# FifthEpoch/longcat-video-tta

Hardware: AMD Instinct MI355X
Metric: denoised latent frames/sec (49x720p, 50-step CFG denoise) (higher is better)
Workload: dtype bf16; 1 GPU; K3: 49x720p (13 latent frames, 46 800 tokens); DiT 48 blocks x 4096 hidden, CFG 4.0, 50-step flow-match Euler, no conditioning frames; depth=48, parallelism=dp1

## Files before the change

### include/lcv_hip.h

```cpp
#ifndef LCV_HIP_H
#define LCV_HIP_H

#include <stdint.h>

#ifdef __cplusplus
extern "C" {
#endif

#define LCV_OK 0
#define LCV_EINVAL (-1)
#define LCV_EDEVICE (-2)
#define LCV_ELAUNCH (-3)

int lcv_version(void);
const char* lcv_last_error(void);
int lcv_device_check(void);

int lcv_knobs_reload(void);
const char* lcv_knobs_list(void);

int lcv_adaln_modulate_fwd(const void* x, const float* mod, void* y,
                           int64_t B, int64_t T, int64_t S, int64_t C,
                           int64_t mod_stride, int64_t shift_off, int64_t scale_off,
                           float eps, void* stream);
int lcv_adaln_modulate_bwd(const void* x, const float* mod, const void* dy,
                           void* dx, float* dmod,
                           int64_t B, int64_t T, int64_t S, int64_t C,
                           int64_t mod_stride, int64_t shift_off, int64_t scale_off,
                           float eps, const void* dres, void* stream);
int lcv_layernorm_affine_fwd(const void* x, const float* w, const float* b, void* y,
                             int64_t rows, int64_t C, float eps, void* stream);
int lcv_layernorm_affine_bwd(const void* x, const float* w, const void* dy,
                             void* dx, float* dw, float* db,
                             int64_t rows, int64_t C, float eps, const void* dres, void* stream);

int lcv_gate_residual_fwd(const void* x, const void* y, const float* mod, void* out,
                          int64_t B, int64_t T, int64_t S, int64_t C,
                          int64_t mod_stride, int64_t gate_off, void* stream);
int lcv_gate_residual_bwd(const void* y, const float* mod, const void* dout,
                          void* dy, float* dmod,
                          int64_t B, int64_t T, int64_t S, int64_t C,
                          int64_t mod_stride, int64_t gate_off, void* stream);

int lcv_qknorm_rope_fwd(const void* q_in, const void* k_in, const void* v_in,
                        void* q_out, void* k_out, void* v_out,
                        const void* wq, const void* wk, const void* cs,
                        int64_t B, int64_t N, int64_t H,
                        int64_t in_sb, int64_t in_sn,
                        int64_t q_sb, int64_t q_sn,
                        int64_t kv_sb, int64_t kv_sn,
                        int64_t pos_off, float eps, float q_scale, void* stream);
int lcv_qknorm_rope_bwd(const void* q_in, const void* k_in,
                        const void* dq_out, const void* dk_out,
                        void* dq_in, void* dk_in,
                        const void* wq, const void* wk, const void* cs,
                        int64_t B, int64_t N, int64_t H,
                        int64_t in_sb, int64_t in_sn,
                        int64_t q_sb, int64_t q_sn,
                        int64_t kv_sb, int64_t kv_sn,
                        int64_t din_sb, int64_t din_sn,
                        int64_t pos_off, float eps, float q_scale, float* dwq, float* dwk, int64_t dw_slots, void* stream);

int lcv_timestep_embedding(const float* t, float* out, int64_t n, int64_t dim, float max_period, void* stream);

int lcv_attn_fwd(const void* q, const void* k, const void* v, void* o, float* lse,
                 int64_t B, int64_t H, int64_t Nq, int64_t Nk,
                 int64_t q_sb, int64_t q_sn, int64_t q_sh,
                 int64_t k_sb, int64_t k_sn, int64_t k_sh,
                 int64_t v_sb, int64_t v_sn, int64_t v_sh,
                 int64_t o_sb, int64_t o_sn, int64_t o_sh,
                 float scale, void* stream);
const char* lcv_attn_fwd_last_kernel(void);
int64_t lcv_attn_bwd_ws_floats(int64_t B, int64_t H, int64_t Nq, int64_t Nk);
int lcv_attn_bwd(const void* q, const void* k, const void* v, const void* o,
                 const void* d_o, const float* lse,
                 void* dq, void* dk, void* dv,
                 float* delta_ws, int accumulate_kv,
                 int64_t B, int64_t H, int64_t Nq, int64_t Nk,
                 int64_t q_sb, int64_t q_sn, int64_t q_sh,
                 int64_t k_sb, int64_t k_sn, int64_t k_sh,
                 int64_t v_sb, int64_t v_sn, int64_t v_sh,
                 int64_t o_sb, int64_t o_sn, int64_t o_sh,
                 int64_t dq_sb, int64_t dq_sn, int64_t dq_sh,
                 int64_t dk_sb, int64_t dk_sn, int64_t dk_sh,
                 int64_t dv_sb, int64_t dv_sn, int64_t dv_sh,
                 float scale, void* stream);

#define LCV_EPI_NONE 0
#define LCV_EPI_SWIGLU 1
#define LCV_EPI_GATE_RESIDUAL 2
#define LCV_EPI_GELU_TANH 3
#define LCV_EPI_SILU 4
int lcv_gemm_nt(const void* a, const void* w, const void* bias,
                const void* a2, const void* w2,
                void* c, int64_t M, int64_t N, int64_t K, int64_t K2,
                int64_t lda, int64_t ldw, int64_t lda2, int64_t ldw2, int64_t ldc,
                int epilogue, int out_f32,
                const void* resid, const float* mod, int64_t rows_per_frame,
                int64_t mod_stride, int64_t gate_off,
                void* stream);
int lcv_gemm_set_workspace(void* ws, int64_t bytes);
int lcv_lora_down(const void* x, const void* A, void* h, int64_t M, int64_t K, int64_t R,
                  int64_t Rpad, int64_t ldx, float s, void* stream);
int lcv_tn_skinny(const void* g, const void* x, float* out, int64_t M, int64_t K, int64_t R, int64_t Rpad,
                  int64_t ldx, float scale, float* ws, int64_t ws_bytes, void* stream);
int64_t lcv_tn_skinny_ws_bytes(int64_t M, int64_t K, int64_t R);
int lcv_linear_f32_smallm(const float* a, const void* w, const void* bias, float* out, int64_t M, int64_t N,
                          int64_t K, int act_in, void* stream);
int lcv_linear_f32_smallm_bwd(const float* dy, const void* w, const float* a, float* da, int64_t M, int64_t N,
                              int64_t K, int act_in, void* stream);

int lcv_swiglu_fwd(const void* gate, const void* up, void* out, int64_t rows, int64_t F,
                   int64_t ld_in, void* stream);
int lcv_swiglu_bwd(const void* gate, const void* up, const void* dout, void* dgate, void* dup,
                   int64_t rows, int64_t F, int64_t ld_in, void* stream);
int lcv_swiglu_bwd_interleaved(const void* gu, const void* dout, void* dgu, int64_t rows, int64_t F, void* stream);

int lcv_patchify(const void* x, void* tok, int64_t B, int64_t Cin, int64_t T, int64_t H, int64_t W,
                 int64_t Kpad, void* stream);
int lcv_unpatchify(const void* tok, float* out, int64_t B, int64_t Cout, int64_t T, int64_t H, int64_t W,
                   int tok_is_f32, void* stream);
int lcv_unpatchify_bwd(const float* dout, float* dtok, int64_t B, int64_t Cout, int64_t T, int64_t H, int64_t W,
                       void* stream);

int lcv_cfg_euler_step(const float* cond, const float* uncond, float* x, float* ws,
                       int64_t B, int64_t n, float guidance, float dt, int negate,
                       int use_zero_star, void* stream);
int lcv_euler_step(const float* v, float* x, int64_t n, float dt, int negate, void* stream);

int lcv_fm_noise(const void* x0, const void* eps, const float* sigma, void* out,
                 int64_t B, int64_t per_sample, void* stream);
#define LCV_FM_MSE_BLOCKS 1024
int lcv_fm_mse(const float* pred, const void* eps, const void* x0, float* loss_out, float* dpred, float* ws,
               int64_t B, int64_t C, int64_t T, int64_t Tc, int64_t HW, void* stream);
#define LCV_FM_MSE_PARTS 256
int lcv_fm_mse_samples(const float* pred, const void* eps, const void* x0, float* loss_out, float* ws,
                       int64_t B, int64_t C, int64_t T, int64_t Tc, int64_t HW, int64_t eps_bstride,
                       int64_t x0_bstride, void* stream);

typedef struct {
  void* param;
  void* grad;
  void* exp_avg;
  void* exp_avg_sq;
  int64_t numel;
  int64_t first_chunk;
} lcv_adam_tensor;
int lcv_grad_norm_clip(const lcv_adam_tensor* tensors, int64_t n_tensors, int64_t total_chunks, int param_f32,
                       float max_norm, float* per_tensor_ws, float* norm_coef_out, void* stream);
int lcv_adamw_step(const lcv_adam_tensor* tensors, int64_t n_tensors, int64_t total_chunks, int param_f32,
                   const float* norm_coef, double lr, double beta1, double beta2, double eps, double weight_decay,
                   int64_t step, void* stream);

int lcv_sgd_step(const lcv_adam_tensor* tensors, int64_t n_tensors, int64_t total_chunks, int param_f32,
                 const float* norm_coef, double lr, double weight_decay, void* stream);

int lcv_transpose_pad(const void* in, void* out, int64_t M, int64_t N, int64_t ld, int64_t Mpad, void* stream);
int lcv_rowsum(const void* in, void* out, int64_t rows, int64_t cols, int out_f32, void* stream);
int lcv_linear_f32_smallm_wgrad(const float* dy, const float* a, void* dw, void* db, int64_t M, int64_t N, int64_t K,
                                int act_in, void* stream);
int lcv_gelu_tanh_fwd(const void* x, void* y, int64_t n, void* stream);
int lcv_gelu_tanh_bwd(const void* x, const void* dy, void* dx, int64_t n, void* stream);

int lcv_causal_conv3d(const void* x, const void* w, const void* bias, const void* resid, void* out,
                      const void* zero_page, int64_t B, int64_t Tin, int64_t Hin, int64_t Win, int64_t Cin,
                      int64_t Cout, int64_t ldc, int kt, int kh, int kw, int up2x, void* stream);
const char* lcv_conv3d_last_kernel(void);
int lcv_conv3d_strided(const void* x, const void* w, const void* bias, void* out, const void* zero_page, int64_t B,
                       int64_t Tin, int64_t Hin, int64_t Win, int64_t Cin, int64_t Cout, int64_t ldc, int kt, int kh,
                       int kw, int st, int sh, int sw, int64_t Tout, int64_t Hout, int64_t Wout, void* stream);
int lcv_vae_rmsnorm_silu(const void* x, const void* gamma, void* y, int64_t rows, int64_t C, int64_t Cpad,
                         int apply_silu, void* stream);
int lcv_softmax_rows(const float* s, void* p, int64_t rows, int64_t n, int64_t ld_s, int64_t ld_p, float scale,
                     void* stream);

int lcv_frame_metric_partials(int64_t H, int64_t W, int64_t C, int win, int64_t* n_sqerr, int64_t* n_ssim);
int lcv_frame_sqerr(const float* gen, const void* gt, int gt_is_u8, float* partials, int64_t N, int64_t E, void* stream);
int lcv_frame_ssim(const float* gen, const void* gt, int gt_is_u8, float* partials, int64_t N, int64_t H, int64_t W,
                   int64_t C, const float* window , int win, float cov_norm,
                   int clamp_var, float c1, float c2, void* stream);

int lcv_gather_rows(const void* table, const int64_t* ids, void* out, int64_t n, int64_t C, int64_t vocab, void* stream);
int lcv_t5_rmsnorm(const void* x, const void* w, void* y, int64_t rows, int64_t C, float eps, void* stream);
int lcv_geglu_tanh_fwd(const void* gate, const void* up, void* out, int64_t rows, int64_t F, int64_t ld_in, void* stream);
int lcv_t5_attention(const void* q, const void* k, const void* v, void* out, const float* bias_by_dist,
                     const int* key_mask, int64_t B, int64_t S, int64_t H, int64_t ld_qkv, int64_t ld_o, int64_t bs_qkv,
                     int64_t bs_o, void* stream);

#ifdef __cplusplus
}
#endif
#endif
```

### longcat-video-tta_amd/csrc/attn_common.h

```cpp
#pragma once
#include "lcv_common.h"

#define AS3 __attribute__((address_space(3)))
typedef AS3 unsigned char lds_u8;
typedef __attribute__((address_space(1))) void gbl_void_t;
typedef AS3 void lds_void_t;
#define SCHED_FENCE() __builtin_amdgcn_sched_barrier(0)
#define ATTN_RESCALE_THR 6.0f

__device__ __forceinline__ int lane_now() { return (int)__builtin_amdgcn_mbcnt_hi(~0u, __builtin_amdgcn_mbcnt_lo(~0u, 0u)); }

__device__ __forceinline__ void half_pair(float v, float& lo, float& hi) {
  float a = v, b = v;
  asm volatile("s_nop 1\n\tv_permlane32_swap_b32 %0, %1\n\ts_nop 0" : "+v"(a), "+v"(b));
  lo = a;
  hi = b;
}
__device__ __forceinline__ float half_max(float v) {
  float lo, hi;
  half_pair(v, lo, hi);
  return fmaxf(lo, hi);
}
__device__ __forceinline__ float half_sum(float v) {
  float lo, hi;
  half_pair(v, lo, hi);
  return lo + hi;
}

__device__ __forceinline__ float gap_exp2(float x) { float y; asm volatile("v_exp_f32 %0, %1" : "=v"(y) : "v"(x)); return y; }
__device__ __forceinline__ float gap_add(float a, float b) { float y; asm volatile("v_add_f32 %0, %1, %2" : "=v"(y) : "v"(a), "v"(b)); return y; }
__device__ __forceinline__ float gap_max3(float a, float b, float c) { float y; asm volatile("v_max3_f32 %0, %1, %2, %3" : "=v"(y) : "v"(a), "v"(b), "v"(c)); return y; }
__device__ __forceinline__ unsigned gap_pack(float lo, float hi) { unsigned y; asm volatile("v_cvt_pk_bf16_f32 %0, %1, %2" : "=v"(y) : "v"(lo), "v"(hi)); return y; }

__device__ __forceinline__ int attn_swz(int row) { return ((row & 3) << 2) | ((row >> 2) & 3); }
__device__ __forceinline__ int attn_tile_off(int row, int ch) { return 256 * row + 16 * (ch ^ attn_swz(row)); }

#define ATTN_BLOCK_DECODE(p, blk, head, b)            \
  {                                                   \
    if ((p).xcd_remap) {                              \
      const int id = blockIdx.x;                      \
      const int xcd = id & 7, j = id >> 3;            \
      const int pair = (j / (p).gx) * 8 + xcd;        \
      blk = j - (j / (p).gx) * (p).gx;                \
      head = pair % (p).d.H;                          \
      b = pair / (p).d.H;                             \
    } else {                                          \
      blk = blockIdx.x; head = blockIdx.y; b = blockIdx.z; \
    }                                                 \
  }
struct AttnGrid { int gx, xcd_remap; dim3 grid; };
static inline AttnGrid attn_grid(int64_t B, int64_t H, int64_t blocks, bool enabled) {
  AttnGrid g;
  g.gx = (int)blocks;
  g.xcd_remap = (enabled && (B * H) % 8 == 0 && blocks >= 8) ? 1 : 0;
  g.grid = g.xcd_remap ? dim3((unsigned)blocks * (unsigned)(H * B)) : dim3((unsigned)blocks, (unsigned)H, (unsigned)B);
  return g;
}

struct AttnArgs {
  const void *q, *k, *v;
  void* o;
  const void* d_o;
  float* lse;
  float* delta_ws;
  void *dq, *dk, *dv;
  int64_t B, H, Nq, Nk;
  int64_t q_sb, q_sn, q_sh, k_sb, k_sn, k_sh, v_sb, v_sn, v_sh, o_sb, o_sn, o_sh;
  int64_t dq_sb, dq_sn, dq_sh, dk_sb, dk_sn, dk_sh, dv_sb, dv_sn, dv_sh;
  float scale;
  int accumulate_kv;
};
struct AttnDims {
  int64_t Nq, Nk;
  int H;
  int64_t q_sb, q_sn, q_sh, k_sb, k_sn, k_sh, v_sb, v_sn, v_sh, o_sb, o_sn, o_sh;
};
static inline AttnDims attn_dims(const AttnArgs& a) {
  return {a.Nq, a.Nk, (int)a.H, a.q_sb, a.q_sn, a.q_sh, a.k_sb, a.k_sn, a.k_sh, a.v_sb, a.v_sn, a.v_sh, a.o_sb, a.o_sn, a.o_sh};
}
struct AttnFwdLead {
  const bf16_t* q;
  const bf16_t* k;
  const bf16_t* v;
  bf16_t* o;
  float* lse;
  AttnDims d;
};
static inline AttnFwdLead attn_fwd_lead(const AttnArgs& a) {
  return {(const bf16_t*)a.q, (const bf16_t*)a.k, (const bf16_t*)a.v, (bf16_t*)a.o, a.lse, attn_dims(a)};
}

static inline bool attn_raise_lds(const void* kern, size_t bytes) {
  return hipFuncSetAttribute(kern, hipFuncAttributeMaxDynamicSharedMemorySize, (int)bytes) == hipSuccess;
}
#define ATTN_RAISE_LDS_ONCE(name, ok)                        \
  do {                                                       \
    static const bool attr_ok__ = (ok);                      \
    if (!attr_ok__) {                                        \
      lcv_set_error("%s: cannot raise dynamic LDS", name);   \
      return LCV_EDEVICE;                                    \
    }                                                        \
  } while (0)

int attn_fwd_w64_launch(const AttnArgs& a, bool xcd_ok, hipStream_t s);
int attn_fwd_pipe_launch(const AttnArgs& a, bool xcd_ok, hipStream_t s);
int attn_bwd_dq2_launch(const AttnArgs& a, hipStream_t s);
int attn_bwd_dkv2_launch(const AttnArgs& a, hipStream_t s);
```

### longcat-video-tta_amd/csrc/attn_fwd.hip

```cpp
#include "attn_common.h"
#include <type_traits>

struct AttnFwdParams : AttnFwdLead {
  float scale, scale_log2e;
  int gx, xcd_remap;
};

template <int NWAVES, int PRIO, bool XATTN, int VAR>
__global__ __launch_bounds__(NWAVES * 64) void attn_fwd_kernel(const AttnFwdParams p) {
  constexpr bool DMA = (VAR & 1) != 0;
  constexpr bool UNIT = (VAR & 2) != 0;
  static_assert(!DMA || NWAVES == 8, "LDS-DMA staging is laid out for 8 waves (2 K + 2 V instructions per wave)");
  constexpr int NT = NWAVES * 64;
  constexpr int QROWS = NWAVES * 32;
  constexpr int NCH = 1024 / NT;
  constexpr int TILE_BYTES = 64 * 256;
  extern __shared__ __attribute__((aligned(16))) unsigned char smem[];
  lds_u8* lds = (lds_u8*)smem;

  const int tid = threadIdx.x;
  const int lane = tid & 63;
  const int wave = __builtin_amdgcn_readfirstlane(tid >> 6);
  const int r = lane & 31, h = lane >> 5;
  int qb, head;
  int64_t b;
  ATTN_BLOCK_DECODE(p, qb, head, b);
  const int64_t q0 = (int64_t)qb * QROWS + wave * 32;

  const bf16_t* kbase = p.k + b * p.d.k_sb + (int64_t)head * p.d.k_sh;
  const bf16_t* vbase = p.v + b * p.d.v_sb + (int64_t)head * p.d.v_sh;

  bf16x8 qf[8];
  {
    int64_t qrow = q0 + r;
    if (qrow > p.d.Nq - 1) qrow = p.d.Nq - 1;
    const bf16_t* qp = p.q + b * p.d.q_sb + qrow * p.d.q_sn + (int64_t)head * p.d.q_sh + 8 * h;
#pragma unroll
    for (int ks = 0; ks < 8; ++ks) qf[ks] = *reinterpret_cast<const bf16x8*>(qp + 16 * ks);
  }

  int st_off[NCH];
  int st_row[NCH];
#pragma unroll
  for (int i = 0; i < NCH; ++i) {
    const int c = tid + i * NT;
    st_row[i] = c >> 4;
    st_off[i] = attn_tile_off(c >> 4, c & 15);
  }
  const int st_col = (tid & 15) * 8;
  u32x4 kreg[NCH], vreg[NCH];
  const bf16_t* kdma[2];
  const bf16_t* vdma[2];
  int dma_row[2], dma_col[2];
#pragma unroll
  for (int i = 0; i < 2; ++i) {
    dma_row[i] = 8 * wave + 4 * i + (lane >> 4);
    dma_col[i] = 8 * ((lane & 15) ^ attn_swz(dma_row[i]));
    kdma[i] = kbase + dma_row[i] * p.d.k_sn + dma_col[i];
    vdma[i] = vbase + dma_row[i] * p.d.v_sn + dma_col[i];
  }
  auto dma_half = [&](auto which_c, int t, int buf, auto full_c) {
    constexpr int which = decltype(which_c)::value;
    constexpr bool FULL = decltype(full_c)::value;
    lds_u8* dst = lds + buf * 2 * TILE_BYTES + which * TILE_BYTES + wave * 2048;
    const bf16_t** src = which ? vdma : kdma;
    const int64_t sn = which ? p.d.v_sn : p.d.k_sn;
    if (FULL || (int64_t)t * 64 + 64 <= p.d.Nk) {
#pragma unroll
      for (int i = 0; i < 2; ++i) {
        __builtin_amdgcn_global_load_lds((gbl_void_t*)src[i], (lds_void_t*)(dst + 1024 * i), 16, 0, 0);
        src[i] += 64 * sn;
      }
    } else {
#pragma unroll
      for (int i = 0; i < 2; ++i) {
        int64_t back = (int64_t)t * 64 + dma_row[i] - (p.d.Nk - 1);
        if (back < 0) back = 0;
        __builtin_amdgcn_global_load_lds((gbl_void_t*)(src[i] - back * sn), (lds_void_t*)(dst + 1024 * i), 16, 0, 0);
      }
    }
  };
  using K_ = std::integral_constant<int, 0>;
  using V_ = std::integral_constant<int, 1>;
  auto dma_tile = [&](int t, int buf, auto full_c) {
    dma_half(K_{}, t, buf, full_c);
    dma_half(V_{}, t, buf, full_c);
  };
  auto load_tile = [&](int64_t kv0) {
#pragma unroll
    for (int i = 0; i < NCH; ++i) {
      int64_t row = kv0 + st_row[i];
      if (row > p.d.Nk - 1) row = p.d.Nk - 1;
      kreg[i] = *reinterpret_cast<const u32x4*>(kbase + row * p.d.k_sn + st_col);
      vreg[i] = *reinterpret_cast<const u32x4*>(vbase + row * p.d.v_sn + st_col);
    }
  };
  auto store_tile = [&](int buf) {
    lds_u8* kb = lds + buf * 2 * TILE_BYTES;
#pragma unroll
    for (int i = 0; i < NCH; ++i) {
      *reinterpret_cast<__attribute__((address_space(3))) u32x4*>(kb + st_off[i]) = kreg[i];
      *reinterpret_cast<__attribute__((address_space(3))) u32x4*>(kb + TILE_BYTES + st_off[i]) = vreg[i];
    }
  };

  const int kf = attn_swz(r);
  const int k_row_off = 256 * r;
  const int q4 = (lane >> 2) & 3, p4 = lane & 3, g1 = (lane >> 4) & 1;
  int v_base[2], v_low[2];
#pragma unroll
  for (int half = 0; half < 2; ++half) {
    v_base[half] = 256 * (4 * h + 8 * half + q4) + 8 * (p4 & 1);
    v_low[half] = (2 * g1 + (p4 >> 1)) ^ (h + 2 * half);
  }

  f32x16 oacc[4];
#pragma unroll
  for (int d = 0; d < 4; ++d)
#pragma unroll
    for (int e = 0; e < 16; ++e) oacc[d][e] = 0.f;
  float m_run = UNIT ? 0.f : -INFINITY;
  f32x16 minit;
#pragma unroll
  for (int e = 0; e < 16; ++e) minit[e] = 0.f;
  float l_run = 0.f;

  if (PRIO == 1 && wave >= NWAVES / 2) __builtin_amdgcn_s_setprio(1);
  const int nt = (int)((p.d.Nk + 63) / 64);
  {
    if (DMA) {
      dma_tile(0, 0, std::false_type{});
    } else {
      load_tile(0);
      store_tile(0);
    }
    __syncthreads();
  }

  auto tile_body = [&](const int t, auto buf_c, auto last_c, auto next_full_c) {
    constexpr int buf = decltype(buf_c)::value;
    constexpr bool has_next = !decltype(last_c)::value;
    if (has_next) {
      if (DMA) dma_tile(t + 1, buf ^ 1, next_full_c);
      else load_tile((int64_t)(t + 1) * 64);
    }

    const lds_u8* kb = lds + buf * 2 * TILE_BYTES;
    const lds_u8* vb = kb + TILE_BYTES;

    f32x16 s0, s1;
#pragma unroll
    for (int e = 0; e < 16; ++e) { s0[e] = UNIT ? minit[e] : 0.f; s1[e] = UNIT ? minit[e] : 0.f; }
#pragma unroll
    for (int ks = 0; ks < 8; ++ks) {
      const int co = 16 * ((2 * ks + h) ^ kf);
      const bf16x8 a0 = *reinterpret_cast<const __attribute__((address_space(3))) bf16x8*>(kb + k_row_off + co);
      const bf16x8 a1 = *reinterpret_cast<const __attribute__((address_space(3))) bf16x8*>(kb + 32 * 256 + k_row_off + co);
      s0 = __builtin_amdgcn_mfma_f32_32x32x16_bf16(a0, qf[ks], s0, 0, 0, 0);
      s1 = __builtin_amdgcn_mfma_f32_32x32x16_bf16(a1, qf[ks], s1, 0, 0, 0);
    }

    if (!has_next && (p.d.Nk & 63)) {
      const int valid = (int)(p.d.Nk - (int64_t)t * 64);
#pragma unroll
      for (int e = 0; e < 16; ++e) {
        const int key = (e & 3) + 8 * (e >> 2) + 4 * h;
        if (key >= valid) s0[e] = -INFINITY;
        if (key + 32 >= valid) s1[e] = -INFINITY;
      }
    }

    float mxa = s0[0], mxb = s1[0];
#pragma unroll
    for (int e = 1; e < 16; ++e) {
      mxa = fmaxf(mxa, s0[e]);
      mxb = fmaxf(mxb, s1[e]);
    }
    float mx = fmaxf(mxa, mxb);
    mx = half_max(mx);
    float psum = 0.f;
    if constexpr (UNIT) {
      if (__builtin_amdgcn_ballot_w64(mx > ATTN_RESCALE_THR) != 0ull || t == 0) {
        const float d = (t == 0) ? mx : fmaxf(mx, 0.f);
        const float alpha = __builtin_amdgcn_exp2f(-d);
        m_run += d;
        l_run *= alpha;
#pragma unroll
        for (int dd = 0; dd < 4; ++dd)
#pragma unroll
          for (int e = 0; e < 16; ++e) oacc[dd][e] *= alpha;
#pragma unroll
        for (int e = 0; e < 16; ++e) {
          s0[e] -= d;
          s1[e] -= d;
          minit[e] = -m_run;
        }
      }
#pragma unroll
      for (int e = 0; e < 16; ++e) {
        s0[e] = __builtin_amdgcn_exp2f(s0[e]);
        s1[e] = __builtin_amdgcn_exp2f(s1[e]);
        psum += s0[e] + s1[e];
      }
    } else {
      if (__builtin_amdgcn_ballot_w64((mx - m_run) * p.scale_log2e > ATTN_RESCALE_THR) != 0ull) {
        const float m_new = fmaxf(m_run, mx);
        const float alpha = __builtin_amdgcn_exp2f((m_run - m_new) * p.scale_log2e);
        m_run = m_new;
        l_run *= alpha;
#pragma unroll
        for (int d = 0; d < 4; ++d)
#pragma unroll
          for (int e = 0; e < 16; ++e) oacc[d][e] *= alpha;
      }
      const float mc = m_run * p.scale_log2e;
#pragma unroll
      for (int e = 0; e < 16; ++e) {
        s0[e] = __builtin_amdgcn_exp2f(s0[e] * p.scale_log2e - mc);
        s1[e] = __builtin_amdgcn_exp2f(s1[e] * p.scale_log2e - mc);
        psum += s0[e] + s1[e];
      }
    }
    l_run += psum;

    bf16x8 pb[4];
#pragma unroll
    for (int j = 0; j < 8; ++j) {
      pb[0][j] = (__bf16)s0[j];
      pb[1][j] = (__bf16)s0[8 + j];
      pb[2][j] = (__bf16)s1[j];
      pb[3][j] = (__bf16)s1[8 + j];
    }

#pragma unroll
    for (int kk = 0; kk < 4; ++kk) {
#pragma unroll
      for (int d = 0; d < 4; ++d) {
        const int dx = 64 * (d ^ q4);
        const s16x4 lo = __builtin_amdgcn_ds_read_tr16_b64_v4i16(
            (__attribute__((address_space(3))) s16x4*)(vb + v_base[0] + 4096 * kk + dx + 16 * v_low[0]));
        const s16x4 hi = __builtin_amdgcn_ds_read_tr16_b64_v4i16(
            (__attribute__((address_space(3))) s16x4*)(vb + v_base[1] + 4096 * kk + dx + 16 * v_low[1]));
        const bf16x8 vf = __builtin_bit_cast(bf16x8, __builtin_shufflevector(lo, hi, 0, 1, 2, 3, 4, 5, 6, 7));
        oacc[d] = __builtin_amdgcn_mfma_f32_32x32x16_bf16(vf, pb[kk], oacc[d], 0, 0, 0);
      }
    }

    if (has_next && !DMA) store_tile(buf ^ 1);
    __syncthreads();
  };
  {
    using B0 = std::integral_constant<int, 0>;
    using B1 = std::integral_constant<int, 1>;
    using Y = std::true_type;
    using N = std::false_type;
    int t = 0;
    for (; t + 3 < nt; t += 2) {
      tile_body(t, B0{}, N{}, Y{});
      tile_body(t + 1, B1{}, N{}, Y{});
    }
    const int left = nt - t;
    if (left == 3) {
      tile_body(t, B0{}, N{}, Y{});
      tile_body(t + 1, B1{}, N{}, N{});
      tile_body(t + 2, B0{}, Y{}, N{});
    } else if (left == 2) {
      tile_body(t, B0{}, N{}, N{});
      tile_body(t + 1, B1{}, Y{}, N{});
    } else {
      tile_body(t, B0{}, Y{}, N{});
    }
  }

  const float l_tot = half_sum(l_run);
  const float inv = 1.0f / l_tot;
  const int64_t qrow = q0 + r;
  if (qrow < p.d.Nq) {
    bf16_t* op = p.o + b * p.d.o_sb + qrow * p.d.o_sn + (int64_t)head * p.d.o_sh;
#pragma unroll
    for (int d = 0; d < 4; ++d)
#pragma unroll
      for (int i = 0; i < 4; ++i) {
        u16x4 pk;
#pragma unroll
        for (int e = 0; e < 4; ++e) pk[e] = f2bf(oacc[d][4 * i + e] * inv);
        *reinterpret_cast<u16x4*>(op + 32 * d + 8 * i + 4 * h) = pk;
      }
    if (p.lse && h == 0) p.lse[(b * p.d.H + head) * p.d.Nq + qrow] = m_run * p.scale + __logf(l_tot);
  }
}

static thread_local const char* g_last_attn_kernel = "none";
extern "C" const char* lcv_attn_fwd_last_kernel(void) { return g_last_attn_kernel; }

extern "C" int lcv_attn_fwd(const void* q, const void* k, const void* v, void* o, float* lse, int64_t B,
                            int64_t H, int64_t Nq, int64_t Nk, int64_t q_sb, int64_t q_sn, int64_t q_sh,
                            int64_t k_sb, int64_t k_sn, int64_t k_sh, int64_t v_sb, int64_t v_sn,
                            int64_t v_sh, int64_t o_sb, int64_t o_sn, int64_t o_sh, float scale,
                            void* stream) {
  LCV_CHECK_ARG(q && k && v && o, "attn_fwd: null pointer");
  LCV_CHECK_ARG(B > 0 && H > 0 && H <= 65535 && B <= 65535, "attn_fwd: bad B/H");
  LCV_CHECK_ARG(Nk > 0, "attn_fwd: Nk must be > 0 (empty key set has no softmax)");
  LCV_CHECK_ARG(q_sn % 8 == 0 && k_sn % 8 == 0 && v_sn % 8 == 0 && q_sh % 8 == 0 && k_sh % 8 == 0 &&
                    v_sh % 8 == 0 && q_sb % 8 == 0 && k_sb % 8 == 0 && v_sb % 8 == 0,
                "attn_fwd: q/k/v strides must be multiples of 8 elements");
  LCV_CHECK_ARG(o_sn % 4 == 0 && o_sh % 4 == 0 && o_sb % 4 == 0, "attn_fwd: o strides must be multiples of 4 elements");
  LCV_CHECK_ARG(((uintptr_t)q % 16 == 0) && ((uintptr_t)k % 16 == 0) && ((uintptr_t)v % 16 == 0) && ((uintptr_t)o % 8 == 0),
                "attn_fwd: pointers must be 16-byte aligned");
  if (Nq == 0) return LCV_OK;
  AttnArgs a = {};
  a.q = q; a.k = k; a.v = v; a.o = o; a.lse = lse; a.B = B; a.H = H; a.Nq = Nq; a.Nk = Nk; a.scale = scale;
  a.q_sb = q_sb; a.q_sn = q_sn; a.q_sh = q_sh; a.k_sb = k_sb; a.k_sn = k_sn; a.k_sh = k_sh;
  a.v_sb = v_sb; a.v_sn = v_sn; a.v_sh = v_sh; a.o_sb = o_sb; a.o_sn = o_sn; a.o_sh = o_sh;
  constexpr int NW = 8;
  const size_t lds = 2 * 2 * 64 * 256;
  const char* xe = lcv_knob("LCV_ATTN_XCD");
  const bool xcd_ok = !(xe && xe[0] == '0');
  const AttnGrid g = attn_grid(B, H, (Nq + NW * 32 - 1) / (NW * 32), xcd_ok);
  const AttnFwdParams p = {attn_fwd_lead(a), scale, scale * 1.4426950408889634f, g.gx, g.xcd_remap};
  auto launch = [&](auto kern) -> int {
    if (!attn_raise_lds((const void*)kern, lds)) {
      lcv_set_error("attn_fwd: cannot raise dynamic LDS");
      return LCV_EDEVICE;
    }
    hipLaunchKernelGGL(kern, g.grid, dim3(NW * 64), lds, (hipStream_t)stream, p);
    return LCV_OK;
  };
  const bool unit = p.scale_log2e > 1.0f - 4e-7f && p.scale_log2e < 1.0f + 4e-7f;
  int rc;
  const bool span32 = (uint64_t)Nk * (uint64_t)(k_sn > v_sn ? k_sn : v_sn) * 2 < (1ull << 32) &&
                      (uint64_t)Nq * (uint64_t)q_sn * 2 < (1ull << 32);
  const char* we = lcv_knob("LCV_ATTN_FWD_W64");
  if (unit && Nk > 512 && span32 && !(we && we[0] == '0')) {
    g_last_attn_kernel = "attn_fwd_w64_kernel";
    return attn_fwd_w64_launch(a, xcd_ok, (hipStream_t)stream);
  }
  if (unit && Nk > 512 && span32) {
    g_last_attn_kernel = "attn_fwd_pipe_kernel";
    return attn_fwd_pipe_launch(a, xcd_ok, (hipStream_t)stream);
  }
  if (Nk <= 512) { g_last_attn_kernel = "attn_fwd_kernel<8, 0, true, 0>"; rc = launch(attn_fwd_kernel<NW, 0, true, 0>); }
  else if (unit) { g_last_attn_kernel = "attn_fwd_kernel<8, 0, false, 3>"; rc = launch(attn_fwd_kernel<NW, 0, false, 3>); }
  else { g_last_attn_kernel = "attn_fwd_kernel<8, 0, false, 1>"; rc = launch(attn_fwd_kernel<NW, 0, false, 1>); }
  if (rc != LCV_OK) return rc;
  LCV_LAUNCH_CHECK("attn_fwd");
  return LCV_OK;
}
```

### longcat-video-tta_amd/csrc/attn_fwd_w64.hip

```cpp
#include "attn_common.h"
#include <type_traits>

struct AttnFwdW64Params : AttnFwdLead {
  float scale;
  int gx, xcd_remap;
};

template <int I, int N, class F>
__device__ __forceinline__ void w64_static_for(F&& f) {
  if constexpr (I < N) { f(std::integral_constant<int, I>{}); w64_static_for<I + 1, N>(f); }
}
enum : unsigned char { W64_NONE, W64_EXP, W64_ADD, W64_PACK, W64_LRUN, W64_VOFF, W64_MAX, W64_HMAX, W64_BALLOT, W64_M0, W64_DMA };
struct W64Op { unsigned char kind, b, e; };
constexpr int W64_SLOTS = 6;
constexpr W64Op W64_P1[32][W64_SLOTS] = {
  {{W64_EXP, 0, 0}, {W64_EXP, 1, 0}},
  {{W64_EXP, 0, 1}},
  {{W64_PACK, 0, 0}, {W64_ADD, 0, 1}, {W64_EXP, 1, 1}, {W64_EXP, 0, 2}},
  {{W64_ADD, 0, 2}, {W64_PACK, 1, 0}, {W64_ADD, 1, 1}, {W64_EXP, 1, 2}},
  {{W64_ADD, 1, 2}, {W64_EXP, 0, 3}, {W64_EXP, 1, 3}},
  {{W64_PACK, 0, 1}, {W64_ADD, 0, 3}, {W64_PACK, 1, 1}, {W64_ADD, 1, 3}, {W64_EXP, 0, 4}},
  {{W64_ADD, 0, 4}, {W64_EXP, 1, 4}, {W64_EXP, 0, 5}},
  {{W64_PACK, 0, 2}, {W64_ADD, 0, 5}, {W64_ADD, 1, 4}, {W64_EXP, 1, 5}},
  {{W64_PACK, 1, 2}, {W64_ADD, 1, 5}, {W64_EXP, 0, 6}, {W64_EXP, 1, 6}},
// ... 76 lines not shown
constexpr bool w64_apart(int from, int to) {
  const int gf = from / 8, gt = to / 8;
  for (int g = gf; g <= gt; ++g) {
    const int ph = g < 32 ? 1 : 2, i = g & 31;
    if ((g > gf && w64_read_first(ph, i)) || (g < gt && w64_wait_last(ph, i))) return true;
  }
  return false;
}
constexpr bool w64_table_complete() {
  int exp_at[2][32] = {}, add_at[2][32] = {}, pack_at[2][16] = {}, max_at[2][9] = {}, n = 0;
  for (int b = 0; b < 2; ++b) for (int m = 0; m < 9; ++m) max_at[b][m] = -1;
  for (int b = 0; b < 2; ++b) for (int e = 0; e < 32; ++e) { exp_at[b][e] = -1; add_at[b][e] = -1; }
  for (int b = 0; b < 2; ++b) for (int m = 0; m < 16; ++m) pack_at[b][m] = -1;
  for (int g = 0; g < 64; ++g)
    for (int s = 0; s < W64_SLOTS; ++s) {
      const W64Op o = g < 32 ? W64_P1[g][s] : W64_P2[g - 32][s];
      const int at = 8 * g + s;
      if (o.kind == W64_EXP) { if (exp_at[o.b][o.e] >= 0) return false; exp_at[o.b][o.e] = at; ++n; }
      if (o.kind == W64_ADD) { if (o.e == 0 || exp_at[o.b][o.e] < 0 || (o.e > 1 && add_at[o.b][o.e - 1] < 0)) return false; add_at[o.b][o.e] = at; }
      if (o.kind == W64_PACK) { if (exp_at[o.b][2 * o.e] < 0 || exp_at[o.b][2 * o.e + 1] < 0) return false; pack_at[o.b][o.e] = at; }
      if (o.kind == W64_LRUN && add_at[o.b][31] < 0) return false;
      if (o.kind == W64_MAX) { if (o.e > 0 && max_at[o.b][o.e - 1] < 0) return false; max_at[o.b][o.e] = at; }
      if (o.kind == W64_HMAX && max_at[o.b][8] < 0) return false;
      if (o.kind == W64_ADD && !(w64_apart(exp_at[o.b][o.e], at) && w64_apart(o.e == 1 ? exp_at[o.b][0] : add_at[o.b][o.e - 1], at))) return false;
      if (o.kind == W64_PACK && !(w64_apart(exp_at[o.b][2 * o.e], at) && w64_apart(exp_at[o.b][2 * o.e + 1], at))) return false;
      if (o.kind == W64_LRUN && !w64_apart(add_at[o.b][31], at)) return false;
      if (o.kind == W64_MAX && o.e > 0 && !w64_apart(max_at[o.b][o.e - 1], at)) return false;
      if (o.kind == W64_HMAX && !w64_apart(max_at[o.b][8], at)) return false;
    }
  for (int b = 0; b < 2; ++b)
    for (int m = 0; m < 16; ++m)
      if (pack_at[b][m] < 0 || pack_at[b][m] >= 8 * (32 + 8 * (m / 4) + b - 1) + W64_SLOTS) return false;
  return n == 64;
}
static_assert(w64_table_complete(), "attn_fwd_w64 gap table: an exp, add or pack is missing, doubled, out of order or right behind what it reads");
static_assert(w64_table_ok(W64_P1, 1, 38, 2) && w64_table_ok(W64_P2, 2, 37, 1), "attn_fwd_w64 gap table over its budget");

template <bool GUARD>
__device__ __forceinline__ void mfma_s(f32x16& c, const bf16x8& a, const bf16x8& b) {
  if constexpr (GUARD) asm volatile("s_nop 3\n\tv_mfma_f32_32x32x16_bf16 %0, %1, %2, %0" : "+v"(c) : "v"(a), "a"(b));
  else asm volatile("v_mfma_f32_32x32x16_bf16 %0, %1, %2, %0" : "+v"(c) : "v"(a), "a"(b));
}
template <bool GUARD>
__device__ __forceinline__ void mfma_s_first(f32x16& d, const f32x16& c, const bf16x8& a, const bf16x8& b) {
  if constexpr (GUARD) asm volatile("s_nop 3\n\tv_mfma_f32_32x32x16_bf16 %0, %2, %3, %1" : "=&v"(d) : "v"(c), "v"(a), "a"(b));
  else asm volatile("v_mfma_f32_32x32x16_bf16 %0, %2, %3, %1" : "=&v"(d) : "v"(c), "v"(a), "a"(b));
}
template <bool GUARD>
__device__ __forceinline__ void mfma_o(f32x16& c, const bf16x8& a, const bf16x8& b) {
  if constexpr (GUARD) asm volatile("s_nop 3\n\tv_mfma_f32_32x32x16_bf16 %0, %1, %2, %0" : "+a"(c) : "v"(a), "v"(b));
  else asm volatile("v_mfma_f32_32x32x16_bf16 %0, %1, %2, %0" : "+a"(c) : "v"(a), "v"(b));
}

#define SCW(S, nb, j) (S[(j) >> 4][nb][(j) & 15])

__global__ __launch_bounds__(256) void attn_fwd_w64_kernel(const AttnFwdW64Params p) {
  constexpr int TILE = 64 * 256;
  extern __shared__ __attribute__((aligned(16))) unsigned char smem[];
  lds_u8* lds = (lds_u8*)smem;
  constexpr int V_REGION = 2 * TILE;

  const int tid = threadIdx.x;
  const int lane = tid & 63;
  const int wave = __builtin_amdgcn_readfirstlane(tid >> 6);
  const int r = lane & 31, h = lane >> 5;
  int qb, head;
  int64_t b;
  ATTN_BLOCK_DECODE(p, qb, head, b);
  const int64_t q0 = (int64_t)qb * 256 + wave * 64;
  const int nt = (int)((p.d.Nk + 63) / 64);
  const bool ragged = (p.d.Nk & 63) != 0;
  const char* kbase_u = lcv_uniform_ptr(p.k + b * p.d.k_sb + (int64_t)head * p.d.k_sh);
  const char* vbase_u = lcv_uniform_ptr(p.v + b * p.d.v_sb + (int64_t)head * p.d.v_sh);

  auto dma_row_of = [&](int ln, int i) { return 16 * wave + 4 * i + (ln >> 4); };
  auto dma_colb_of = [&](int ln, int i) {
    const int row = dma_row_of(ln, i);
    return 16 * ((ln & 15) ^ attn_swz(row));
  };
  unsigned koff[4], voff[4];
#pragma unroll
  for (int i = 0; i < 4; ++i) {
    koff[i] = (unsigned)(dma_row_of(lane, i) * p.d.k_sn * 2 + dma_colb_of(lane, i));
    voff[i] = (unsigned)(dma_row_of(lane, i) * p.d.v_sn * 2 + dma_colb_of(lane, i));
  }
  auto last_off = [&](int i, int64_t sn) {
    const int ln = lane_now();
    int64_t row = (int64_t)(nt - 1) * 64 + dma_row_of(ln, i);
    if (row > p.d.Nk - 1) row = p.d.Nk - 1;
    return (unsigned)(row * sn * 2 + dma_colb_of(ln, i));
  };
  const unsigned lds_wave = (unsigned)(uintptr_t)lds + (unsigned)wave * 4096u;
  auto dma_one = [&](int which, int i, int dst_tile, int tile, bool known_full) __attribute__((always_inline)) {
    const int64_t sn = which ? p.d.v_sn : p.d.k_sn;
    const char* base = which ? vbase_u : kbase_u;
    unsigned off = which ? voff[i] : koff[i];
    if (!known_full && tile == nt - 1) off = last_off(i, sn);
    else base += (int64_t)tile * (128 * sn);
    asm volatile("s_mov_b32 m0, %2\n\ts_nop 0\n\tglobal_load_lds_dwordx4 %0, %1"
                 :: "v"(off), "s"(base), "s"(lds_wave + (unsigned)dst_tile + 1024u * i) : "memory", "m0");
  };
  auto dma_m0 = [&](int i, int dst_tile) __attribute__((always_inline)) {
    asm volatile("s_mov_b32 m0, %0" :: "s"(lds_wave + (unsigned)dst_tile + 1024u * i) : "memory", "m0");
  };
  auto dma_req = [&](int which, int i, int tile, bool known_full) __attribute__((always_inline)) {
    const int64_t sn = which ? p.d.v_sn : p.d.k_sn;
    const char* base = which ? vbase_u : kbase_u;
    unsigned off = which ? voff[i] : koff[i];
    if (!known_full && tile == nt - 1) off = last_off(i, sn);
    else base += (int64_t)tile * (128 * sn);
    asm volatile("global_load_lds_dwordx4 %0, %1" :: "v"(off), "s"(base) : "memory");
  };
  auto dma_tile = [&](int which, int dst_tile, int tile) __attribute__((always_inline)) {
#pragma unroll
    for (int i = 0; i < 4; ++i) dma_one(which, i, dst_tile, tile, false);
  };
  constexpr int KOP = 0, VOP = 1;
  auto dma_wait_and_barrier = [&]() { asm volatile("s_waitcnt vmcnt(0)\n\ts_barrier" ::: "memory"); };

  int k_off[8];
  int v_off[2][4];
  auto set_read_offsets = [&](int ln, int slot) {
    const int rr = ln & 31, hh = ln >> 5;
    const int kfz = ((rr & 3) << 2) | ((rr >> 2) & 3);
#pragma unroll
    for (int ks = 0; ks < 8; ++ks) k_off[ks] = 256 * rr + 16 * ((2 * ks + hh) ^ kfz);
    const int q4 = (ln >> 2) & 3, p4 = ln & 3, g1 = (ln >> 4) & 1;
#pragma unroll
    for (int half = 0; half < 2; ++half)
#pragma unroll
      for (int d = 0; d < 4; ++d)
        v_off[half][d] = (int)(unsigned)(uintptr_t)lds + V_REGION + slot * TILE + 256 * (4 * hh + 8 * half + q4) + 8 * (p4 & 1) + 64 * (d ^ q4) +
                         16 * ((2 * g1 + (p4 >> 1)) ^ (hh + 2 * half));
  };
  set_read_offsets(lane, 2);
  auto read_k = [&](const lds_u8* kb, int f) __attribute__((always_inline)) -> bf16x8 {
    return *reinterpret_cast<const AS3 bf16x8*>(kb + (f & 1) * 32 * 256 + k_off[f >> 1]);
  };
  auto read_v = [&](int g) __attribute__((always_inline)) -> bf16x8 {
    const s16x4 lo = __builtin_amdgcn_ds_read_tr16_b64_v4i16((AS3 s16x4*)(uintptr_t)(unsigned)(v_off[0][g & 3] + 4096 * (g >> 2)));
    const s16x4 hi = __builtin_amdgcn_ds_read_tr16_b64_v4i16((AS3 s16x4*)(uintptr_t)(unsigned)(v_off[1][g & 3] + 4096 * (g >> 2)));
    return __builtin_bit_cast(bf16x8, __builtin_shufflevector(lo, hi, 0, 1, 2, 3, 4, 5, 6, 7));
  };

  bf16x8 qf[2][8];
#pragma unroll
  for (int nb = 0; nb < 2; ++nb) {
    int64_t qrow = q0 + 32 * nb + r;
    if (qrow > p.d.Nq - 1) qrow = p.d.Nq - 1;
    const bf16_t* qp = p.q + b * p.d.q_sb + qrow * p.d.q_sn + (int64_t)head * p.d.q_sh + 8 * h;
#pragma unroll
    for (int ks = 0; ks < 8; ++ks) qf[nb][ks] = *reinterpret_cast<const bf16x8*>(qp + 16 * ks);
  }
#pragma unroll
  for (int nb = 0; nb < 2; ++nb)
#pragma unroll
    for (int ks = 0; ks < 8; ++ks) asm volatile("" : "+a"(qf[nb][ks]));

  f32x16 oacc[2][4];
#pragma unroll
  for (int nb = 0; nb < 2; ++nb)
#pragma unroll
    for (int d = 0; d < 4; ++d) {
#pragma unroll
      for (int e = 0; e < 16; ++e) oacc[nb][d][e] = 0.f;
      asm volatile("" : "+a"(oacc[nb][d]));
    }
  float m_run[2] = {0.f, 0.f}, l_run[2] = {0.f, 0.f};
  f32x16 minit[2];
#pragma unroll
  for (int nb = 0; nb < 2; ++nb)
#pragma unroll
    for (int e = 0; e < 16; ++e) minit[nb][e] = 0.f;
  f32x16 sa[2][2], sb[2][2];

  auto mask_last = [&](f32x16 (&s)[2][2]) __attribute__((always_inline)) {
    const int valid = (int)(p.d.Nk - (int64_t)(nt - 1) * 64);
    const int hh_ = lane_now() >> 5;
#pragma unroll
    for (int nb = 0; nb < 2; ++nb)
#pragma unroll
      for (int e = 0; e < 16; ++e) {
        const int key = (e & 3) + 8 * (e >> 2) + 4 * hh_;
        if (key >= valid) s[0][nb][e] = -INFINITY;
        if (key + 32 >= valid) s[1][nb][e] = -INFINITY;
      }
  };
  auto fence_o = [&]() __attribute__((always_inline)) {
    asm volatile("s_nop 15\n\ts_nop 15\n\ts_nop 15\n\ts_nop 15"
                 : "+a"(oacc[0][0]), "+a"(oacc[0][1]), "+a"(oacc[0][2]), "+a"(oacc[0][3]), "+a"(oacc[1][0]), "+a"(oacc[1][1]),
                   "+a"(oacc[1][2]), "+a"(oacc[1][3]));
  };
  auto fence_s = [&](f32x16 (&s)[2][2]) __attribute__((always_inline)) {
    asm volatile("s_nop 15\n\ts_nop 15\n\ts_nop 15\n\ts_nop 15" : "+v"(s[0][0]), "+v"(s[0][1]), "+v"(s[1][0]), "+v"(s[1][1]));
  };
  auto settle = [&](f32x16 (&s)[2][2], auto nb_c, float mx, bool first, bool need) __attribute__((always_inline)) {
    constexpr int nb = decltype(nb_c)::value;
    if (need || first) {
      fence_o();
      const float d = first ? mx : fmaxf(mx, 0.f);
      const float alpha = __builtin_amdgcn_exp2f(-d);
      m_run[nb] += d;
      l_run[nb] *= alpha;
#pragma unroll
      for (int dd = 0; dd < 4; ++dd)
#pragma unroll
        for (int e = 0; e < 16; ++e) oacc[nb][dd][e] *= alpha;
#pragma unroll
      for (int e = 0; e < 16; ++e) {
        s[0][nb][e] -= d;
        s[1][nb][e] -= d;
        asm volatile("v_mov_b32 %0, %1" : "+v"(minit[nb][e]) : "v"(-m_run[nb]));
      }
      fence_o();
    }
  };

#ifndef W64_PD
#define W64_PD 2
#endif
  constexpr int PD = W64_PD, RING = PD + 1;
  bf16x8 kfr[RING], vfr[RING];
  int v_slot = 2;
  auto next_v_slot = [&]() __attribute__((always_inline)) -> int {
    v_slot = (v_slot == 2) ? 0 : v_slot + 1;
    return (v_slot == 0) ? -2 * TILE : TILE;
  };

  dma_tile(KOP, 0, 0);
  dma_tile(VOP, V_REGION, 0);
  dma_tile(KOP, TILE, 1);
  dma_tile(VOP, V_REGION + TILE, 1);
  dma_wait_and_barrier();
  {
#pragma unroll
    for (int kb_ = 0; kb_ < 2; ++kb_)
#pragma unroll
      for (int nb = 0; nb < 2; ++nb)
#pragma unroll
        for (int e = 0; e < 16; ++e) sa[kb_][nb][e] = 0.f;
#pragma unroll
    for (int f = 0; f < 16; ++f) {
      const bf16x8 a = read_k(lds, f);
      mfma_s<true>(sa[f & 1][0], a, qf[0][f >> 1]);
      mfma_s<true>(sa[f & 1][1], a, qf[1][f >> 1]);
    }
    fence_s(sa);
    auto first_settle = [&](auto nb_c) __attribute__((always_inline)) {
      constexpr int nb = decltype(nb_c)::value;
      float mx = sa[0][nb][0];
#pragma unroll
      for (int e = 1; e < 16; ++e) mx = fmaxf(mx, sa[0][nb][e]);
#pragma unroll
      for (int e = 0; e < 16; ++e) mx = fmaxf(mx, sa[1][nb][e]);
      settle(sa, nb_c, half_max(mx), true, true);
    };
    first_settle(std::integral_constant<int, 0>{});
    first_settle(std::integral_constant<int, 1>{});
  }
  __syncthreads();
  dma_tile(KOP, 0, 2);
#pragma unroll
  for (int i = 0; i < PD; ++i) kfr[i] = read_k(lds + TILE, i);

  auto iteration = [&](const int t, auto par_c, auto steady_c, f32x16 (&c)[2][2], f32x16 (&n)[2][2]) __attribute__((always_inline)) {
    constexpr int PAR = decltype(par_c)::value;
    constexpr bool STEADY = decltype(steady_c)::value;
    const lds_u8* kb = lds + (PAR ^ 1) * TILE;
    const lds_u8* kb_next = lds + PAR * TILE;
    const bool has_k3 = STEADY || t + 3 < nt;
    const bool has_v2 = STEADY || t + 2 < nt;
    const int v_delta = next_v_slot();
    const int v_dst = V_REGION + ((v_slot == 0) ? 2 : v_slot - 1) * TILE;
    float psum[2];
    float ex[2][32];
    unsigned pw[2][16];
    float mxa[2] = {0.f, 0.f}, mxb[2] = {0.f, 0.f}, mxh[2] = {0.f, 0.f};
    bool need[2] = {false, false};
    auto run_op = [&](auto phase_c, auto gap_c, auto slot_c) __attribute__((always_inline)) {
      constexpr W64Op o = decltype(phase_c)::value == 1 ? W64_P1[decltype(gap_c)::value][decltype(slot_c)::value]
                                                        : W64_P2[decltype(gap_c)::value][decltype(slot_c)::value];
      constexpr int b_ = o.b, e = o.e;
      if constexpr (o.kind == W64_EXP) ex[b_][e] = gap_exp2(SCW(c, b_, e));
      if constexpr (o.kind == W64_ADD) psum[b_] = gap_add((e == 1) ? ex[b_][0] : psum[b_], ex[b_][e]);
      if constexpr (o.kind == W64_PACK) pw[b_][e] = gap_pack(ex[b_][2 * e], ex[b_][2 * e + 1]);
      if constexpr (o.kind == W64_LRUN) l_run[b_] = gap_add(l_run[b_], psum[b_]);
      if constexpr (o.kind == W64_VOFF) asm volatile("v_add_u32 %0, %1, %0" : "+v"(v_off[b_ >> 2][b_ & 3]) : "s"(v_delta));
      if constexpr (o.kind == W64_MAX) {
        if constexpr (e == 0) {
          mxa[b_] = gap_max3(n[0][b_][0], n[0][b_][1], n[0][b_][2]);
          mxb[b_] = gap_max3(n[1][b_][0], n[1][b_][1], n[1][b_][2]);
        } else if constexpr (e < 7) {
          mxa[b_] = gap_max3(mxa[b_], n[0][b_][2 * e + 1], n[0][b_][2 * e + 2]);
          mxb[b_] = gap_max3(mxb[b_], n[1][b_][2 * e + 1], n[1][b_][2 * e + 2]);
        } else if constexpr (e == 7) {
          mxa[b_] = gap_max3(mxa[b_], n[0][b_][15], mxb[b_]);
        } else {
          mxb[b_] = gap_max3(mxa[b_], n[1][b_][15], n[1][b_][14]);
        }
      }
      if constexpr (o.kind == W64_HMAX) mxh[b_] = half_max(mxb[b_]);
      if constexpr (o.kind == W64_BALLOT) need[b_] = __builtin_amdgcn_ballot_w64(mxh[b_] > ATTN_RESCALE_THR) != 0ull;
      if constexpr (o.kind == W64_M0) {
        if constexpr (b_ < 4) { if (has_k3) dma_m0(b_, (PAR ^ 1) * TILE); }
        else { if (has_v2) dma_m0(b_ & 3, v_dst); }
      }
// ... 139 lines not shown
```

### longcat-video-tta_amd/csrc/elementwise.hip

```cpp
#include "lcv_common.h"
#include "cfg_guidance.h"

#define ROWNORM_MAXCH 8

template <int MODE>
__global__ __launch_bounds__(256) void rownorm_fwd_kernel(
    const bf16_t* __restrict__ x, const float* __restrict__ p_add, const float* __restrict__ p_mul,
    bf16_t* __restrict__ y, int64_t rows, int C, int64_t S, int64_t mod_stride, float eps) {
  const int lane = threadIdx.x & 63;
  const int64_t row = (int64_t)blockIdx.x * 4 + (threadIdx.x >> 6);
  if (row >= rows) return;
  const bf16_t* xr = x + row * C;
  float v[ROWNORM_MAXCH][8];
  float sum = 0.f;
#pragma unroll
  for (int ch = 0; ch < ROWNORM_MAXCH; ++ch) {
    const int c = (ch * 64 + lane) * 8;
    if (c < C) {
      u16x8 raw = *reinterpret_cast<const u16x8*>(xr + c);
      unpack8(raw, v[ch]);
#pragma unroll
      for (int i = 0; i < 8; ++i) sum += v[ch][i];
    } else {
#pragma unroll
      for (int i = 0; i < 8; ++i) v[ch][i] = 0.f;
    }
  }
  const float mean = wave_sum(sum) / (float)C;
  float sq = 0.f;
#pragma unroll
  for (int ch = 0; ch < ROWNORM_MAXCH; ++ch) {
    const int c = (ch * 64 + lane) * 8;
    if (c < C) {
#pragma unroll
      for (int i = 0; i < 8; ++i) {
        const float d = v[ch][i] - mean;
        sq += d * d;
      }
    }
  }
  const float rstd = rsqrtf(wave_sum(sq) / (float)C + eps);
  const float* pa = p_add;
  const float* pm = p_mul;
  if (MODE == 0) {
    const int64_t frame = row / S;
    pa += frame * mod_stride;
    pm += frame * mod_stride;
  }
  bf16_t* yr = y + row * C;
#pragma unroll
  for (int ch = 0; ch < ROWNORM_MAXCH; ++ch) {
    const int c = (ch * 64 + lane) * 8;
    if (c < C) {
      const f32x4 a0 = *reinterpret_cast<const f32x4*>(pa + c);
      const f32x4 a1 = *reinterpret_cast<const f32x4*>(pa + c + 4);
      const f32x4 m0 = *reinterpret_cast<const f32x4*>(pm + c);
      const f32x4 m1 = *reinterpret_cast<const f32x4*>(pm + c + 4);
      float o[8];
#pragma unroll
      for (int i = 0; i < 8; ++i) {
        const float xh = (v[ch][i] - mean) * rstd;
        const float mul = (i < 4) ? m0[i] : m1[i - 4];
        const float add = (i < 4) ? a0[i] : a1[i - 4];
        o[i] = (MODE == 0) ? (xh * (mul + 1.0f) + add) : (xh * mul + add);
      }
      *reinterpret_cast<u16x8*>(yr + c) = pack8(o);
    }
  }
}

extern "C" int lcv_adaln_modulate_fwd(const void* x, const float* mod, void* y, int64_t B, int64_t T,
                                      int64_t S, int64_t C, int64_t mod_stride, int64_t shift_off,
                                      int64_t scale_off, float eps, void* stream) {
  LCV_CHECK_ARG(x && mod && y, "adaln_modulate_fwd: null pointer");
  LCV_CHECK_ARG(C > 0 && C % 8 == 0 && C <= 4096, "adaln_modulate_fwd: C=%ld must be a multiple of 8 and <= 4096", (long)C);
  LCV_CHECK_ARG(B > 0 && T > 0 && S > 0, "adaln_modulate_fwd: bad sizes");
  LCV_CHECK_ARG(shift_off % 4 == 0 && scale_off % 4 == 0 && mod_stride % 4 == 0, "adaln_modulate_fwd: offsets must be 16-byte aligned");
  const int64_t rows = B * T * S;
  const unsigned grid = (unsigned)((rows + 3) / 4);
  hipLaunchKernelGGL(rownorm_fwd_kernel<0>, dim3(grid), dim3(256), 0, (hipStream_t)stream,
                     (const bf16_t*)x, mod + shift_off, mod + scale_off, (bf16_t*)y, rows, (int)C, S,
                     mod_stride, eps);
  LCV_LAUNCH_CHECK("adaln_modulate_fwd");
  return LCV_OK;
}

extern "C" int lcv_layernorm_affine_fwd(const void* x, const float* w, const float* b, void* y,
                                        int64_t rows, int64_t C, float eps, void* stream) {
  LCV_CHECK_ARG(x && w && b && y, "layernorm_affine_fwd: null pointer");
  LCV_CHECK_ARG(C > 0 && C % 8 == 0 && C <= 4096, "layernorm_affine_fwd: C=%ld must be a multiple of 8 and <= 4096", (long)C);
  if (rows == 0) return LCV_OK;
  const unsigned grid = (unsigned)((rows + 3) / 4);
  hipLaunchKernelGGL(rownorm_fwd_kernel<1>, dim3(grid), dim3(256), 0, (hipStream_t)stream,
                     (const bf16_t*)x, b, w, (bf16_t*)y, rows, (int)C, (int64_t)1, (int64_t)0, eps);
  LCV_LAUNCH_CHECK("layernorm_affine_fwd");
  return LCV_OK;
}

__global__ __launch_bounds__(256) void gate_residual_fwd_kernel(
    const bf16_t* __restrict__ x, const bf16_t* __restrict__ y, const float* __restrict__ gate,
    bf16_t* __restrict__ out, int64_t n_packets, int cpk , int64_t S, int64_t mod_stride) {
  for (int64_t p = (int64_t)blockIdx.x * blockDim.x + threadIdx.x; p < n_packets;
       p += (int64_t)gridDim.x * blockDim.x) {
    const int64_t row = p / cpk;
    const int c = (int)(p - row * cpk) * 8;
    float xf[8], yf[8], o[8];
    unpack8(*reinterpret_cast<const u16x8*>(x + p * 8), xf);
    unpack8(*reinterpret_cast<const u16x8*>(y + p * 8), yf);
    if (gate) {
      const float* g = gate + (row / S) * mod_stride + c;
      const f32x4 g0 = *reinterpret_cast<const f32x4*>(g);
      const f32x4 g1 = *reinterpret_cast<const f32x4*>(g + 4);
#pragma unroll
      for (int i = 0; i < 8; ++i) o[i] = xf[i] + ((i < 4) ? g0[i] : g1[i - 4]) * yf[i];
    } else {
#pragma unroll
      for (int i = 0; i < 8; ++i) o[i] = xf[i] + yf[i];
    }
    *reinterpret_cast<u16x8*>(out + p * 8) = pack8(o);
  }
}

extern "C" int lcv_gate_residual_fwd(const void* x, const void* y, const float* mod, void* out,
                                     int64_t B, int64_t T, int64_t S, int64_t C, int64_t mod_stride,
                                     int64_t gate_off, void* stream) {
  LCV_CHECK_ARG(x && y && out, "gate_residual_fwd: null pointer");
  LCV_CHECK_ARG(C > 0 && C % 8 == 0, "gate_residual_fwd: C must be a multiple of 8");
  LCV_CHECK_ARG(gate_off % 4 == 0 && mod_stride % 4 == 0, "gate_residual_fwd: offsets must be 16-byte aligned");
  const int64_t n_packets = B * T * S * (C / 8);
  if (n_packets == 0) return LCV_OK;
  int64_t blocks = (n_packets + 255) / 256;
  if (blocks > 256 * 16) blocks = 256 * 16;
  hipLaunchKernelGGL(gate_residual_fwd_kernel, dim3((unsigned)blocks), dim3(256), 0, (hipStream_t)stream,
                     (const bf16_t*)x, (const bf16_t*)y, mod ? mod + gate_off : nullptr, (bf16_t*)out,
                     n_packets, (int)(C / 8), S, mod_stride);
  LCV_LAUNCH_CHECK("gate_residual_fwd");
  return LCV_OK;
}

__device__ __forceinline__ void norm_rope_vec(const bf16_t* src, bf16_t* dst, const float (&w)[8],
                                              const float (&cs)[8], bool do_rope, float eps, float out_scale) {
  float f[8];
  unpack8(*reinterpret_cast<const u16x8*>(src), f);
  float ss = 0.f;
#pragma unroll
  for (int i = 0; i < 8; ++i) ss += f[i] * f[i];
  ss += __shfl_xor(ss, 8, 64);
  ss += __shfl_xor(ss, 4, 64);
  ss += __shfl_xor(ss, 2, 64);
  ss += __shfl_xor(ss, 1, 64);
  const float r = rsqrtf(ss * (1.0f / 128.0f) + eps);
  float o[8];
#pragma unroll
  for (int i = 0; i < 8; ++i) f[i] = bfround(bfround(f[i] * r) * w[i]);
  if (do_rope) {
#pragma unroll
    for (int i = 0; i < 4; ++i) {
      const float c = cs[2 * i], s = cs[2 * i + 1];
      const float x0 = f[2 * i], x1 = f[2 * i + 1];
      o[2 * i] = __fadd_rn(__fmul_rn(x0, c), __fmul_rn(-x1, s));
      o[2 * i + 1] = __fadd_rn(__fmul_rn(x1, c), __fmul_rn(x0, s));
    }
  } else {
#pragma unroll
    for (int i = 0; i < 8; ++i) o[i] = f[i];
  }
#pragma unroll
  for (int i = 0; i < 8; ++i) o[i] *= out_scale;
  *reinterpret_cast<u16x8*>(dst) = pack8(o);
}

__global__ __launch_bounds__(256) void qknorm_rope_fwd_kernel(
    const bf16_t* __restrict__ q_in, const bf16_t* __restrict__ k_in, const bf16_t* __restrict__ v_in,
    bf16_t* __restrict__ q_out, bf16_t* __restrict__ k_out, bf16_t* __restrict__ v_out,
    const bf16_t* __restrict__ wq, const bf16_t* __restrict__ wk, const float* __restrict__ cs_tab,
    int H, int64_t in_sb, int64_t in_sn, int64_t q_sb, int64_t q_sn, int64_t kv_sb, int64_t kv_sn,
    int64_t pos_off, float eps, float q_scale) {
  const int64_t n = blockIdx.x, b = blockIdx.y;
  const int sub = threadIdx.x & 15;
  const int hl = threadIdx.x >> 4;
  float cs[8] = {1, 0, 1, 0, 1, 0, 1, 0};
  const bool do_rope = cs_tab != nullptr;
  if (do_rope) {
    const float* p = cs_tab + ((pos_off + n) * 64 + sub * 4) * 2;
    const f32x4 a = *reinterpret_cast<const f32x4*>(p);
    const f32x4 c = *reinterpret_cast<const f32x4*>(p + 4);
    cs[0] = a[0]; cs[1] = a[1]; cs[2] = a[2]; cs[3] = a[3];
    cs[4] = c[0]; cs[5] = c[1]; cs[6] = c[2]; cs[7] = c[3];
  }
  float wqf[8], wkf[8];
  unpack8(*reinterpret_cast<const u16x8*>(wq + sub * 8), wqf);
  unpack8(*reinterpret_cast<const u16x8*>(wk + sub * 8), wkf);
  const int64_t in_base = b * in_sb + n * in_sn;
  for (int h0 = 0; h0 < H; h0 += 16) {
    const int h = h0 + hl;
    if (h >= H) continue;
    const int64_t off = (int64_t)h * 128 + sub * 8;
    if (q_in) norm_rope_vec(q_in + in_base + off, q_out + b * q_sb + n * q_sn + off, wqf, cs, do_rope, eps, q_scale);
    if (k_in) norm_rope_vec(k_in + in_base + off, k_out + b * kv_sb + n * kv_sn + off, wkf, cs, do_rope, eps, 1.0f);
    if (v_out) {
      *reinterpret_cast<u16x8*>(v_out + b * kv_sb + n * kv_sn + off) =
          *reinterpret_cast<const u16x8*>(v_in + in_base + off);
    }
  }
}

extern "C" int lcv_qknorm_rope_fwd(const void* q_in, const void* k_in, const void* v_in, void* q_out,
                                   void* k_out, void* v_out, const void* wq, const void* wk,
                                   const void* cs, int64_t B, int64_t N, int64_t H, int64_t in_sb,
                                   int64_t in_sn, int64_t q_sb, int64_t q_sn, int64_t kv_sb,
                                   int64_t kv_sn, int64_t pos_off, float eps, float q_scale, void* stream) {
  LCV_CHECK_ARG((q_in || k_in) && wq && wk, "qknorm_rope_fwd: null pointer");
  LCV_CHECK_ARG(q_scale > 0.f, "qknorm_rope_fwd: q_scale must be positive (1 = none)");
  LCV_CHECK_ARG(!q_in || q_out, "qknorm_rope_fwd: q_out missing");
  LCV_CHECK_ARG(!k_in || k_out, "qknorm_rope_fwd: k_out missing");
  LCV_CHECK_ARG(H > 0, "qknorm_rope_fwd: H must be positive");
  LCV_CHECK_ARG(in_sn % 8 == 0 && q_sn % 8 == 0 && kv_sn % 8 == 0 && in_sb % 8 == 0 && q_sb % 8 == 0 && kv_sb % 8 == 0,
                "qknorm_rope_fwd: strides must be multiples of 8 elements");
  if (B == 0 || N == 0) return LCV_OK;
  const bool copy_v = v_out && v_in && v_out != v_in;
  hipLaunchKernelGGL(qknorm_rope_fwd_kernel, dim3((unsigned)N, (unsigned)B), dim3(256), 0,
                     (hipStream_t)stream, (const bf16_t*)q_in, (const bf16_t*)k_in, (const bf16_t*)v_in,
                     (bf16_t*)q_out, (bf16_t*)k_out, copy_v ? (bf16_t*)v_out : nullptr, (const bf16_t*)wq,
                     (const bf16_t*)wk, (const float*)cs, (int)H, in_sb, in_sn, q_sb, q_sn, kv_sb, kv_sn,
                     pos_off, eps, q_scale);
  LCV_LAUNCH_CHECK("qknorm_rope_fwd");
  return LCV_OK;
}

__global__ __launch_bounds__(256) void swiglu_fwd_kernel(const bf16_t* __restrict__ gate,
                                                         const bf16_t* __restrict__ up,
                                                         bf16_t* __restrict__ out, int64_t rows,
                                                         int fpk , int64_t ld_in) {
  const int64_t n_packets = rows * fpk;
  for (int64_t p = (int64_t)blockIdx.x * blockDim.x + threadIdx.x; p < n_packets;
       p += (int64_t)gridDim.x * blockDim.x) {
    const int64_t row = p / fpk;
    const int c = (int)(p - row * fpk) * 8;
    float g[8], u[8], o[8];
    unpack8(*reinterpret_cast<const u16x8*>(gate + row * ld_in + c), g);
    unpack8(*reinterpret_cast<const u16x8*>(up + row * ld_in + c), u);
#pragma unroll
    for (int i = 0; i < 8; ++i) o[i] = bfround(silu_f(g[i])) * u[i];
    *reinterpret_cast<u16x8*>(out + p * 8) = pack8(o);
  }
}

extern "C" int lcv_swiglu_fwd(const void* gate, const void* up, void* out, int64_t rows, int64_t F,
                              int64_t ld_in, void* stream) {
  LCV_CHECK_ARG(gate && up && out, "swiglu_fwd: null pointer");
  LCV_CHECK_ARG(F % 8 == 0 && ld_in % 8 == 0, "swiglu_fwd: F and ld_in must be multiples of 8");
  const int64_t n_packets = rows * (F / 8);
  if (n_packets == 0) return LCV_OK;
  int64_t blocks = (n_packets + 255) / 256;
  if (blocks > 256 * 16) blocks = 256 * 16;
  hipLaunchKernelGGL(swiglu_fwd_kernel, dim3((unsigned)blocks), dim3(256), 0, (hipStream_t)stream,
                     (const bf16_t*)gate, (const bf16_t*)up, (bf16_t*)out, rows, (int)(F / 8), ld_in);
  LCV_LAUNCH_CHECK("swiglu_fwd");
  return LCV_OK;
}

__global__ __launch_bounds__(256) void patchify_kernel(const bf16_t* __restrict__ x,
                                                       bf16_t* __restrict__ tok, int64_t B, int Cin,
                                                       int T, int H, int W, int Kpad) {
  const int Hh = H / 2, Wh = W / 2;
  const int kq = Kpad / 4;
  const int64_t total = (int64_t)B * T * Hh * Wh * kq;
  for (int64_t i = (int64_t)blockIdx.x * blockDim.x + threadIdx.x; i < total;
       i += (int64_t)gridDim.x * blockDim.x) {
    const int c = (int)(i % kq);
    int64_t tkn = i / kq;
    const int wq = (int)(tkn % Wh);
    int64_t r = tkn / Wh;
    const int hq = (int)(r % Hh);
    r /= Hh;
    const int t = (int)(r % T);
    const int64_t b = r / T;
    u16x4 o = {0, 0, 0, 0};
    if (c < Cin) {
      const bf16_t* p = x + ((((b * Cin + c) * T + t) * H + 2 * hq) * (int64_t)W + 2 * wq);
      const u16x2 r0 = *reinterpret_cast<const u16x2*>(p);
      const u16x2 r1 = *reinterpret_cast<const u16x2*>(p + W);
      o[0] = r0[0]; o[1] = r0[1]; o[2] = r1[0]; o[3] = r1[1];
    }
    *reinterpret_cast<u16x4*>(tok + tkn * Kpad + c * 4) = o;
  }
}

extern "C" int lcv_patchify(const void* x, void* tok, int64_t B, int64_t Cin, int64_t T, int64_t H,
                            int64_t W, int64_t Kpad, void* stream) {
  LCV_CHECK_ARG(x && tok, "patchify: null pointer");
  LCV_CHECK_ARG(H % 2 == 0 && W % 2 == 0, "patchify: H, W must be even (patch 1x2x2)");
  LCV_CHECK_ARG(Kpad % 4 == 0 && Kpad >= Cin * 4, "patchify: Kpad must be a multiple of 4 and >= 4*Cin");
  const int64_t total = B * T * (H / 2) * (W / 2) * (Kpad / 4);
  if (total == 0) return LCV_OK;
  int64_t blocks = (total + 255) / 256;
  if (blocks > 256 * 16) blocks = 256 * 16;
  hipLaunchKernelGGL(patchify_kernel, dim3((unsigned)blocks), dim3(256), 0, (hipStream_t)stream,
                     (const bf16_t*)x, (bf16_t*)tok, B, (int)Cin, (int)T, (int)H, (int)W, (int)Kpad);
  LCV_LAUNCH_CHECK("patchify");
  return LCV_OK;
}

template <typename TokT>
__global__ __launch_bounds__(256) void unpatchify_kernel(const TokT* __restrict__ tok,
                                                         float* __restrict__ out, int64_t B, int Cout,
                                                         int T, int H, int W) {
  const int Hh = H / 2, Wh = W / 2;
  const int64_t total = (int64_t)B * Cout * T * H * W;
  for (int64_t i = (int64_t)blockIdx.x * blockDim.x + threadIdx.x; i < total;
       i += (int64_t)gridDim.x * blockDim.x) {
    const int w = (int)(i % W);
    int64_t r = i / W;
    const int h = (int)(r % H);
    r /= H;
    const int t = (int)(r % T);
    r /= T;
    const int c = (int)(r % Cout);
    const int64_t b = r / Cout;
    const int64_t tkn = ((b * T + t) * Hh + (h >> 1)) * Wh + (w >> 1);
    const int k = ((h & 1) * 2 + (w & 1)) * Cout + c;
    const TokT vraw = tok[tkn * (4 * Cout) + k];
// ... 253 lines not shown
```

### longcat-video-tta_amd/csrc/lcv_common.h

```cpp
#pragma once
#include <hip/hip_runtime.h>
#include <stdint.h>
#include <stdio.h>
#include <stdarg.h>
#include "../../include/lcv_hip.h"

typedef unsigned short bf16_t;
typedef __attribute__((ext_vector_type(2))) unsigned short u16x2;
typedef __attribute__((ext_vector_type(4))) unsigned short u16x4;
typedef __attribute__((ext_vector_type(8))) unsigned short u16x8;
typedef __attribute__((ext_vector_type(8))) __bf16 bf16x8;
typedef __attribute__((ext_vector_type(4))) __bf16 bf16x4;
typedef __attribute__((ext_vector_type(4))) short s16x4;
typedef __attribute__((ext_vector_type(4))) float f32x4;
typedef __attribute__((ext_vector_type(16))) float f32x16;
typedef __attribute__((ext_vector_type(4))) unsigned int u32x4;
typedef __attribute__((ext_vector_type(2))) unsigned int u32x2;

#define LCV_WAVE 64

void lcv_set_error(const char* fmt, ...);
#define LCV_CHECK_ARG(cond, ...)            \
  do {                                      \
    if (!(cond)) {                          \
      lcv_set_error(__VA_ARGS__);           \
      return LCV_EINVAL;                    \
    }                                       \
  } while (0)
#define LCV_LAUNCH_CHECK(name)                                             \
  do {                                                                     \
    hipError_t e__ = hipGetLastError();                                    \
    if (e__ != hipSuccess) {                                               \
      lcv_set_error("%s: launch failed: %s", name, hipGetErrorString(e__)); \
      return LCV_ELAUNCH;                                                  \
    }                                                                      \
  } while (0)

const char* lcv_knob(const char* name);

__device__ __forceinline__ float bf2f(bf16_t u) {
  return __builtin_bit_cast(float, (unsigned int)u << 16);
}
__device__ __forceinline__ bf16_t f2bf(float f) {
  __bf16 b = (__bf16)f;
  return __builtin_bit_cast(bf16_t, b);
}
__device__ __forceinline__ float bfround(float f) { return bf2f(f2bf(f)); }

__device__ __forceinline__ void unpack8(const u16x8& v, float (&f)[8]) {
#pragma unroll
  for (int i = 0; i < 8; ++i) f[i] = bf2f(v[i]);
}
__device__ __forceinline__ u16x8 pack8(const float (&f)[8]) {
  u16x8 v;
#pragma unroll
  for (int i = 0; i < 8; ++i) v[i] = f2bf(f[i]);
  return v;
}

__device__ __forceinline__ float wave_sum(float v) {
#pragma unroll
  for (int o = 32; o > 0; o >>= 1) v += __shfl_xor(v, o, 64);
  return v;
}
__device__ __forceinline__ float wave_max(float v) {
#pragma unroll
  for (int o = 32; o > 0; o >>= 1) v = fmaxf(v, __shfl_xor(v, o, 64));
  return v;
}

__device__ __forceinline__ float silu_f(float x) { return x / (1.0f + __expf(-x)); }

__device__ __forceinline__ void lcv_lds_dma16(const void* gsrc, unsigned lds_dst) {
  unsigned keep;
  asm volatile("s_mov_b32 %0, m0\n\ts_mov_b32 m0, %2\n\ts_nop 0\n\tglobal_load_lds_dwordx4 %1, off\n\ts_mov_b32 m0, %0"
               : "=&s"(keep)
               : "v"(gsrc), "s"(lds_dst)
               : "memory");
}
__device__ __forceinline__ void lcv_lds_dma16_sv(unsigned voff, const char* sbase, unsigned lds_dst) {
  unsigned keep;
  asm volatile("s_mov_b32 %0, m0\n\ts_mov_b32 m0, %3\n\ts_nop 0\n\tglobal_load_lds_dwordx4 %1, %2\n\ts_mov_b32 m0, %0"
               : "=&s"(keep)
               : "v"(voff), "s"(sbase), "s"(lds_dst)
               : "memory");
}
__device__ __forceinline__ void lcv_lds_dma4_sv(unsigned voff, const char* sbase, unsigned lds_dst) {
  unsigned keep;
  asm volatile("s_mov_b32 %0, m0\n\ts_mov_b32 m0, %3\n\ts_nop 0\n\tglobal_load_lds_dword %1, %2\n\ts_mov_b32 m0, %0"
               : "=&s"(keep)
               : "v"(voff), "s"(sbase), "s"(lds_dst)
               : "memory");
}
__device__ __forceinline__ const char* lcv_uniform_ptr(const void* ptr) {
  const unsigned long long v = (unsigned long long)ptr;
  const unsigned lo = __builtin_amdgcn_readfirstlane((unsigned)v), hi = __builtin_amdgcn_readfirstlane((unsigned)(v >> 32));
  return (const char*)(((unsigned long long)hi << 32) | lo);
}
__device__ __forceinline__ void lcv_dma_wait_all() { asm volatile("s_waitcnt vmcnt(0)" ::: "memory"); }
```

### longcat-video-tta_amd/csrc/lib.hip

```cpp
#include "lcv_common.h"
#include <mutex>
#include <stdlib.h>
#include <string.h>

static thread_local char g_err[512] = "";

void lcv_set_error(const char* fmt, ...) {
  va_list ap;
  va_start(ap, fmt);
  vsnprintf(g_err, sizeof(g_err), fmt, ap);
  va_end(ap);
}

extern "C" int lcv_version(void) { return 14; }

extern "C" const char* lcv_last_error(void) { return g_err; }

extern "C" int lcv_device_check(void) {
  int dev = 0;
  if (hipGetDevice(&dev) != hipSuccess) {
    lcv_set_error("device_check: no HIP device");
    return LCV_EDEVICE;
  }
  hipDeviceProp_t prop;
  if (hipGetDeviceProperties(&prop, dev) != hipSuccess) {
    lcv_set_error("device_check: hipGetDeviceProperties failed");
    return LCV_EDEVICE;
  }
  if (strncmp(prop.gcnArchName, "gfx950", 6) != 0) {
    lcv_set_error("device_check: device is %s, this library is built for gfx950 only", prop.gcnArchName);
    return LCV_EDEVICE;
  }
  return LCV_OK;
}

namespace {
struct Knob { const char* name; char value[32]; bool set; };
Knob g_knobs[] = {
    {"LCV_GEMM_TILE"}, {"LCV_GEMM_GROUP_M"}, {"LCV_GEMM_FAST_EPI"}, {"LCV_GEMM_SPLITK_TAIL"},
    {"LCV_CONV_8P"}, {"LCV_CONV_N192"}, {"LCV_CONV_ROWS"}, {"LCV_CONV_ROWS_GRID"}, {"LCV_CONV_ROWS_ORDER"},
    {"LCV_ATTN_FWD_W64"}, {"LCV_ATTN_XCD"},
    {"LCV_ATTN_BWD_VAR"}, {"LCV_ATTN_BWD_DKV_WAVES"}, {"LCV_ATTN_BWD_DQ_WAVES"}, {"LCV_ATTN_BWD_PIPE"}, {"LCV_ATTN_BWD_STAGGER"},
    {"LCV_ATTN_BWD_XCD"},
};
std::mutex g_knob_mutex;
bool g_knobs_read = false;
void knobs_read_locked() {
  for (Knob& k : g_knobs) {
    const char* e = getenv(k.name);
    k.set = e != nullptr;
    k.value[0] = 0;
    if (e) { strncpy(k.value, e, sizeof(k.value) - 1); k.value[sizeof(k.value) - 1] = 0; }
  }
  g_knobs_read = true;
}
}

const char* lcv_knob(const char* name) {
  std::lock_guard<std::mutex> g(g_knob_mutex);
  if (!g_knobs_read) knobs_read_locked();
  for (const Knob& k : g_knobs)
    if (strcmp(k.name, name) == 0) return k.set ? k.value : nullptr;
  return nullptr;
}

extern "C" int lcv_knobs_reload(void) {
  std::lock_guard<std::mutex> g(g_knob_mutex);
  knobs_read_locked();
  int n = 0;
  for (const Knob& k : g_knobs) n += k.set ? 1 : 0;
  return n;
}

extern "C" const char* lcv_knobs_list(void) {
  static char buf[1024];
  static std::once_flag once;
  std::call_once(once, [] {
    buf[0] = 0;
    for (const Knob& k : g_knobs) { strcat(buf, k.name); strcat(buf, " "); }
  });
  return buf;
}
```

### longcat-video-tta_amd/lcv_hip/autograd_ops.py

```python
import weakref
from typing import List, Optional

import torch

from . import ops
from .lib import (LCV_EPI_GELU_TANH, LCV_EPI_NONE, LCV_EPI_SWIGLU, LcvError)

BF16 = torch.bfloat16
F32 = torch.float32

_EPI = {None: LCV_EPI_NONE, "gelu_tanh": LCV_EPI_GELU_TANH}


def _needs_grad(*ts) -> bool:
    return torch.is_grad_enabled() and any(t is not None and t.requires_grad for t in ts)


_WT_CACHE = {}


def transposed_weight(w: torch.Tensor) -> torch.Tensor:
    key = id(w)
    ent = _WT_CACHE.get(key)
    if ent is not None and ent[0]() is w and ent[1] == w._version and ent[2].data_ptr() != 0:
        return ent[2]
    with torch.no_grad():
        wt = w.detach().t().contiguous()
    _WT_CACHE[key] = (weakref.ref(w, lambda _r, k=key: _WT_CACHE.pop(k, None)), w._version, wt)
    return wt


def clear_weight_caches():
    _WT_CACHE.clear()
    _XT_LAST.clear()


_XT_LAST = {}


def _transposed_input(x: torch.Tensor) -> torch.Tensor:
    key = (x.data_ptr(), x._version, tuple(x.shape))
    ent = _XT_LAST.get("x")
    if ent is not None and ent[0] == key:
        return ent[1]
    xt = ops.transpose_pad(x)
    _XT_LAST["x"] = (key, xt)
    return xt


def _dense_param_grads(x2: torch.Tensor, dyb: torch.Tensor, want_dw: bool, want_db: bool, w_dtype, b_dtype):
    dyT = ops.transpose_pad(dyb)
    dw = ops.dense_wgrad(dyT, _transposed_input(x2)).to(w_dtype) if want_dw else None
    db = ops.rowsum(dyT).to(b_dtype) if want_db else None
    return dw, db


def _pad_cols(t: torch.Tensor, width: int = 64) -> torch.Tensor:
    out = torch.zeros((t.shape[0], width), dtype=t.dtype, device=t.device)
    out[:, : t.shape[1]].copy_(t)
    return out


class _LinearFn(torch.autograd.Function):
    @staticmethod
    def forward(ctx, x, w, b, epi, out_f32):
        ctx.save_for_backward(x if w.requires_grad else None, w)
        ctx.out_f32 = out_f32
        ctx.b_dtype = b.dtype if b is not None else None
        if epi != LCV_EPI_NONE:
            raise LcvError("linear: fused activation epilogues have no backward (use the unfused form when training)")
        return ops.gemm_nt(x, w, b, epilogue=epi, out_f32=out_f32)

    @staticmethod
    def backward(ctx, dy):
        x, w = ctx.saved_tensors
        dyb = (dy if dy.dtype == BF16 else dy.to(BF16)).contiguous()
        N, K = w.shape
        dx = dw = db = None
        if ctx.needs_input_grad[0]:
            if not w.requires_grad:
                wt = transposed_weight(w)
            elif N % 64 == 0 and w.is_contiguous():
                wt = ops.transpose_pad(w.detach())
            else:
                wt = w.detach().t().contiguous()
            dx = ops.gemm_nt(dyb, wt, None)
        want_db = ctx.needs_input_grad[2]
        if w.requires_grad and N <= 32 and not want_db:
            dw = ops.tn_skinny(_pad_cols(dyb), x, N).to(w.dtype)
        elif w.requires_grad and K <= 32 and not want_db:
            dw = ops.tn_skinny(_pad_cols(x), dyb, K).t().contiguous().to(w.dtype)
        elif w.requires_grad or want_db:
            dw, db = _dense_param_grads(x if w.requires_grad else None, dyb, w.requires_grad, want_db, w.dtype, ctx.b_dtype)
        return dx, dw, db, None, None


def linear(x: torch.Tensor, w: torch.Tensor, b: Optional[torch.Tensor], epilogue: Optional[str] = None,
           out_f32: bool = False) -> torch.Tensor:
    x = x if x.dtype == BF16 else x.to(BF16)
    if not x.is_contiguous():
        x = x.contiguous()
    epi = _EPI[epilogue]
    if _needs_grad(x, w, b):
        return _LinearFn.apply(x, w, b, epi, out_f32)
    return ops.gemm_nt(x, w, b, epilogue=epi, out_f32=out_f32)


class _LinearF32Fn(torch.autograd.Function):
    @staticmethod
    def forward(ctx, a, w, b, act_in):
        ctx.save_for_backward(a, w)
        ctx.act_in = act_in
        ctx.b_dtype = b.dtype if b is not None else None
        return ops.linear_f32_smallm(a, w, b, act_in)

    @staticmethod
    def backward(ctx, dy):
        a, w = ctx.saved_tensors
        dw = db = None
        if w.requires_grad or ctx.needs_input_grad[2]:
            dw, db = ops.linear_f32_smallm_wgrad(dy.contiguous().float(), a, ctx.act_in, ctx.needs_input_grad[2])
            dw = dw.to(w.dtype) if w.requires_grad else None
            db = db.to(ctx.b_dtype) if db is not None else None
        da = ops.linear_f32_smallm_bwd(dy.contiguous(), w, a, ctx.act_in) if ctx.needs_input_grad[0] else None
        return da, dw, db, None


def linear_f32(a: torch.Tensor, w: torch.Tensor, b: Optional[torch.Tensor], act_in: int = 0) -> torch.Tensor:
    if _needs_grad(a, w, b):
        return _LinearF32Fn.apply(a.contiguous(), w, b, act_in)
    return ops.linear_f32_smallm(a, w, b, act_in)


class _AdaLNFn(torch.autograd.Function):
    @staticmethod
    def forward(ctx, x, mod, shift_idx, scale_idx, T, eps):
        ctx.save_for_backward(x, mod)
        ctx.args = (shift_idx, scale_idx, T, eps)
        return ops.adaln_modulate(x, mod, shift_idx, scale_idx, T, eps)

    @staticmethod
    def backward(ctx, dy):
        x, mod = ctx.saved_tensors
        shift_idx, scale_idx, T, eps = ctx.args
        dx, dmod = ops.adaln_modulate_bwd(x, mod, dy.contiguous(), shift_idx, scale_idx, T, eps,
                                          need_dmod=ctx.needs_input_grad[1])
        return dx, dmod, None, None, None, None


class _AdaLNForkFn(torch.autograd.Function):

    @staticmethod
    def forward(ctx, x, mod, shift_idx, scale_idx, T, eps):
        ctx.save_for_backward(x, mod)
        ctx.args = (shift_idx, scale_idx, T, eps)
        ctx.set_materialize_grads(False)
        return ops.adaln_modulate(x, mod, shift_idx, scale_idx, T, eps), x.view_as(x)

    @staticmethod
    def backward(ctx, dy, dres):
        x, mod = ctx.saved_tensors
        shift_idx, scale_idx, T, eps = ctx.args
        if dy is None:
            return dres, None, None, None, None, None
        dx, dmod = ops.adaln_modulate_bwd(x, mod, dy.contiguous(), shift_idx, scale_idx, T, eps,
                                          need_dmod=ctx.needs_input_grad[1], dres=dres)
        return dx, dmod, None, None, None, None


def adaln_modulate_fork(x, mod, shift_idx, scale_idx, T, eps=1e-6):
    if _needs_grad(x, mod):
        return _AdaLNForkFn.apply(x, mod, shift_idx, scale_idx, T, eps)
    return ops.adaln_modulate(x, mod, shift_idx, scale_idx, T, eps), x


def adaln_modulate(x, mod, shift_idx, scale_idx, T, eps=1e-6):
    if _needs_grad(x, mod):
        return _AdaLNFn.apply(x, mod, shift_idx, scale_idx, T, eps)
    return ops.adaln_modulate(x, mod, shift_idx, scale_idx, T, eps)


class _LayerNormAffineFn(torch.autograd.Function):
    @staticmethod
    def forward(ctx, x, w, b, eps):
        ctx.save_for_backward(x, w)
        ctx.eps = eps
        return ops.layernorm_affine(x, w, b, eps)

    @staticmethod
    def backward(ctx, dy):
        x, w = ctx.saved_tensors
        dx, dw, db = ops.layernorm_affine_bwd(x, w, dy.contiguous(), ctx.eps,
                                              need_dw=ctx.needs_input_grad[1] or ctx.needs_input_grad[2])
        return dx, (dw.to(w.dtype) if dw is not None else None), (db.to(w.dtype) if db is not None else None), None


class _LayerNormAffineForkFn(torch.autograd.Function):

    @staticmethod
    def forward(ctx, x, w, b, eps):
        ctx.save_for_backward(x, w)
        ctx.eps = eps
        ctx.set_materialize_grads(False)
        return ops.layernorm_affine(x, w, b, eps), x.view_as(x)

    @staticmethod
    def backward(ctx, dy, dres):
        x, w = ctx.saved_tensors
        if dy is None:
            return dres, None, None, None
        dx, dw, db = ops.layernorm_affine_bwd(x, w, dy.contiguous(), ctx.eps,
                                              need_dw=ctx.needs_input_grad[1] or ctx.needs_input_grad[2], dres=dres)
        return dx, (dw.to(w.dtype) if dw is not None else None), (db.to(w.dtype) if db is not None else None), None


def layernorm_affine_fork(x, w, b, eps=1e-6):
    if _needs_grad(x, w, b):
        return _LayerNormAffineForkFn.apply(x, w, b, eps)
    return ops.layernorm_affine(x, w, b, eps), x


def layernorm_affine(x, w, b, eps=1e-6):
    if _needs_grad(x, w, b):
        return _LayerNormAffineFn.apply(x, w, b, eps)
    return ops.layernorm_affine(x, w, b, eps)


class _GateResidualFn(torch.autograd.Function):
    @staticmethod
    def forward(ctx, x, y, mod, gate_idx, T):
        ctx.save_for_backward(y, mod)
        ctx.args = (gate_idx, T)
        return ops.gate_residual(x, y, mod, gate_idx, T)

    @staticmethod
    def backward(ctx, dout):
        y, mod = ctx.saved_tensors
        gate_idx, T = ctx.args
        dout = dout.contiguous()
        if mod is None:
            return dout, dout, None, None, None
        dy, dmod = ops.gate_residual_bwd(y, mod, dout, gate_idx, T, need_dmod=ctx.needs_input_grad[2])
        return dout, dy, dmod, None, None


def gate_residual(x, y, mod, gate_idx, T):
    if _needs_grad(x, y, mod):
        return _GateResidualFn.apply(x, y, mod, gate_idx, T)
    return ops.gate_residual(x, y, mod, gate_idx, T)


class _PadFrontZeroFn(torch.autograd.Function):
    @staticmethod
    def forward(ctx, x, n):
        ctx.n = n
        B, N, C = x.shape
        out = x.new_zeros((B, N + n, C))
        out[:, n:].copy_(x)
        return out

    @staticmethod
    def backward(ctx, dout):
        return dout[:, ctx.n:].contiguous(), None


def pad_front_zero(x: torch.Tensor, n: int) -> torch.Tensor:
    if _needs_grad(x):
        return _PadFrontZeroFn.apply(x, n)
    B, N, C = x.shape
    out = x.new_zeros((B, N + n, C))
    out[:, n:].copy_(x)
    return out


def _attend_regions(q, k, v, scale, n_cond, need_lse):
    B, N, H, D = q.shape
    o = torch.empty((B, N, H, D), dtype=BF16, device=q.device)
    lses = []
    if n_cond > 0:
        _, l1 = ops.attention(q[:, :n_cond], k[:, :n_cond], v[:, :n_cond], scale, out=o[:, :n_cond], need_lse=need_lse)
        lses.append(l1)
        if N > n_cond:
            _, l2 = ops.attention(q[:, n_cond:], k, v, scale, out=o[:, n_cond:], need_lse=need_lse)
            lses.append(l2)
    else:
        _, l1 = ops.attention(q, k, v, scale, out=o, need_lse=need_lse)
        lses.append(l1)
    return o, lses


class _SelfAttentionFn(torch.autograd.Function):
    @staticmethod
    def forward(ctx, qkv, wq, wk, cs, scale, n_cond, eps):
        B, N, _, H, D = qkv.shape
        qk = torch.empty((B, N, 2, H, D), dtype=BF16, device=qkv.device)
        ops.qknorm_rope(qkv[:, :, 0], qkv[:, :, 1], None, qk[:, :, 0], qk[:, :, 1], None, wq, wk, cs, 0, eps,
                        q_scale=ops.log2_qscale(scale))
        o, lses = _attend_regions(qk[:, :, 0], qk[:, :, 1], qkv[:, :, 2], ops.LN2, n_cond, True)
        ctx.save_for_backward(qkv, qk, o, wq, wk, cs, *lses)
        ctx.args = (scale, n_cond, eps)
        return o

    @staticmethod
    def backward(ctx, do):
        qkv, qk, o, wq, wk, cs, *lses = ctx.saved_tensors
        scale, n_cond, eps = ctx.args
        want_dw = wq.requires_grad or wk.requires_grad
        B, N, _, H, D = qkv.shape
        do = do.contiguous()
        dqkv = torch.empty_like(qkv)
        dqk_r = torch.empty((B, N, 2, H, D), dtype=BF16, device=qkv.device)
        q, k, v = qk[:, :, 0], qk[:, :, 1], qkv[:, :, 2]
        dq, dk, dv = dqk_r[:, :, 0], dqk_r[:, :, 1], dqkv[:, :, 2]
        if n_cond > 0 and N > n_cond:
            ops.attention_bwd(q[:, n_cond:], k, v, o[:, n_cond:], do[:, n_cond:], lses[1],
                              dq[:, n_cond:], dk, dv, ops.LN2, accumulate_kv=False)
            ops.attention_bwd(q[:, :n_cond], k[:, :n_cond], v[:, :n_cond], o[:, :n_cond], do[:, :n_cond], lses[0],
                              dq[:, :n_cond], dk[:, :n_cond], dv[:, :n_cond], ops.LN2, accumulate_kv=True)
        else:
            ops.attention_bwd(q, k, v, o, do, lses[0], dq, dk, dv, ops.LN2, accumulate_kv=False)
        dwq = torch.zeros(D, dtype=torch.float32, device=qkv.device) if want_dw else None
        dwk = torch.zeros(D, dtype=torch.float32, device=qkv.device) if want_dw else None
        ops.qknorm_rope_bwd(qkv[:, :, 0], qkv[:, :, 1], dq, dk, dqkv[:, :, 0], dqkv[:, :, 1], wq, wk, cs, 0, eps,
                            q_scale=ops.log2_qscale(scale), dwq=dwq, dwk=dwk)
        return (dqkv, dwq.to(wq.dtype) if (want_dw and wq.requires_grad) else None,
                dwk.to(wk.dtype) if (want_dw and wk.requires_grad) else None, None, None, None, None)


def self_attention(qkv, wq, wk, cs, scale, n_cond, eps, return_kv=False):
    if _needs_grad(qkv, wq, wk):
        if return_kv:
            raise LcvError("self_attention: return_kv is an inference-only path")
        return _SelfAttentionFn.apply(qkv, wq, wk, cs, scale, n_cond, eps), None
    q, k, v = qkv[:, :, 0], qkv[:, :, 1], qkv[:, :, 2]
    ops.qknorm_rope(q, k, None, q, k, None, wq, wk, cs, 0, eps, q_scale=ops.log2_qscale(scale))
    o, _ = _attend_regions(q, k, v, ops.LN2, n_cond, False)
    kv = (k.contiguous(), v.contiguous()) if return_kv else None
    return o, kv


class _SPSelfAttentionFn(torch.autograd.Function):

    @staticmethod
    def forward(ctx, qkv, wq, wk, cs, scale, eps, sp, n_cond_loc, n_cond_glob):
        B, N, _, H, D = qkv.shape
        qk = torch.empty((B, N, 2, H, D), dtype=BF16, device=qkv.device)
        ops.qknorm_rope(qkv[:, :, 0], qkv[:, :, 1], None, qk[:, :, 0], qk[:, :, 1], None, wq, wk, cs, sp.token_offset, eps,
                        q_scale=ops.log2_qscale(scale))
        k_full, v_full = sp.all_gather_kv(qk[:, :, 1].contiguous(), qkv[:, :, 2].contiguous())
        q = qk[:, :, 0]
        o = torch.empty((B, N, H, D), dtype=BF16, device=qkv.device)
        lses = []
        if n_cond_loc > 0:
            _, l1 = ops.attention(q[:, :n_cond_loc], k_full[:, :n_cond_glob], v_full[:, :n_cond_glob], ops.LN2,
                                  out=o[:, :n_cond_loc], need_lse=True)
            lses.append(l1)
        if N > n_cond_loc:
            _, l2 = ops.attention(q[:, n_cond_loc:], k_full, v_full, ops.LN2, out=o[:, n_cond_loc:], need_lse=True)
            lses.append(l2)
        ctx.save_for_backward(qkv, qk, k_full, v_full, o, wq, wk, cs, *lses)
        ctx.args = (scale, eps, sp, n_cond_loc, n_cond_glob)
        return o

    @staticmethod
    def backward(ctx, do):
        qkv, qk, k_full, v_full, o, wq, wk, cs, *lses = ctx.saved_tensors
        scale, eps, sp, n_cond_loc, n_cond_glob = ctx.args
        B, N, _, H, D = qkv.shape
        do = do.contiguous()
        q = qk[:, :, 0]
        dq = torch.zeros((B, N, H, D), dtype=BF16, device=qkv.device)
        dk_full = sp.padded_zeros(k_full)
        dv_full = sp.padded_zeros(v_full)
        i = 0
        if n_cond_loc > 0:
            ops.attention_bwd(q[:, :n_cond_loc], k_full[:, :n_cond_glob], v_full[:, :n_cond_glob], o[:, :n_cond_loc],
                              do[:, :n_cond_loc], lses[i], dq[:, :n_cond_loc], dk_full[:, :n_cond_glob],
                              dv_full[:, :n_cond_glob], ops.LN2, accumulate_kv=False)
            i += 1
        if N > n_cond_loc:
            ops.attention_bwd(q[:, n_cond_loc:], k_full, v_full, o[:, n_cond_loc:], do[:, n_cond_loc:], lses[i],
                              dq[:, n_cond_loc:], dk_full, dv_full, ops.LN2, accumulate_kv=(n_cond_loc > 0))
        dk = sp.reduce_scatter_kv(dk_full)
        dv = sp.reduce_scatter_kv(dv_full)
        dqkv = torch.empty_like(qkv)
        want_dw = wq.requires_grad or wk.requires_grad
        dwq = torch.zeros(D, dtype=torch.float32, device=qkv.device) if want_dw else None
        dwk = torch.zeros(D, dtype=torch.float32, device=qkv.device) if want_dw else None
        ops.qknorm_rope_bwd(qkv[:, :, 0], qkv[:, :, 1], dq, dk, dqkv[:, :, 0], dqkv[:, :, 1], wq, wk, cs, sp.token_offset, eps,
                            q_scale=ops.log2_qscale(scale), dwq=dwq, dwk=dwk)
        dqkv[:, :, 2].copy_(dv)
        return (dqkv, dwq.to(wq.dtype) if (want_dw and wq.requires_grad) else None,
                dwk.to(wk.dtype) if (want_dw and wk.requires_grad) else None, None, None, None, None, None, None)


def sp_self_attention(qkv, wq, wk, cs, scale, eps, sp, n_cond_loc, n_cond_glob):
    if _needs_grad(qkv, wq, wk):
        return _SPSelfAttentionFn.apply(qkv, wq, wk, cs, scale, eps, sp, n_cond_loc, n_cond_glob)
    B, N, _, H, D = qkv.shape
    q, k, v = qkv[:, :, 0], qkv[:, :, 1], qkv[:, :, 2]
    ops.qknorm_rope(q, k, None, q, k, None, wq, wk, cs, sp.token_offset, eps, q_scale=ops.log2_qscale(scale))
    if n_cond_glob == 0 and sp.overlap and qkv.is_cuda and sp.world > 1:
        return _sp_attention_overlapped(q, k.contiguous(), v.contiguous(), sp)
    k_full, v_full = sp.all_gather_kv(k.contiguous(), v.contiguous())
    if n_cond_glob == 0:
        o, _ = ops.attention(q, k_full, v_full, ops.LN2)
        return o
    o = torch.empty((B, N, H, D), dtype=BF16, device=qkv.device)
    if n_cond_loc > 0:
        ops.attention(q[:, :n_cond_loc], k_full[:, :n_cond_glob], v_full[:, :n_cond_glob], ops.LN2, out=o[:, :n_cond_loc])
    if N > n_cond_loc:
        ops.attention(q[:, n_cond_loc:], k_full, v_full, ops.LN2, out=o[:, n_cond_loc:])
    return o


def _sp_attention_overlapped(q, k_loc, v_loc, sp):
    main = torch.cuda.current_stream()
    side = sp.side_stream(q.device)
    side.wait_stream(main)
    with torch.cuda.stream(side):
        k_full, v_full = sp.all_gather_kv(k_loc, v_loc)
    parts = [ops.attention(q, k_loc, v_loc, ops.LN2, need_lse=True)]
    main.wait_stream(side)
    k_full.record_stream(main); v_full.record_stream(main)
    lo, hi = sp.token_offset, sp.token_offset + k_loc.shape[1]
    if lo > 0:
        parts.append(ops.attention(q, k_full[:, :lo], v_full[:, :lo], ops.LN2, need_lse=True))
    if hi < k_full.shape[1]:
        parts.append(ops.attention(q, k_full[:, hi:], v_full[:, hi:], ops.LN2, need_lse=True))
    return merge_attention_parts(parts)


def merge_attention_parts(parts):
    if len(parts) == 1:
        return parts[0][0]
    lses = torch.stack([l for _, l in parts], 0)
    lse = torch.logsumexp(lses, dim=0)
    out = None
    for (o_i, l_i) in parts:
        w_i = torch.exp(l_i - lse).permute(0, 2, 1).unsqueeze(-1)
        out = o_i.float() * w_i if out is None else out + o_i.float() * w_i
    return out.to(BF16)


def cached_attention(qkv, k_c, v_c, wq, wk, cs, scale, eps):
    if _needs_grad(qkv):
        raise LcvError("cached_attention: the KV-cached step is an inference-only path")
    B, N, _, H, D = qkv.shape
    n_c = k_c.shape[1]
    kbuf = torch.empty((B, n_c + N, H, D), dtype=BF16, device=qkv.device)
    vbuf = torch.empty((B, n_c + N, H, D), dtype=BF16, device=qkv.device)
    kbuf[:, :n_c].copy_(k_c if k_c.shape[0] == B else k_c.expand(B, -1, -1, -1))
    vbuf[:, :n_c].copy_(v_c if v_c.shape[0] == B else v_c.expand(B, -1, -1, -1))
    q = qkv[:, :, 0]
    ops.qknorm_rope(q, qkv[:, :, 1], qkv[:, :, 2], q, kbuf[:, n_c:], vbuf[:, n_c:], wq, wk, cs, n_c, eps,
                    q_scale=ops.log2_qscale(scale))
    o, _ = ops.attention(q, kbuf, vbuf, ops.LN2)
    return o


class _CrossAttentionFn(torch.autograd.Function):
    @staticmethod
    def forward(ctx, q_raw, kv_raw, wq, wk, seqlens, scale, eps):
        B, N, H, D = q_raw.shape
        L = kv_raw.shape[1]
        qn = torch.empty_like(q_raw)
        kn = torch.empty((1, L, H, D), dtype=BF16, device=q_raw.device)
        ops.qknorm_rope(q_raw, None, None, qn, None, None, wq, wk, None, 0, eps)
        ops.qknorm_rope(None, kv_raw[:, :, 0], None, None, kn, None, wq, wk, None, 0, eps)
        o = torch.empty_like(q_raw)
        lses, off = [], 0
        for b in range(B):
            Lb = int(seqlens[b])
            _, l = ops.attention(qn[b:b + 1], kn[:, off:off + Lb], kv_raw[:, off:off + Lb, 1], scale, out=o[b:b + 1],
                                 need_lse=True)
            lses.append(l)
            off += Lb
        ctx.save_for_backward(q_raw, kv_raw, qn, kn, o, wq, wk, *lses)
        ctx.args = (list(seqlens), scale, eps)
        return o

    @staticmethod
    def backward(ctx, do):
        q_raw, kv_raw, qn, kn, o, wq, wk, *lses = ctx.saved_tensors
        seqlens, scale, eps = ctx.args
        want_dw = wq.requires_grad or wk.requires_grad
        B, N, H, D = q_raw.shape
        L = kv_raw.shape[1]
        do = do.contiguous()
        dqn = torch.empty_like(qn)
        dkv = torch.zeros((1, L, 2, H, D), dtype=BF16, device=q_raw.device)
        off = 0
        for b in range(B):
            Lb = int(seqlens[b])
            ops.attention_bwd(qn[b:b + 1], kn[:, off:off + Lb], kv_raw[:, off:off + Lb, 1], o[b:b + 1], do[b:b + 1],
                              lses[b], dqn[b:b + 1], dkv[:, off:off + Lb, 0], dkv[:, off:off + Lb, 1], scale,
                              accumulate_kv=False)
            off += Lb
        dq_raw = torch.empty_like(q_raw)
        dwq = torch.zeros(D, dtype=torch.float32, device=q_raw.device) if want_dw else None
        dwk = torch.zeros(D, dtype=torch.float32, device=q_raw.device) if want_dw else None
        ops.qknorm_rope_bwd(q_raw, None, dqn, None, dq_raw, None, wq, wk, None, 0, eps, dwq=dwq)
        dkv_raw = torch.empty_like(kv_raw)
        ops.qknorm_rope_bwd(None, kv_raw[:, :, 0], None, dkv[:, :, 0], None, dkv_raw[:, :, 0], wq, wk, None, 0, eps, dwk=dwk)
        dkv_raw[:, :, 1].copy_(dkv[:, :, 1])
        return (dq_raw, dkv_raw, dwq.to(wq.dtype) if (want_dw and wq.requires_grad) else None,
                dwk.to(wk.dtype) if (want_dw and wk.requires_grad) else None, None, None, None)


def cross_attention(q, kv, wq, wk, seqlens: List[int], scale, eps):
    if _needs_grad(q, kv, wq, wk):
        return _CrossAttentionFn.apply(q, kv, wq, wk, seqlens, scale, eps)
    B, N, H, D = q.shape
    k, v = kv[:, :, 0], kv[:, :, 1]
    ops.qknorm_rope(q, None, None, q, None, None, wq, wk, None, 0, eps)
    ops.qknorm_rope(None, k, None, None, k, None, wq, wk, None, 0, eps)
    o = torch.empty_like(q)
    off = 0
    for b in range(B):
        Lb = int(seqlens[b])
        ops.attention(q[b:b + 1], k[:, off:off + Lb], v[:, off:off + Lb], scale, out=o[b:b + 1])
        off += Lb
    return o


class _GeluTanhFn(torch.autograd.Function):
    @staticmethod
    def forward(ctx, x):
        ctx.save_for_backward(x)
        return ops.gelu_tanh(x)

    @staticmethod
    def backward(ctx, dy):
        (x,) = ctx.saved_tensors
        return ops.gelu_tanh_bwd(x, (dy if dy.dtype == BF16 else dy.to(BF16)).contiguous())


def gelu_tanh(x: torch.Tensor) -> torch.Tensor:
    if _needs_grad(x):
        return _GeluTanhFn.apply(x)
    return ops.gelu_tanh(x)


class _SwiGLUFn(torch.autograd.Function):
    @staticmethod
    def forward(ctx, g, u):
        ctx.save_for_backward(g, u)
        return ops.swiglu(g, u)

    @staticmethod
    def backward(ctx, dout):
        g, u = ctx.saved_tensors
        dg, du = ops.swiglu_bwd(g, u, dout.contiguous())
        return dg, du


def swiglu(g, u):
    if _needs_grad(g, u):
        return _SwiGLUFn.apply(g, u)
    return ops.swiglu(g, u)


class _SwiGLUFusedFn(torch.autograd.Function):

    @staticmethod
    def forward(ctx, x2, w13):
        gu = torch.empty((x2.shape[0], w13.shape[0]), dtype=BF16, device=x2.device)
        h = ops.gemm_nt(x2, w13, None, epilogue=LCV_EPI_SWIGLU, swiglu_aux=gu)
        ctx.save_for_backward(gu, w13)
        return h

    @staticmethod
    def backward(ctx, dh):
        gu, w13 = ctx.saved_tensors
        dgu = ops.swiglu_bwd_interleaved(gu, dh if dh.is_contiguous() else dh.contiguous())
        return ops.gemm_nt(dgu, transposed_weight(w13), None), None


def swiglu_fused(x2: torch.Tensor, w13: torch.Tensor) -> torch.Tensor:
    x2 = x2 if x2.is_contiguous() else x2.contiguous()
    if torch.is_grad_enabled() and x2.requires_grad:
        return _SwiGLUFusedFn.apply(x2, w13)
    return ops.gemm_nt(x2, w13, None, epilogue=LCV_EPI_SWIGLU)


class _PatchEmbedFn(torch.autograd.Function):

    @staticmethod
    def forward(ctx, x, w, b):
        B, C = x.shape[0], w.shape[0]
        kin = w[0].numel()
        kpad = ((kin + 63) // 64) * 64
        w2 = w.reshape(C, kin)
        if kpad != kin:
            w2 = torch.nn.functional.pad(w2, (0, kpad - kin))
        tok = ops.patchify(x if x.dtype == BF16 else x.to(BF16), kpad).view(-1, kpad)
        ctx.save_for_backward(tok)
        ctx.meta = (tuple(w.shape), kin, w.dtype, b.dtype if b is not None else None, w.requires_grad)
        return ops.gemm_nt(tok, w2.contiguous(), b).view(B, -1, C)

    @staticmethod
    def backward(ctx, dy):
        (tok,) = ctx.saved_tensors
        wshape, kin, wdt, bdt, wreq = ctx.meta
        dyb = dy.reshape(-1, dy.shape[-1])
        dyb = (dyb if dyb.dtype == BF16 else dyb.to(BF16)).contiguous()
        dw2, db = _dense_param_grads(tok, dyb, wreq, ctx.needs_input_grad[2], wdt, bdt)
        dw = dw2[:, :kin].reshape(wshape).contiguous() if dw2 is not None else None
        return None, dw, db


def patch_embed(x: torch.Tensor, w: torch.Tensor, b: torch.Tensor) -> torch.Tensor:
    if _needs_grad(x):
        raise LcvError("patch_embed: gradients w.r.t. the latent input are out of scope")
    if _needs_grad(w, b):
        return _PatchEmbedFn.apply(x, w, b)
    B = x.shape[0]
    C = w.shape[0]
    kin = w[0].numel()
    kpad = ((kin + 63) // 64) * 64
    w2 = w.reshape(C, kin)
    if kpad != kin:
        w2 = torch.nn.functional.pad(w2, (0, kpad - kin))
    tok = ops.patchify(x if x.dtype == BF16 else x.to(BF16), kpad)
    y = ops.gemm_nt(tok.view(-1, kpad), w2.contiguous(), b)
    return y.view(B, -1, C)


class _UnpatchifyFn(torch.autograd.Function):
    @staticmethod
    def forward(ctx, tok, Cout, T, H, W):
        ctx.args = (Cout, T, H, W, tok.dtype)
        return ops.unpatchify(tok, Cout, T, H, W)

    @staticmethod
    def backward(ctx, dout):
        Cout, T, H, W, dt = ctx.args
        return ops.unpatchify_bwd(dout.contiguous(), Cout, T, H, W).to(dt), None, None, None, None


def unpatchify(tok, Cout, T, H, W):
    if _needs_grad(tok):
        return _UnpatchifyFn.apply(tok, Cout, T, H, W)
    return ops.unpatchify(tok, Cout, T, H, W)
```

### longcat-video-tta_amd/lcv_hip/lib.py

```python
import ctypes
import os
from ctypes import c_char_p, c_double, c_float, c_int, c_int64, c_uint64, c_void_p
from pathlib import Path

_LIB_PATH = Path(__file__).resolve().parent / "liblcv_hip.so"

P, I64, F32, I, F64, U64 = c_void_p, c_int64, c_float, c_int, c_double, c_uint64

_SIGNATURES = {
    "lcv_device_check": [],
    "lcv_adaln_modulate_fwd": [P, P, P, I64, I64, I64, I64, I64, I64, I64, F32, P],
    "lcv_adaln_modulate_bwd": [P, P, P, P, P, I64, I64, I64, I64, I64, I64, I64, F32, P, P],
    "lcv_layernorm_affine_fwd": [P, P, P, P, I64, I64, F32, P],
    "lcv_layernorm_affine_bwd": [P, P, P, P, P, P, I64, I64, F32, P, P],
    "lcv_gate_residual_fwd": [P, P, P, P, I64, I64, I64, I64, I64, I64, P],
    "lcv_gate_residual_bwd": [P, P, P, P, P, I64, I64, I64, I64, I64, I64, P],
    "lcv_qknorm_rope_fwd": [P, P, P, P, P, P, P, P, P, I64, I64, I64, I64, I64, I64, I64, I64, I64, I64, F32, F32, P],
    "lcv_qknorm_rope_bwd": [P, P, P, P, P, P, P, P, P, I64, I64, I64, I64, I64, I64, I64, I64, I64, I64, I64, I64, F32, F32, P, P, I64, P],
    "lcv_attn_fwd": [P, P, P, P, P, I64, I64, I64, I64] + [I64] * 12 + [F32, P],
    "lcv_attn_bwd": [P, P, P, P, P, P, P, P, P, P, I, I64, I64, I64, I64] + [I64] * 21 + [F32, P],
    "lcv_gemm_nt": [P, P, P, P, P, P, I64, I64, I64, I64, I64, I64, I64, I64, I64, I, I, P, P, I64, I64, I64, P],
    "lcv_gemm_set_workspace": [P, I64],
    "lcv_linear_f32_smallm": [P, P, P, P, I64, I64, I64, I, P],
    "lcv_lora_down": [P, P, P, I64, I64, I64, I64, I64, F32, P],
    "lcv_tn_skinny": [P, P, P, I64, I64, I64, I64, I64, F32, P, I64, P],
    "lcv_linear_f32_smallm_bwd": [P, P, P, P, I64, I64, I64, I, P],
    "lcv_timestep_embedding": [P, P, I64, I64, F32, P],
    "lcv_swiglu_fwd": [P, P, P, I64, I64, I64, P],
    "lcv_swiglu_bwd": [P, P, P, P, P, I64, I64, I64, P],
    "lcv_swiglu_bwd_interleaved": [P, P, P, I64, I64, P],
    "lcv_patchify": [P, P, I64, I64, I64, I64, I64, I64, P],
    "lcv_unpatchify": [P, P, I64, I64, I64, I64, I64, I, P],
    "lcv_unpatchify_bwd": [P, P, I64, I64, I64, I64, I64, P],
    "lcv_cfg_euler_step": [P, P, P, P, I64, I64, F32, F32, I, I, P],
    "lcv_euler_step": [P, P, I64, F32, I, P],
    "lcv_fm_noise": [P, P, P, P, I64, I64, P],
    "lcv_fm_mse": [P, P, P, P, P, P, I64, I64, I64, I64, I64, P],
    "lcv_fm_mse_samples": [P, P, P, P, P, I64, I64, I64, I64, I64, I64, I64, P],
    "lcv_grad_norm_clip": [P, I64, I64, I, F32, P, P, P],
    "lcv_adamw_step": [P, I64, I64, I, P, F64, F64, F64, F64, F64, I64, P],
    "lcv_sgd_step": [P, I64, I64, I, P, F64, F64, P],
    "lcv_transpose_pad": [P, P, I64, I64, I64, I64, P],
    "lcv_rowsum": [P, P, I64, I64, I, P],
    "lcv_linear_f32_smallm_wgrad": [P, P, P, P, I64, I64, I64, I, P],
    "lcv_gelu_tanh_fwd": [P, P, I64, P],
    "lcv_gelu_tanh_bwd": [P, P, P, I64, P],
    "lcv_causal_conv3d": [P, P, P, P, P, P, I64, I64, I64, I64, I64, I64, I64, I, I, I, I, P],
    "lcv_conv3d_strided": [P, P, P, P, P, I64, I64, I64, I64, I64, I64, I64, I, I, I, I, I, I, I64, I64, I64, P],
    "lcv_vae_rmsnorm_silu": [P, P, P, I64, I64, I64, I, P],
    "lcv_softmax_rows": [P, P, I64, I64, I64, I64, F32, P],
    "lcv_gather_rows": [P, P, P, I64, I64, I64, P],
    "lcv_t5_rmsnorm": [P, P, P, I64, I64, F32, P],
    "lcv_geglu_tanh_fwd": [P, P, P, I64, I64, I64, P],
    "lcv_t5_attention": [P, P, P, P, P, P, I64, I64, I64, I64, I64, I64, I64, P],
    "lcv_frame_metric_partials": [I64, I64, I64, I, P, P],
    "lcv_frame_sqerr": [P, P, I, P, I64, I64, P],
    "lcv_frame_ssim": [P, P, I, P, I64, I64, I64, I64, P, I, F32, I, F32, F32, P],
}

_SIGNATURES_LPIPS = {
    "lcv_lpips_pack_weight": [P, P, I64, I64, I64, I64, I64, P],
    "lcv_lpips_conv_relu": [P, P, I, I, P, P, P, P, I64, I64, I64, I64, I64, I64, I64, I64, I64, I64, P],
    "lcv_lpips_maxpool": [P, P, I64, I64, I64, I64, P],
    "lcv_lpips_tap_distance": [P, P, P, P, I, I64, I64, I64, P],
}
LCV_LPIPS_TAP_BLOCKS = 64

_SIGNATURES_DET = {
    "lcv_det_adaln_modulate_bwd": [P, P, P, P, P, I64, I64, I64, I64, I64, I64, I64, F32, P, P, I64, P],
    "lcv_det_layernorm_affine_bwd": [P, P, P, P, P, P, I64, I64, F32, P, P, I64, P],
    "lcv_det_gate_residual_bwd": [P, P, P, P, P, I64, I64, I64, I64, I64, I64, P, I64, P],
    "lcv_det_qknorm_rope_bwd": [P, P, P, P, P, P, P, P, P, I64, I64, I64, I64, I64, I64, I64, I64, I64, I64, I64, I64, F32, F32, P, P, P, I64, P],
    "lcv_det_linear_f32_smallm_bwd": [P, P, P, P, I64, I64, I64, I, P, I64, P],
    "lcv_det_grad_norm_clip": [P, I64, I64, I, F32, P, P, P, I64, P],
}
LCV_DET_ADALN, LCV_DET_LAYERNORM, LCV_DET_GATE, LCV_DET_QKNORM, LCV_DET_SMALLM, LCV_DET_GRAD_NORM = range(6)

_SIGNATURES_LORA = {
    "lcv_lora_down_dropout": [P, P, P, I64, I64, I64, I64, I64, F32, F64, U64, U64, I64, P],
    "lcv_tn_skinny_dropout": [P, P, P, I64, I64, I64, I64, I64, F32, F64, U64, U64, I64, P, I64, P],
    "lcv_lora_dx_dropout_add": [P, P, P, I64, I64, I64, I64, I64, F64, U64, U64, I64, P],
    "lcv_lora_dropout_mask": [P, I64, I64, F64, U64, U64, I64, P],
}

_SIGNATURES_MASTER = {
    "lcv_master_sgd_step": [P, P, I64, I64, P, F64, F64, P],
    "lcv_master_adamw_step": [P, P, I64, I64, P, F64, F64, F64, F64, F64, I64, P],
    "lcv_master_split": [P, P, P, I64, P],
    "lcv_master_join": [P, P, P, I64, P],
}

_SIGNATURES_MOMENTS8 = {
    "lcv_master_adamw8_step": [P, P, P, I64, I64, P, F64, F64, F64, F64, F64, I64, P],
    "lcv_moments8_encode": [P, P, P, P, P, I64, P],
    "lcv_moments8_decode": [P, P, P, P, P, I64, P],
}

_SIGNATURES_ACCUM = {
    "lcv_grad_accumulate": [P, P, I64, I64, F64, P],
    "lcv_master_sgd_step_g32": [P, P, I64, I64, P, F64, F64, P],
    "lcv_master_adamw_step_g32": [P, P, I64, I64, P, F64, F64, F64, F64, F64, I64, P],
}

_SIGNATURES_ANCHOR = {
    "lcv_master_sgd_step_anchor": [P, P, P, I64, I64, P, F64, F64, I, P],
    "lcv_master_adamw_step_anchor": [P, P, P, I64, I64, P, F64, F64, F64, F64, F64, I64, I, P],
    "lcv_master_adamw8_step_anchor": [P, P, P, P, I64, I64, P, F64, F64, F64, F64, F64, I64, P],
    "lcv_master_drift_sumsq": [P, P, P, I64, I64, P, I64, P, P],
}

_SIGNATURES_EMA = {
    "lcv_master_ema_load": [P, P, P, I64, I64, P],
    "lcv_master_ema_update": [P, P, P, I64, I64, F64, P],
    "lcv_master_ema_swap": [P, P, P, I64, I64, P],
}

_SIGNATURES_STEPCACHE = {
    "lcv_stepcache_diff": [P, P, P, P, I64, I64, F32, P, I64, P, P],
    "lcv_stepcache_store": [P, P, P, I64, P],
    "lcv_stepcache_apply": [P, P, P, I64, P],
}

_SIGNATURES_SOLVER = {
    "lcv_cfg_lms_step": [P, P, P, P, P, P, P, I64, I64, F32, F32, F32, F32, I, I, I, P],
}

_SIGNATURES_CFGREUSE = {
    "lcv_cfg_delta_store": [P, P, P, P, P, I64, I64, F32, I, P],
    "lcv_cfg_delta_apply": [P, P, P, I64, I64, P],
}

_SIGNATURES_APG = {
    "lcv_cfg_apg": [P, P, P, P, P, P, I64, I64, F32, F32, F32, F32, I, I, P],
}

_SIGNATURES_SR = {
    "lcv_sr_sgd_step": [P, I64, I64, P, F64, F64, U64, U64, P],
    "lcv_sr_adamw_step": [P, I64, I64, P, F64, F64, F64, F64, F64, I64, U64, U64, P],
    "lcv_sr_round": [P, P, I64, U64, U64, P],
}

LCV_EPI_NONE, LCV_EPI_SWIGLU, LCV_EPI_GATE_RESIDUAL, LCV_EPI_GELU_TANH, LCV_EPI_SILU = 0, 1, 2, 3, 4


class LcvError(RuntimeError):
    code = None

    @property
    def fatal(self) -> bool:
        return self.code in (-2, -3)


_lib = None


def lib_path() -> Path:
    return _LIB_PATH


def load():
    global _lib
    if _lib is not None:
        return _lib
    if not _LIB_PATH.exists():
        raise LcvError(
            f"{_LIB_PATH} is missing: build it with `python __graft_entry__.py` (hipcc, gfx950). "
            "There is no fallback path.")
    import torch
    lib = ctypes.CDLL(str(_LIB_PATH), mode=os.RTLD_NOW | getattr(os, "RTLD_LOCAL", 0))
    lib.lcv_version.restype = c_int
    lib.lcv_version.argtypes = []
    lib.lcv_last_error.restype = c_char_p
# ... 56 lines not shown
```

### longcat-video-tta_amd/lcv_hip/ops.py

```python
import os
from typing import Optional, Tuple

import torch

from . import lib as _lib
from .lib import (LCV_EPI_GATE_RESIDUAL, LCV_EPI_GELU_TANH, LCV_EPI_NONE, LCV_EPI_SILU, LCV_EPI_SWIGLU,
                  call)

BF16 = torch.bfloat16
F32 = torch.float32
PROFILE = None
PROFILE_BWD = None


_DETERMINISTIC = os.environ.get("LCV_DETERMINISTIC", "") == "1"


def set_deterministic(flag: bool) -> None:
    global _DETERMINISTIC
    _DETERMINISTIC = bool(flag)


def is_deterministic() -> bool:
    return _DETERMINISTIC


def _det_ws(kind: int, device, d0: int, d1: int = 0, d2: int = 0):
    n = int(_lib.load().lcv_det_ws_bytes(kind, d0, d1, d2))
    if n < 0:
        raise _lib.LcvError(f"lcv_det_ws_bytes: unknown kind {kind}")
    return torch.empty((max(n, 16) // 4,), dtype=F32, device=device), n


def _ptr(t: Optional[torch.Tensor]):
    return None if t is None else t.data_ptr()


def _stream():
    return torch.cuda.current_stream().cuda_stream


def _req(t: torch.Tensor, dtype, name: str):
    if not t.is_cuda:
        raise _lib.LcvError(f"{name}: tensor must live on the GPU (no CPU path exists)")
    if t.dtype != dtype:
        raise _lib.LcvError(f"{name}: expected {dtype}, got {t.dtype}")


def adaln_modulate(x: torch.Tensor, mod: torch.Tensor, shift_idx: int, scale_idx: int, T: int,
                   eps: float = 1e-6) -> torch.Tensor:
    _req(x, BF16, "adaln_modulate.x"); _req(mod, F32, "adaln_modulate.mod")
    B, N, C = x.shape
    x = x.contiguous(); mod = mod.contiguous()
    y = torch.empty_like(x)
    call("lcv_adaln_modulate_fwd", _ptr(x), _ptr(mod), _ptr(y), B, T, N // T, C, mod.shape[-1],
         shift_idx * C, scale_idx * C, eps, _stream())
    return y


def layernorm_affine(x: torch.Tensor, w: torch.Tensor, b: torch.Tensor, eps: float = 1e-6) -> torch.Tensor:
    _req(x, BF16, "layernorm_affine.x")
    C = x.shape[-1]
    x = x.contiguous()
    wf = w.detach().to(F32).contiguous(); bf = b.detach().to(F32).contiguous()
    y = torch.empty_like(x)
    call("lcv_layernorm_affine_fwd", _ptr(x), _ptr(wf), _ptr(bf), _ptr(y), x.numel() // C, C, eps, _stream())
    return y


def gate_residual(x: torch.Tensor, y: torch.Tensor, mod: Optional[torch.Tensor], gate_idx: int, T: int) -> torch.Tensor:
    _req(x, BF16, "gate_residual.x"); _req(y, BF16, "gate_residual.y")
    B, N, C = x.shape
    x = x.contiguous(); y = y.contiguous()
    out = torch.empty_like(x)
    if mod is not None:
        _req(mod, F32, "gate_residual.mod")
        mod = mod.contiguous()
        call("lcv_gate_residual_fwd", _ptr(x), _ptr(y), _ptr(mod), _ptr(out), B, T, N // T, C, mod.shape[-1],
             gate_idx * C, _stream())
    else:
        call("lcv_gate_residual_fwd", _ptr(x), _ptr(y), None, _ptr(out), B, 1, N, C, 0, 0, _stream())
    return out


def timestep_embedding(t: torch.Tensor, dim: int, max_period: float = 10000.0) -> torch.Tensor:
    _req(t, F32, "timestep_embedding.t")
    t = t.contiguous().view(-1)
    out = torch.empty((t.numel(), dim), dtype=F32, device=t.device)
    call("lcv_timestep_embedding", _ptr(t), _ptr(out), t.numel(), dim, float(max_period), _stream())
    return out


def qknorm_rope(q_in: Optional[torch.Tensor], k_in: Optional[torch.Tensor], v_in: Optional[torch.Tensor],
                q_out: Optional[torch.Tensor], k_out: Optional[torch.Tensor], v_out: Optional[torch.Tensor],
                wq: torch.Tensor, wk: torch.Tensor, cs: Optional[torch.Tensor], pos_off: int = 0,
                eps: float = 1e-6, q_scale: float = 1.0) -> None:
    ref = q_in if q_in is not None else k_in
    B, N, H, D = ref.shape
    if D != 128:
        raise _lib.LcvError("qknorm_rope: head_dim must be 128")

    def chk(t, name):
        if t is None:
            return
        _req(t, BF16, name)
        if t.stride(3) != 1 or t.stride(2) != D:
            raise _lib.LcvError(f"{name}: (H, D) must be contiguous")

    for t, nme in ((q_in, "q_in"), (k_in, "k_in"), (v_in, "v_in"), (q_out, "q_out"), (k_out, "k_out"), (v_out, "v_out")):
        chk(t, "qknorm_rope." + nme)
    ins = [t for t in (q_in, k_in, v_in) if t is not None]
    if any(t.stride(0) != ins[0].stride(0) or t.stride(1) != ins[0].stride(1) for t in ins):
        raise _lib.LcvError("qknorm_rope: q_in/k_in/v_in must share strides")
    kvs = [t for t in (k_out, v_out) if t is not None]
    if kvs and any(t.stride(0) != kvs[0].stride(0) or t.stride(1) != kvs[0].stride(1) for t in kvs):
        raise _lib.LcvError("qknorm_rope: k_out/v_out must share strides")
    if cs is not None:
        _req(cs, F32, "qknorm_rope.cs")
        if cs.shape[0] < pos_off + N:
            raise _lib.LcvError("qknorm_rope: cos/sin table shorter than pos_off + N")
    qo = q_out if q_out is not None else ref
    ko = kvs[0] if kvs else ref
    call("lcv_qknorm_rope_fwd", _ptr(q_in), _ptr(k_in), _ptr(v_in), _ptr(q_out), _ptr(k_out), _ptr(v_out),
         _ptr(wq), _ptr(wk), _ptr(cs), B, N, H, ins[0].stride(0), ins[0].stride(1), qo.stride(0), qo.stride(1),
         ko.stride(0), ko.stride(1), pos_off, eps, q_scale, _stream())


LOG2E = 1.4426950408889634
LN2 = 0.6931471805599453


def log2_qscale(scale: float) -> float:
    return scale * LOG2E


def attention(q: torch.Tensor, k: torch.Tensor, v: torch.Tensor, scale: float,
              out: Optional[torch.Tensor] = None, need_lse: bool = False) -> Tuple[torch.Tensor, Optional[torch.Tensor]]:
    for t, nme in ((q, "q"), (k, "k"), (v, "v")):
        _req(t, BF16, "attention." + nme)
        if t.shape[-1] != 128 or t.stride(-1) != 1:
            raise _lib.LcvError("attention: head_dim must be 128 and contiguous")
    B, Nq, H, D = q.shape
    Nk = k.shape[1]
    if out is None:
        out = torch.empty((B, Nq, H, D), dtype=BF16, device=q.device)
    lse = torch.empty((B, H, Nq), dtype=F32, device=q.device) if need_lse else None
    if PROFILE is not None:
        ev0 = torch.cuda.Event(enable_timing=True); ev1 = torch.cuda.Event(enable_timing=True)
        ev0.record()
    call("lcv_attn_fwd", _ptr(q), _ptr(k), _ptr(v), _ptr(out), _ptr(lse), B, H, Nq, Nk,
         q.stride(0), q.stride(1), q.stride(2), k.stride(0), k.stride(1), k.stride(2),
         v.stride(0), v.stride(1), v.stride(2), out.stride(0), out.stride(1), out.stride(2),
         float(scale), _stream())
    if PROFILE is not None:
        ev1.record()
        PROFILE.append((ev0, ev1, 4.0 * B * H * Nq * Nk * D, Nq, Nk, _lib.load().lcv_attn_fwd_last_kernel().decode()))
    return out, lse


_GEMM_WS = {}
GEMM_WS_BYTES = 256 << 20


def _ensure_gemm_workspace(device: torch.device) -> None:
    idx = device.index if device.index is not None else torch.cuda.current_device()
    if idx not in _GEMM_WS:
        if _GEMM_WS:
            raise _lib.LcvError(
                f"gemm_nt on cuda:{idx}, but this process already bound the library's split-K workspace to cuda:"
                f"{next(iter(_GEMM_WS))}: the build runs one process per GPU (torch.distributed), a second device in the "
                "same process would write its partial sums into the first device's memory")
        ws = torch.empty(GEMM_WS_BYTES, dtype=torch.uint8, device=device)
        call("lcv_gemm_set_workspace", _ptr(ws), GEMM_WS_BYTES)
        _GEMM_WS[idx] = ws


PARAM_EPOCH = 0


def gemm_nt(a: torch.Tensor, w: torch.Tensor, bias: Optional[torch.Tensor] = None, *,
            a2: Optional[torch.Tensor] = None, w2: Optional[torch.Tensor] = None,
            epilogue: int = LCV_EPI_NONE, out_f32: bool = False, resid: Optional[torch.Tensor] = None,
            mod: Optional[torch.Tensor] = None, gate_idx: int = 0, rows_per_frame: int = 1,
            out: Optional[torch.Tensor] = None, swiglu_aux: Optional[torch.Tensor] = None) -> torch.Tensor:
    _req(a, BF16, "gemm_nt.a"); _req(w, BF16, "gemm_nt.w")
    if a.shape[0] >= 2048:
        _ensure_gemm_workspace(a.device)
    if a.dim() != 2 or w.dim() != 2 or a.stride(1) != 1 or w.stride(1) != 1:
        raise _lib.LcvError("gemm_nt: a and w must be 2-D with contiguous rows")
    M, K = a.shape
    N = w.shape[0]
    if w.shape[1] != K:
        raise _lib.LcvError(f"gemm_nt: K mismatch ({K} vs {w.shape[1]})")
    if K % 64:
        pad = 64 - K % 64
        a = torch.nn.functional.pad(a, (0, pad))
        w = torch.nn.functional.pad(w, (0, pad))
        K += pad
    K2 = 0
    if a2 is not None:
        _req(a2, BF16, "gemm_nt.a2"); _req(w2, BF16, "gemm_nt.w2")
        K2 = a2.shape[1]
    n_out = N // 2 if epilogue == LCV_EPI_SWIGLU else N
    if out is None:
        out = torch.empty((M, n_out), dtype=F32 if out_f32 else BF16, device=a.device)
    if bias is not None:
        _req(bias, BF16, "gemm_nt.bias")
    if swiglu_aux is not None:
        _req(swiglu_aux, BF16, "gemm_nt.swiglu_aux")
        if epilogue != LCV_EPI_SWIGLU or resid is not None or swiglu_aux.shape != (M, N) or not swiglu_aux.is_contiguous():
            raise _lib.LcvError("gemm_nt: swiglu_aux needs the SwiGLU epilogue and a contiguous [M, N] tensor")
        resid = swiglu_aux
    C = N
    mod_stride = 0
    if mod is not None:
        _req(mod, F32, "gemm_nt.mod")
        mod_stride = mod.shape[-1]
    call("lcv_gemm_nt", _ptr(a), _ptr(w), _ptr(bias), _ptr(a2), _ptr(w2), _ptr(out), M, N, K, K2,
         a.stride(0), w.stride(0), a2.stride(0) if a2 is not None else 0, w2.stride(0) if w2 is not None else 0,
         out.stride(0), epilogue, 1 if out_f32 else 0, _ptr(resid), _ptr(mod), rows_per_frame, mod_stride,
         gate_idx * C, _stream())
    return out


def linear_f32_smallm(a: torch.Tensor, w: torch.Tensor, bias: Optional[torch.Tensor], act_in: int = 0) -> torch.Tensor:
    _req(a, F32, "linear_f32_smallm.a"); _req(w, BF16, "linear_f32_smallm.w")
    a = a.contiguous()
    M, K = a.shape
    N = w.shape[0]
    out = torch.empty((M, N), dtype=F32, device=a.device)
    call("lcv_linear_f32_smallm", _ptr(a), _ptr(w.contiguous()), _ptr(bias), _ptr(out), M, N, K, act_in, _stream())
    return out


def _lora_down(name: str, x: torch.Tensor, A: torch.Tensor, s: float, rpad: int, draw=()) -> torch.Tensor:
    M, K = x.shape
    h = torch.empty((M, rpad), dtype=BF16, device=x.device)
    call(name, _ptr(x), _ptr(A.contiguous()), _ptr(h), M, K, A.shape[0], rpad, x.stride(0), float(s), *draw, _stream())
    return h


def lora_down(x: torch.Tensor, A: torch.Tensor, s: float, rpad: int = 64) -> torch.Tensor:
    _req(x, BF16, "lora_down.x"); _req(A, BF16, "lora_down.A")
    return _lora_down("lcv_lora_down", x, A, s, rpad)


_U64 = (1 << 64) - 1


def draw_philox_offset(device: torch.device) -> Tuple[int, int]:
    index = device.index if device.index is not None else torch.cuda.current_device()
    gen = torch.cuda.default_generators[index]
    seed, offset = gen.initial_seed(), gen.get_offset()
    gen.set_offset(offset + 4)
    return seed, offset


def sr_round(x: torch.Tensor, seed: int, offset: int, out: Optional[torch.Tensor] = None) -> torch.Tensor:
    _req(x, F32, "sr_round.x")
    if not x.is_contiguous():
        raise _lib.LcvError("sr_round: x must be contiguous")
    out = torch.empty(x.shape, dtype=BF16, device=x.device) if out is None else out
    _req(out, BF16, "sr_round.out")
    if out.numel() != x.numel() or not out.is_contiguous():
        raise _lib.LcvError("sr_round: out must be contiguous with x's element count")
    if x.numel():
        call("lcv_sr_round", _ptr(x), _ptr(out), x.numel(), int(seed) & _U64, int(offset) & _U64, _stream())
    return out


def _draw(p: float, seed: int, offset: int, row0: int) -> tuple:
    return float(p), int(seed) & _U64, int(offset) & _U64, int(row0)


def lora_down_dropout(x: torch.Tensor, A: torch.Tensor, s: float, p: float, seed: int, offset: int, rpad: int = 64,
                      row0: int = 0) -> torch.Tensor:
    _req(x, BF16, "lora_down_dropout.x"); _req(A, BF16, "lora_down_dropout.A")
    if x.dim() != 2 or x.stride(1) != 1:
        raise _lib.LcvError("lora_down_dropout: x must be 2-D with contiguous rows")
    return _lora_down("lcv_lora_down_dropout", x, A, s, rpad, _draw(p, seed, offset, row0))


def tn_skinny_dropout(g: torch.Tensor, x: torch.Tensor, R: int, p: float, seed: int, offset: int, scale: float = 1.0,
                      row0: int = 0) -> torch.Tensor:
    _req(g, BF16, "tn_skinny_dropout.g"); _req(x, BF16, "tn_skinny_dropout.x")
    if x.dim() != 2 or x.stride(1) != 1 or not g.is_contiguous():
        raise _lib.LcvError("tn_skinny_dropout: x must be 2-D with contiguous rows, g contiguous")
    return _tn_skinny("lcv_tn_skinny_dropout", g, x, R, scale, _draw(p, seed, offset, row0))


def lora_dx_dropout_add(dx: torch.Tensor, g: torch.Tensor, A: torch.Tensor, p: float, seed: int, offset: int,
                        row0: int = 0) -> torch.Tensor:
    _req(dx, BF16, "lora_dx_dropout_add.dx"); _req(g, BF16, "lora_dx_dropout_add.g"); _req(A, BF16, "lora_dx_dropout_add.A")
    if dx.dim() != 2 or not dx.is_contiguous() or g.dim() != 2 or g.stride(1) != 1:
        raise _lib.LcvError("lora_dx_dropout_add: dx must be 2-D contiguous, g 2-D with contiguous rows")
    M, K = dx.shape
    R = A.shape[0]
    call("lcv_lora_dx_dropout_add", _ptr(dx), _ptr(g), _ptr(A.contiguous()), M, K, R, g.shape[1], g.stride(0),
         *_draw(p, seed, offset, row0), _stream())
    return dx


def lora_dropout_mask(M: int, K: int, p: float, seed: int, offset: int, row0: int = 0, device="cuda") -> torch.Tensor:
    out = torch.empty((M, K), dtype=torch.uint8, device=device)
    _req(out, torch.uint8, "lora_dropout_mask.out")
    call("lcv_lora_dropout_mask", _ptr(out), M, K, *_draw(p, seed, offset, row0), _stream())
# ... 690 lines not shown
```

### longcat-video-tta_amd/longcat_video/modules/layers.py

```python
from typing import Optional, Tuple

import torch
import torch.nn as nn

from lcv_hip import autograd_ops as A
from lcv_hip import ops

BF16 = torch.bfloat16


def is_pristine(m: nn.Module, cls) -> bool:
    return (type(m) is cls and "forward" not in m.__dict__ and not m._forward_hooks
            and not m._forward_pre_hooks and not m._backward_hooks and not getattr(m, "_backward_pre_hooks", {}))


class HipLinear(nn.Linear):

    def reset_parameters(self) -> None:
        pass

    def forward(self, x: torch.Tensor) -> torch.Tensor:
        shp = x.shape
        y = A.linear(x.reshape(-1, shp[-1]), self.weight, self.bias)
        return y.view(*shp[:-1], self.out_features)


def _proj_out(proj: "HipLinear", o: torch.Tensor, fuse) -> torch.Tensor:
    if fuse is None:
        return proj(o)
    from lcv_hip.lib import LCV_EPI_GATE_RESIDUAL
    resid, mod, gate_idx, T = fuse
    B, N, C = resid.shape
    out = ops.gemm_nt(o.reshape(B * N, -1), proj.weight, proj.bias, epilogue=LCV_EPI_GATE_RESIDUAL,
                      resid=resid.reshape(B * N, C), mod=mod, gate_idx=gate_idx, rows_per_frame=max(N // T, 1))
    return out.view(B, N, C)


class LayerNorm_FP32(nn.LayerNorm):

    def forward(self, x: torch.Tensor) -> torch.Tensor:
        if self.weight is None:
            raise RuntimeError("the non-affine mod_norm_* layers are fused into adaln_modulate")
        return A.layernorm_affine(x, self.weight, self.bias, self.eps)


class RMSNorm_FP32(nn.Module):

    def __init__(self, dim: int, eps: float = 1e-6, device=None, dtype=None):
        super().__init__()
        self.eps = eps
        self.weight = nn.Parameter(torch.ones(dim, device=device, dtype=dtype))


class AdaLNModulation(nn.Sequential):

    def __init__(self, tembed_dim: int, out_dim: int, device=None, dtype=None):
        super().__init__(nn.SiLU(), HipLinear(tembed_dim, out_dim, bias=True, device=device, dtype=dtype))

    def forward(self, t: torch.Tensor) -> torch.Tensor:
        lin = self[1]
        shp = t.shape
        y = A.linear_f32(t.reshape(-1, shp[-1]).float(), lin.weight, lin.bias, act_in=1)
        return y.view(*shp[:-1], lin.out_features)


class RotaryPositionalEmbedding(nn.Module):

    def __init__(self, head_dim: int, cp_split_hw=None):
        super().__init__()
        assert head_dim % 8 == 0
        self.head_dim = head_dim
        self.base = 10000.0
        self.cp_split_hw = cp_split_hw
        self._tables = {}

    def table(self, grid: Tuple[int, int, int], device) -> torch.Tensor:
        key = (tuple(int(g) for g in grid), str(device))
        tab = self._tables.get(key)
        if tab is None:
            T, H, W = key[0]
            D = self.head_dim
            dim_t = D - 4 * (D // 6)
            dim_h = dim_w = 2 * (D // 6)

            def axis(n, dim):
                freqs = 1.0 / (self.base ** (torch.arange(0, dim, 2)[: dim // 2].float() / dim))
                return torch.outer(torch.arange(n, dtype=torch.float32), freqs)

            ft, fh, fw = axis(T, dim_t), axis(H, dim_h), axis(W, dim_w)
            ang = torch.cat([
                ft[:, None, None, :].expand(T, H, W, dim_t // 2),
                fh[None, :, None, :].expand(T, H, W, dim_h // 2),
                fw[None, None, :, :].expand(T, H, W, dim_w // 2),
            ], dim=-1).reshape(T * H * W, D // 2)
            tab = torch.stack([ang.cos(), ang.sin()], dim=-1).contiguous().to(device)
            self._tables[key] = tab
        return tab


class Attention(nn.Module):

    def __init__(self, dim: int, num_heads: int, cp_split_hw=None, device=None, dtype=None):
        super().__init__()
        self.dim, self.num_heads = dim, num_heads
        self.head_dim = dim // num_heads
        self.scale = self.head_dim ** -0.5
        self.qkv = HipLinear(dim, dim * 3, bias=True, device=device, dtype=dtype)
        self.q_norm = RMSNorm_FP32(self.head_dim, eps=1e-6, device=device, dtype=dtype)
        self.k_norm = RMSNorm_FP32(self.head_dim, eps=1e-6, device=device, dtype=dtype)
        self.proj = HipLinear(dim, dim, bias=True, device=device, dtype=dtype)
        self.rope_3d = RotaryPositionalEmbedding(self.head_dim, cp_split_hw=cp_split_hw)

    def forward(self, x, shape=None, num_cond_latents=None, return_kv=False, fuse_residual=None):
        B, N, C = x.shape
        H, D = self.num_heads, self.head_dim
        qkv = self.qkv(x).view(B, N, 3, H, D)
        sp = getattr(self, "_sp", None)
        if sp is not None:
            return self._forward_sequence_parallel(qkv, shape, num_cond_latents, sp, fuse_residual)
        cs = self.rope_3d.table(shape, x.device)
        n_cond = 0
        if num_cond_latents is not None and num_cond_latents > 0:
            n_cond = num_cond_latents * (N // shape[0])
        o, kv = A.self_attention(qkv, self.q_norm.weight, self.k_norm.weight, cs, self.scale, n_cond,
                                 self.q_norm.eps, return_kv)
        out = _proj_out(self.proj, o.view(B, N, C), fuse_residual)
        if return_kv:
            return out, kv
        return out

    def _forward_sequence_parallel(self, qkv, shape, num_cond_latents, sp, fuse_residual=None):
        B, N, _, H, D = qkv.shape
        cs = self.rope_3d.table(sp.grid, qkv.device)
        n_loc = int(num_cond_latents or 0) * sp.S
        n_glob = int(getattr(sp, "num_cond_frames", 0)) * sp.tokens_per_frame
        o = A.sp_self_attention(qkv, self.q_norm.weight, self.k_norm.weight, cs, self.scale, self.q_norm.eps, sp, n_loc, n_glob)
        return _proj_out(self.proj, o.view(B, N, H * D), fuse_residual)

    def forward_with_kv_cache(self, x, shape=None, num_cond_latents=None, kv_cache=None, fuse_residual=None):
        B, N, C = x.shape
        H, D = self.num_heads, self.head_dim
        qkv = self.qkv(x).view(B, N, 3, H, D)
        k_c, v_c = kv_cache
        n_c = k_c.shape[1]
        sp = getattr(self, "_sp", None)
        if sp is not None:
            t_c = n_c // sp.tokens_per_frame
            cs = self.rope_3d.table((sp.num_frames + t_c, sp.rows_per_frame, sp.S), x.device)
            q, k, v = qkv[:, :, 0], qkv[:, :, 1], qkv[:, :, 2]
            ops.qknorm_rope(q, k, None, q, k, None, self.q_norm.weight, self.k_norm.weight, cs, n_c + sp.token_offset,
                            self.q_norm.eps, q_scale=ops.log2_qscale(self.scale))
            k_full, v_full = sp.all_gather_kv(k.contiguous(), v.contiguous())
            ex = (lambda t: t if t.shape[0] == B else t.expand(B, -1, -1, -1))
            o, _ = ops.attention(q, torch.cat([ex(k_c), k_full], dim=1), torch.cat([ex(v_c), v_full], dim=1), ops.LN2)
            return _proj_out(self.proj, o.view(B, N, C), fuse_residual)
        T, Hh, Ww = shape
        t_c = n_c // (Hh * Ww)
        cs = self.rope_3d.table((T + t_c, Hh, Ww), x.device)
        o = A.cached_attention(qkv, k_c, v_c, self.q_norm.weight, self.k_norm.weight, cs, self.scale,
                               self.q_norm.eps)
        return _proj_out(self.proj, o.view(B, N, C), fuse_residual)


class MultiHeadCrossAttention(nn.Module):

    def __init__(self, dim: int, num_heads: int, device=None, dtype=None):
        super().__init__()
        self.dim, self.num_heads = dim, num_heads
        self.head_dim = dim // num_heads
        self.scale = self.head_dim ** -0.5
        self.q_linear = HipLinear(dim, dim, bias=True, device=device, dtype=dtype)
        self.kv_linear = HipLinear(dim, dim * 2, bias=True, device=device, dtype=dtype)
        self.proj = HipLinear(dim, dim, bias=True, device=device, dtype=dtype)
        self.q_norm = RMSNorm_FP32(self.head_dim, eps=1e-6, device=device, dtype=dtype)
        self.k_norm = RMSNorm_FP32(self.head_dim, eps=1e-6, device=device, dtype=dtype)

    def _process_cross_attn(self, x, cond, kv_seqlen, fuse_residual=None):
        B, N, C = x.shape
        H, D = self.num_heads, self.head_dim
        q = self.q_linear(x).view(B, N, H, D)
        kv = self.kv_linear(cond).view(1, -1, 2, H, D)
        o = A.cross_attention(q, kv, self.q_norm.weight, self.k_norm.weight, list(kv_seqlen), self.scale,
                              self.q_norm.eps)
        return _proj_out(self.proj, o.view(B, N, C), fuse_residual)

    def forward(self, x, cond, kv_seqlen, num_cond_latents=None, shape=None, fuse_residual=None):
        if num_cond_latents is None or num_cond_latents == 0:
            return self._process_cross_attn(x, cond, kv_seqlen, fuse_residual)
        if fuse_residual is not None:
            raise ValueError("fuse_residual is only offered without conditioning tokens")
        B, N, C = x.shape
        assert shape is not None, "SHOULD pass in the shape"
        n_cond = num_cond_latents * (N // shape[0])
        out_noise = self._process_cross_attn(x[:, n_cond:], cond, kv_seqlen)
        return A.pad_front_zero(out_noise, n_cond)


class FeedForwardSwiGLU(nn.Module):
    def __init__(self, dim: int, hidden_dim: int, multiple_of: int = 256, device=None, dtype=None):
        super().__init__()
        hidden_dim = int(2 * hidden_dim / 3)
        hidden_dim = multiple_of * ((hidden_dim + multiple_of - 1) // multiple_of)
        self.dim, self.hidden_dim = dim, hidden_dim
        self.w1 = HipLinear(dim, hidden_dim, bias=False, device=device, dtype=dtype)
        self.w2 = HipLinear(hidden_dim, dim, bias=False, device=device, dtype=dtype)
        self.w3 = HipLinear(dim, hidden_dim, bias=False, device=device, dtype=dtype)
        self._w13 = None
        self._w13_key = None

    def fused_w13(self) -> Optional[torch.Tensor]:
        if not (is_pristine(self.w1, HipLinear) and is_pristine(self.w3, HipLinear)):
            return None
        if self.hidden_dim % 32:
            return None
        epoch = ops.PARAM_EPOCH if (self.w1.weight.requires_grad or self.w3.weight.requires_grad) else -1
        key = (self.w1.weight.data_ptr(), self.w3.weight.data_ptr(), self.w1.weight._version, self.w3.weight._version, epoch)
        if self._w13 is None or self._w13_key != key:
            F_, K = self.w1.weight.shape
            with torch.no_grad():
                self._w13 = torch.stack([self.w1.weight.view(F_ // 32, 32, K), self.w3.weight.view(F_ // 32, 32, K)],
                                        dim=1).reshape(2 * F_, K).contiguous()
            self._w13_key = key
        return self._w13

    def forward(self, x, fuse_residual=None):
        shp = x.shape
        x2 = x.reshape(-1, shp[-1])
        pristine = is_pristine(self.w1, HipLinear) and is_pristine(self.w3, HipLinear)
        trainable = pristine and (self.w1.weight.requires_grad or self.w3.weight.requires_grad)
        w13 = None if (not pristine or (torch.is_grad_enabled() and trainable)) else self.fused_w13()
        if w13 is not None:
            h = A.swiglu_fused(x2, w13)
        else:
            h = A.swiglu(self.w1(x2), self.w3(x2))
        if fuse_residual is not None:
            return _proj_out(self.w2, h.view(*shp[:-1], -1), fuse_residual)
        return self.w2(h).view(*shp[:-1], self.dim)


class PatchEmbed3D(nn.Module):
    def __init__(self, patch_size, in_chans, embed_dim, device=None, dtype=None):
        super().__init__()
        self.patch_size = tuple(patch_size)
        if self.patch_size != (1, 2, 2):
            raise NotImplementedError("the HIP patchify kernel is written for patch (1, 2, 2)")
        self.proj = nn.Conv3d(in_chans, embed_dim, kernel_size=self.patch_size, stride=self.patch_size,
                              device=device, dtype=dtype)

    def forward(self, x):
        return A.patch_embed(x, self.proj.weight, self.proj.bias)


class TimestepEmbedder(nn.Module):

    def __init__(self, t_embed_dim: int, frequency_embedding_size: int = 256, device=None, dtype=None):
        super().__init__()
        self.frequency_embedding_size = frequency_embedding_size
        self.mlp = nn.Sequential(
            HipLinear(frequency_embedding_size, t_embed_dim, bias=True, device=device, dtype=dtype),
            nn.SiLU(),
            HipLinear(t_embed_dim, t_embed_dim, bias=True, device=device, dtype=dtype),
        )

    @staticmethod
    def timestep_embedding(t, dim, max_period=10000):
        return ops.timestep_embedding(t.float(), dim, float(max_period))

    def forward(self, t, dtype=torch.float32):
        t_freq = self.timestep_embedding(t, self.frequency_embedding_size)
        h = A.linear_f32(t_freq, self.mlp[0].weight, self.mlp[0].bias, act_in=0)
        return A.linear_f32(h, self.mlp[2].weight, self.mlp[2].bias, act_in=1)


class CaptionEmbedder(nn.Module):
    def __init__(self, in_channels: int, hidden_size: int, device=None, dtype=None):
        super().__init__()
        self.y_proj = nn.Sequential(
            HipLinear(in_channels, hidden_size, bias=True, device=device, dtype=dtype),
            nn.GELU(approximate="tanh"),
            HipLinear(hidden_size, hidden_size, bias=True, device=device, dtype=dtype),
        )

    def forward(self, caption):
        shp = caption.shape
        x = caption.reshape(-1, shp[-1])
        if torch.is_grad_enabled() and any(p.requires_grad for p in self.y_proj.parameters()):
            h = A.gelu_tanh(A.linear(x, self.y_proj[0].weight, self.y_proj[0].bias))
        else:
            h = A.linear(x, self.y_proj[0].weight, self.y_proj[0].bias, epilogue="gelu_tanh")
        y = A.linear(h, self.y_proj[2].weight, self.y_proj[2].bias)
        return y.view(*shp[:-1], y.shape[-1])


class FinalLayer_FP32(nn.Module):
    def __init__(self, hidden_size, num_patch, out_channels, adaln_tembed_dim, device=None, dtype=None):
        super().__init__()
        self.norm_final = nn.LayerNorm(hidden_size, elementwise_affine=False, eps=1e-6)
        self.linear = HipLinear(hidden_size, num_patch * out_channels, bias=True, device=device, dtype=dtype)
        self.adaLN_modulation = AdaLNModulation(adaln_tembed_dim, 2 * hidden_size, device=device, dtype=dtype)

    def forward(self, x, t, latent_shape):
        T = latent_shape[0]
        mod = self.adaLN_modulation(t)
        xm = A.adaln_modulate(x, mod, 0, 1, T, self.norm_final.eps)
        B, N, C = xm.shape
        y = A.linear(xm.view(B * N, C), self.linear.weight, self.linear.bias, out_f32=True)
        return y.view(B, N, -1)


class LongCatSingleStreamBlock(nn.Module):
    def __init__(self, hidden_size, num_heads, mlp_ratio, adaln_tembed_dim, cp_split_hw=None, device=None,
                 dtype=None):
        super().__init__()
        self.hidden_size = hidden_size
        kw = dict(device=device, dtype=dtype)
        self.adaLN_modulation = AdaLNModulation(adaln_tembed_dim, 6 * hidden_size, **kw)
        self.mod_norm_attn = LayerNorm_FP32(hidden_size, eps=1e-6, elementwise_affine=False)
        self.mod_norm_ffn = LayerNorm_FP32(hidden_size, eps=1e-6, elementwise_affine=False)
        self.pre_crs_attn_norm = LayerNorm_FP32(hidden_size, eps=1e-6, elementwise_affine=True, **kw)
        self.attn = Attention(hidden_size, num_heads, cp_split_hw=cp_split_hw, **kw)
        self.cross_attn = MultiHeadCrossAttention(hidden_size, num_heads, **kw)
        self.ffn = FeedForwardSwiGLU(hidden_size, int(hidden_size * mlp_ratio), **kw)

    def forward(self, x, y, t, y_seqlen, latent_shape, num_cond_latents=None, return_kv=False, kv_cache=None,
                skip_crs_attn=False):
        T = latent_shape[0]
        mod = self.adaLN_modulation(t)
        x_m, x = A.adaln_modulate_fork(x, mod, 0, 1, T, self.mod_norm_attn.eps)
        kv = None
        nograd = not torch.is_grad_enabled()
        fa = (x, mod, 2, T) if (nograd and is_pristine(self.attn, Attention) and is_pristine(self.attn.proj, HipLinear)) else None
        akw = {} if fa is None else {"fuse_residual": fa}
        if kv_cache is not None:
            x_s = self.attn.forward_with_kv_cache(x_m, shape=latent_shape, num_cond_latents=num_cond_latents,
                                                  kv_cache=kv_cache, **akw)
        elif return_kv:
# ... 24 lines not shown
```

Before: 0.06161 latent frames/s.

## Fuse Q RMSNorm and RoPE into attention load; varlen cross-attn; cache rownorm modulation

Applies the Q RMSNorm, RoPE and log2 scale inside the attention forward kernels as Q is loaded, so the separate qknorm pass no longer reads and writes Q. Cross-attention gets a per-batch kv_ranges table, letting one launch serve packed variable-length keys up to 512. The adaLN row-norm kernel now handles runs of rows per block and stages the shift/scale vectors in shared memory instead of re-reading them from global for every row. In exchange the attention kernels carry extra register pressure and loads for the norm, and the pipe kernel path does not support the fusion.

```diff
diff --git a/include/lcv_hip.h b/include/lcv_hip.h
--- a/include/lcv_hip.h
+++ b/include/lcv_hip.h
@@ -69,7 +69,9 @@
                  int64_t k_sb, int64_t k_sn, int64_t k_sh,
                  int64_t v_sb, int64_t v_sn, int64_t v_sh,
                  int64_t o_sb, int64_t o_sn, int64_t o_sh,
-                 float scale, void* stream);
+                 float scale,
+                 const void* q_norm_w, const float* rope_cs, int64_t rope_token_offset, float eps, float q_scale,
+                 const int32_t* kv_ranges, int64_t kv_rows, void* stream);
 const char* lcv_attn_fwd_last_kernel(void);
 int64_t lcv_attn_bwd_ws_floats(int64_t B, int64_t H, int64_t Nq, int64_t Nk);
 int lcv_attn_bwd(const void* q, const void* k, const void* v, const void* o,
diff --git a/longcat-video-tta_amd/csrc/attn_common.h b/longcat-video-tta_amd/csrc/attn_common.h
--- a/longcat-video-tta_amd/csrc/attn_common.h
+++ b/longcat-video-tta_amd/csrc/attn_common.h
@@ -57,6 +57,12 @@
   return g;
 }
 
+struct AttnQNorm {
+  const bf16_t* w;
+  const float* rope_cs;
+  int64_t rope_token_offset;
+  float eps, q_scale;
+};
 struct AttnArgs {
   const void *q, *k, *v;
   void* o;
@@ -69,6 +75,7 @@
   int64_t dq_sb, dq_sn, dq_sh, dk_sb, dk_sn, dk_sh, dv_sb, dv_sn, dv_sh;
   float scale;
   int accumulate_kv;
+  AttnQNorm qn;
 };
 struct AttnDims {
   int64_t Nq, Nk;
@@ -85,9 +92,75 @@
   bf16_t* o;
   float* lse;
   AttnDims d;
+  AttnQNorm qn;
 };
 static inline AttnFwdLead attn_fwd_lead(const AttnArgs& a) {
-  return {(const bf16_t*)a.q, (const bf16_t*)a.k, (const bf16_t*)a.v, (bf16_t*)a.o, a.lse, attn_dims(a)};
+  return {(const bf16_t*)a.q, (const bf16_t*)a.k, (const bf16_t*)a.v, (bf16_t*)a.o, a.lse, attn_dims(a), a.qn};
+}
+
+struct AttnQNormHalf { u16x8 w[4]; f32x4 cs[4][2]; };
+__device__ __forceinline__ void attn_qn_request(AttnQNormHalf& b, const AttnQNorm& n, int64_t token, int half, int h) {
+  const float* csrow = n.rope_cs + (n.rope_token_offset + token) * 128;
+#pragma unroll
+  for (int j = 0; j < 4; ++j) {
+    const int g = 2 * (4 * half + j) + h;
+    b.w[j] = *reinterpret_cast<const u16x8*>(n.w + 8 * g);
+    if (n.rope_cs) {
+      b.cs[j][0] = *reinterpret_cast<const f32x4*>(csrow + 8 * g);
+      b.cs[j][1] = *reinterpret_cast<const f32x4*>(csrow + 8 * g + 4);
+    }
+  }
+  SCHED_FENCE();
+}
+__device__ __forceinline__ float attn_qn_rstd(const bf16x8 (&q)[8], const AttnQNorm& n) {
+  float ss[8];
+#pragma unroll
+  for (int ks = 0; ks < 8; ++ks) {
+    float f[8];
+    unpack8(__builtin_bit_cast(u16x8, q[ks]), f);
+    ss[ks] = qknorm_ss8(f);
+  }
+  const float t8a = ss[0] + ss[4], t8b = ss[1] + ss[5], t8c = ss[2] + ss[6], t8d = ss[3] + ss[7];
+  const float t4a = t8a + t8c, t4b = t8b + t8d;
+  return qknorm_rstd(half_sum(t4a + t4b), n.eps);
+}
+__device__ __forceinline__ void attn_qn_apply(bf16x8 (&q)[8], const AttnQNormHalf& b, float r, const AttnQNorm& n, int half) {
+  const bool do_rope = n.rope_cs != nullptr;
+#pragma unroll
+  for (int j = 0; j < 4; ++j) {
+    float f[8], w[8];
+    float cs[8] = {1, 0, 1, 0, 1, 0, 1, 0};
+    unpack8(__builtin_bit_cast(u16x8, q[4 * half + j]), f);
+    unpack8(b.w[j], w);
+    if (do_rope) {
+      const f32x4 a = b.cs[j][0], c = b.cs[j][1];
+      cs[0] = a[0]; cs[1] = a[1]; cs[2] = a[2]; cs[3] = a[3];
+      cs[4] = c[0]; cs[5] = c[1]; cs[6] = c[2]; cs[7] = c[3];
+    }
+    q[4 * half + j] = __builtin_bit_cast(bf16x8, qknorm_rope_out8(f, r, w, cs, do_rope, n.q_scale));
+  }
+  SCHED_FENCE();
+}
+__device__ __forceinline__ void attn_q_norm_on_load(bf16x8 (&q)[8], const AttnQNorm& n, int64_t token, int h) {
+  AttnQNormHalf b0, b1;
+  attn_qn_request(b0, n, token, 0, h);
+  const float r = attn_qn_rstd(q, n);
+  attn_qn_request(b1, n, token, 1, h);
+  attn_qn_apply(q, b0, r, n, 0);
+  attn_qn_apply(q, b1, r, n, 1);
+}
+__device__ __forceinline__ void attn_q_norm_on_load(bf16x8 (&qa)[8], bf16x8 (&qb)[8], const AttnQNorm& n, int64_t token_a,
+                                                    int64_t token_b, int h) {
+  AttnQNormHalf b0, b1;
+  attn_qn_request(b0, n, token_a, 0, h);
+  const float ra = attn_qn_rstd(qa, n), rb = attn_qn_rstd(qb, n);
+  attn_qn_request(b1, n, token_a, 1, h);
+  attn_qn_apply(qa, b0, ra, n, 0);
+  attn_qn_request(b0, n, token_b, 0, h);
+  attn_qn_apply(qa, b1, ra, n, 1);
+  attn_qn_request(b1, n, token_b, 1, h);
+  attn_qn_apply(qb, b0, rb, n, 0);
+  attn_qn_apply(qb, b1, rb, n, 1);
 }
 
 static inline bool attn_raise_lds(const void* kern, size_t bytes) {
diff --git a/longcat-video-tta_amd/csrc/attn_fwd.hip b/longcat-video-tta_amd/csrc/attn_fwd.hip
--- a/longcat-video-tta_amd/csrc/attn_fwd.hip
+++ b/longcat-video-tta_amd/csrc/attn_fwd.hip
@@ -4,6 +4,8 @@
 struct AttnFwdParams : AttnFwdLead {
   float scale, scale_log2e;
   int gx, xcd_remap;
+  const int* kv_ranges;
+  int64_t kv_rows;
 };
 
 template <int NWAVES, int PRIO, bool XATTN, int VAR>
@@ -27,8 +29,17 @@
   ATTN_BLOCK_DECODE(p, qb, head, b);
   const int64_t q0 = (int64_t)qb * QROWS + wave * 32;
 
-  const bf16_t* kbase = p.k + b * p.d.k_sb + (int64_t)head * p.d.k_sh;
-  const bf16_t* vbase = p.v + b * p.d.v_sb + (int64_t)head * p.d.v_sh;
+  int64_t Nk = p.d.Nk, kv0 = 0;
+  if (p.kv_ranges) {
+    int64_t off = p.kv_ranges[2 * b], len = p.kv_ranges[2 * b + 1];
+    off = off < 0 ? 0 : (off > p.kv_rows - 1 ? p.kv_rows - 1 : off);
+    const int64_t room = p.kv_rows - off < Nk ? p.kv_rows - off : Nk;
+    len = len < 1 ? 1 : (len > room ? room : len);
+    kv0 = off;
+    Nk = len;
+  }
+  const bf16_t* kbase = p.k + b * p.d.k_sb + kv0 * p.d.k_sn + (int64_t)head * p.d.k_sh;
+  const bf16_t* vbase = p.v + b * p.d.v_sb + kv0 * p.d.v_sn + (int64_t)head * p.d.v_sh;
 
   bf16x8 qf[8];
   {
@@ -37,6 +48,7 @@
     const bf16_t* qp = p.q + b * p.d.q_sb + qrow * p.d.q_sn + (int64_t)head * p.d.q_sh + 8 * h;
 #pragma unroll
     for (int ks = 0; ks < 8; ++ks) qf[ks] = *reinterpret_cast<const bf16x8*>(qp + 16 * ks);
+    if (p.qn.w) attn_q_norm_on_load(qf, p.qn, qrow, h);
   }
 
   int st_off[NCH];
@@ -65,7 +77,7 @@
     lds_u8* dst = lds + buf * 2 * TILE_BYTES + which * TILE_BYTES + wave * 2048;
     const bf16_t** src = which ? vdma : kdma;
     const int64_t sn = which ? p.d.v_sn : p.d.k_sn;
-    if (FULL || (int64_t)t * 64 + 64 <= p.d.Nk) {
+    if (FULL || (int64_t)t * 64 + 64 <= Nk) {
 #pragma unroll
       for (int i = 0; i < 2; ++i) {
         __builtin_amdgcn_global_load_lds((gbl_void_t*)src[i], (lds_void_t*)(dst + 1024 * i), 16, 0, 0);
@@ -74,7 +86,7 @@
     } else {
 #pragma unroll
       for (int i = 0; i < 2; ++i) {
-        int64_t back = (int64_t)t * 64 + dma_row[i] - (p.d.Nk - 1);
+        int64_t back = (int64_t)t * 64 + dma_row[i] - (Nk - 1);
         if (back < 0) back = 0;
         __builtin_amdgcn_global_load_lds((gbl_void_t*)(src[i] - back * sn), (lds_void_t*)(dst + 1024 * i), 16, 0, 0);
       }
@@ -90,7 +102,7 @@
 #pragma unroll
     for (int i = 0; i < NCH; ++i) {
       int64_t row = kv0 + st_row[i];
-      if (row > p.d.Nk - 1) row = p.d.Nk - 1;
+      if (row > Nk - 1) row = Nk - 1;
       kreg[i] = *reinterpret_cast<const u32x4*>(kbase + row * p.d.k_sn + st_col);
       vreg[i] = *reinterpret_cast<const u32x4*>(vbase + row * p.d.v_sn + st_col);
     }
@@ -126,7 +138,7 @@
   float l_run = 0.f;
 
   if (PRIO == 1 && wave >= NWAVES / 2) __builtin_amdgcn_s_setprio(1);
-  const int nt = (int)((p.d.Nk + 63) / 64);
+  const int nt = (int)((Nk + 63) / 64);
   {
     if (DMA) {
       dma_tile(0, 0, std::false_type{});
@@ -160,8 +172,8 @@
       s1 = __builtin_amdgcn_mfma_f32_32x32x16_bf16(a1, qf[ks], s1, 0, 0, 0);
     }
 
-    if (!has_next && (p.d.Nk & 63)) {
-      const int valid = (int)(p.d.Nk - (int64_t)t * 64);
+    if (!has_next && (Nk & 63)) {
+      const int valid = (int)(Nk - (int64_t)t * 64);
 #pragma unroll
       for (int e = 0; e < 16; ++e) {
         const int key = (e & 3) + 8 * (e >> 2) + 4 * h;
@@ -297,7 +309,8 @@
                             int64_t H, int64_t Nq, int64_t Nk, int64_t q_sb, int64_t q_sn, int64_t q_sh,
                             int64_t k_sb, int64_t k_sn, int64_t k_sh, int64_t v_sb, int64_t v_sn,
                             int64_t v_sh, int64_t o_sb, int64_t o_sn, int64_t o_sh, float scale,
-                            void* stream) {
+                            const void* q_norm_w, const float* rope_cs, int64_t rope_token_offset, float eps,
+                            float q_scale, const int32_t* kv_ranges, int64_t kv_rows, void* stream) {
   LCV_CHECK_ARG(q && k && v && o, "attn_fwd: null pointer");
   LCV_CHECK_ARG(B > 0 && H > 0 && H <= 65535 && B <= 65535, "attn_fwd: bad B/H");
   LCV_CHECK_ARG(Nk > 0, "attn_fwd: Nk must be > 0 (empty key set has no softmax)");
@@ -307,8 +320,13 @@
   LCV_CHECK_ARG(o_sn % 4 == 0 && o_sh % 4 == 0 && o_sb % 4 == 0, "attn_fwd: o strides must be multiples of 4 elements");
   LCV_CHECK_ARG(((uintptr_t)q % 16 == 0) && ((uintptr_t)k % 16 == 0) && ((uintptr_t)v % 16 == 0) && ((uintptr_t)o % 8 == 0),
                 "attn_fwd: pointers must be 16-byte aligned");
+  LCV_CHECK_ARG(q_norm_w || !rope_cs, "attn_fwd: rope_cs needs q_norm_w (RoPE on load comes with the q norm)");
+  LCV_CHECK_ARG(!q_norm_w || (q_scale > 0.f && rope_token_offset >= 0 && (uintptr_t)q_norm_w % 16 == 0 && (uintptr_t)rope_cs % 16 == 0),
+                "attn_fwd: q norm on load needs q_scale > 0, rope_token_offset >= 0 and 16-byte aligned q_norm_w / rope_cs");
+  LCV_CHECK_ARG(!kv_ranges || (Nk <= 512 && kv_rows > 0), "attn_fwd: kv_ranges serves the short-key body only (Nk <= 512) and needs kv_rows > 0");
   if (Nq == 0) return LCV_OK;
   AttnArgs a = {};
+  a.qn = {(const bf16_t*)q_norm_w, q_norm_w ? rope_cs : nullptr, rope_token_offset, eps, q_scale};
   a.q = q; a.k = k; a.v = v; a.o = o; a.lse = lse; a.B = B; a.H = H; a.Nq = Nq; a.Nk = Nk; a.scale = scale;
   a.q_sb = q_sb; a.q_sn = q_sn; a.q_sh = q_sh; a.k_sb = k_sb; a.k_sn = k_sn; a.k_sh = k_sh;
   a.v_sb = v_sb; a.v_sn = v_sn; a.v_sh = v_sh; a.o_sb = o_sb; a.o_sn = o_sn; a.o_sh = o_sh;
@@ -317,7 +335,7 @@
   const char* xe = lcv_knob("LCV_ATTN_XCD");
   const bool xcd_ok = !(xe && xe[0] == '0');
   const AttnGrid g = attn_grid(B, H, (Nq + NW * 32 - 1) / (NW * 32), xcd_ok);
-  const AttnFwdParams p = {attn_fwd_lead(a), scale, scale * 1.4426950408889634f, g.gx, g.xcd_remap};
+  const AttnFwdParams p = {attn_fwd_lead(a), scale, scale * 1.4426950408889634f, g.gx, g.xcd_remap, (const int*)kv_ranges, kv_rows};
   auto launch = [&](auto kern) -> int {
     if (!attn_raise_lds((const void*)kern, lds)) {
       lcv_set_error("attn_fwd: cannot raise dynamic LDS");
@@ -335,6 +353,8 @@
     g_last_attn_kernel = "attn_fwd_w64_kernel";
     return attn_fwd_w64_launch(a, xcd_ok, (hipStream_t)stream);
   }
+  LCV_CHECK_ARG(!(unit && Nk > 512 && span32 && q_norm_w),
+                "attn_fwd: q norm on load is not built into attn_fwd_pipe_kernel (LCV_ATTN_FWD_W64=0): norm q with lcv_qknorm_rope_fwd");
   if (unit && Nk > 512 && span32) {
     g_last_attn_kernel = "attn_fwd_pipe_kernel";
     return attn_fwd_pipe_launch(a, xcd_ok, (hipStream_t)stream);
diff --git a/longcat-video-tta_amd/csrc/attn_fwd_w64.hip b/longcat-video-tta_amd/csrc/attn_fwd_w64.hip
--- a/longcat-video-tta_amd/csrc/attn_fwd_w64.hip
+++ b/longcat-video-tta_amd/csrc/attn_fwd_w64.hip
@@ -252,6 +252,15 @@
 #pragma unroll
     for (int ks = 0; ks < 8; ++ks) qf[nb][ks] = *reinterpret_cast<const bf16x8*>(qp + 16 * ks);
   }
+  if (p.qn.w) {
+    bf16x8 ta[8], tb[8];
+#pragma unroll
+    for (int ks = 0; ks < 8; ++ks) { ta[ks] = qf[0][ks]; tb[ks] = qf[1][ks]; }
+    const int64_t last = p.d.Nq - 1;
+    attn_q_norm_on_load(ta, tb, p.qn, (q0 + r > last) ? last : q0 + r, (q0 + 32 + r > last) ? last : q0 + 32 + r, h);
+#pragma unroll
+    for (int ks = 0; ks < 8; ++ks) { qf[0][ks] = ta[ks]; qf[1][ks] = tb[ks]; }
+  }
 #pragma unroll
   for (int nb = 0; nb < 2; ++nb)
 #pragma unroll
diff --git a/longcat-video-tta_amd/csrc/elementwise.hip b/longcat-video-tta_amd/csrc/elementwise.hip
--- a/longcat-video-tta_amd/csrc/elementwise.hip
+++ b/longcat-video-tta_amd/csrc/elementwise.hip
@@ -2,71 +2,99 @@
 #include "cfg_guidance.h"
 
 #define ROWNORM_MAXCH 8
+#define ROWNORM_RUN 8
 
 template <int MODE>
 __global__ __launch_bounds__(256) void rownorm_fwd_kernel(
     const bf16_t* __restrict__ x, const float* __restrict__ p_add, const float* __restrict__ p_mul,
-    bf16_t* __restrict__ y, int64_t rows, int C, int64_t S, int64_t mod_stride, float eps) {
+    bf16_t* __restrict__ y, int C, int64_t S, int64_t mod_stride, float eps, int run, int64_t runs_per_frame) {
+  __shared__ __attribute__((aligned(16))) float s_add[ROWNORM_MAXCH * 512], s_mul[ROWNORM_MAXCH * 512];
   const int lane = threadIdx.x & 63;
-  const int64_t row = (int64_t)blockIdx.x * 4 + (threadIdx.x >> 6);
-  if (row >= rows) return;
-  const bf16_t* xr = x + row * C;
-  float v[ROWNORM_MAXCH][8];
-  float sum = 0.f;
-#pragma unroll
-  for (int ch = 0; ch < ROWNORM_MAXCH; ++ch) {
-    const int c = (ch * 64 + lane) * 8;
-    if (c < C) {
-      u16x8 raw = *reinterpret_cast<const u16x8*>(xr + c);
-      unpack8(raw, v[ch]);
-#pragma unroll
-      for (int i = 0; i < 8; ++i) sum += v[ch][i];
-    } else {
-#pragma unroll
-      for (int i = 0; i < 8; ++i) v[ch][i] = 0.f;
-    }
-  }
-  const float mean = wave_sum(sum) / (float)C;
-  float sq = 0.f;
-#pragma unroll
-  for (int ch = 0; ch < ROWNORM_MAXCH; ++ch) {
-    const int c = (ch * 64 + lane) * 8;
-    if (c < C) {
-#pragma unroll
-      for (int i = 0; i < 8; ++i) {
-        const float d = v[ch][i] - mean;
-        sq += d * d;
+  const int64_t frame = (int64_t)blockIdx.x / runs_per_frame;
+  const int64_t first = ((int64_t)blockIdx.x - frame * runs_per_frame) * (4 * run);
+  const int n_rows = (int)((S - first < 4 * run) ? S - first : 4 * run);
+  {
+    const float* pa = p_add;
+    const float* pm = p_mul;
+    if (MODE == 0) {
+      pa += frame * mod_stride;
+      pm += frame * mod_stride;
+    }
+    for (int c = threadIdx.x * 4; c < C; c += 1024) {
+      *reinterpret_cast<f32x4*>(s_add + c) = *reinterpret_cast<const f32x4*>(pa + c);
+      *reinterpret_cast<f32x4*>(s_mul + c) = *reinterpret_cast<const f32x4*>(pm + c);
+    }
+  }
+  __syncthreads();
+  for (int ri = threadIdx.x >> 6; ri < n_rows; ri += 4) {
+    const int64_t row = frame * S + first + ri;
+    const bf16_t* xr = x + row * C;
+    float v[ROWNORM_MAXCH][8];
+    float sum = 0.f;
+#pragma unroll
+    for (int ch = 0; ch < ROWNORM_MAXCH; ++ch) {
+      const int c = (ch * 64 + lane) * 8;
+      if (c < C) {
+        u16x8 raw = *reinterpret_cast<const u16x8*>(xr + c);
+        unpack8(raw, v[ch]);
+#pragma unroll
+        for (int i = 0; i < 8; ++i) sum += v[ch][i];
+      } else {
+#pragma unroll
+        for (int i = 0; i < 8; ++i) v[ch][i] = 0.f;
       }
     }
-  }
-  const float rstd = rsqrtf(wave_sum(sq) / (float)C + eps);
-  const float* pa = p_add;
-  const float* pm = p_mul;
-  if (MODE == 0) {
-    const int64_t frame = row / S;
-    pa += frame * mod_stride;
-    pm += frame * mod_stride;
-  }
-  bf16_t* yr = y + row * C;
-#pragma unroll
-  for (int ch = 0; ch < ROWNORM_MAXCH; ++ch) {
-    const int c = (ch * 64 + lane) * 8;
-    if (c < C) {
-      const f32x4 a0 = *reinterpret_cast<const f32x4*>(pa + c);
-      const f32x4 a1 = *reinterpret_cast<const f32x4*>(pa + c + 4);
-      const f32x4 m0 = *reinterpret_cast<const f32x4*>(pm + c);
-      const f32x4 m1 = *reinterpret_cast<const f32x4*>(pm + c + 4);
-      float o[8];
-#pragma unroll
-      for (int i = 0; i < 8; ++i) {
-        const float xh = (v[ch][i] - mean) * rstd;
-        const float mul = (i < 4) ? m0[i] : m1[i - 4];
-        const float add = (i < 4) ? a0[i] : a1[i - 4];
-        o[i] = (MODE == 0) ? (xh * (mul + 1.0f) + add) : (xh * mul + add);
+    const float mean = wave_sum(sum) / (float)C;
+    float sq = 0.f;
+#pragma unroll
+    for (int ch = 0; ch < ROWNORM_MAXCH; ++ch) {
+      const int c = (ch * 64 + lane) * 8;
+      if (c < C) {
+#pragma unroll
+        for (int i = 0; i < 8; ++i) {
+          const float d = v[ch][i] - mean;
+          sq += d * d;
+        }
       }
-      *reinterpret_cast<u16x8*>(yr + c) = pack8(o);
-    }
-  }
+    }
+    const float rstd = rsqrtf(wave_sum(sq) / (float)C + eps);
+    bf16_t* yr = y + row * C;
+#pragma unroll
+    for (int ch = 0; ch < ROWNORM_MAXCH; ++ch) {
+      const int c = (ch * 64 + lane) * 8;
+      if (c < C) {
+        const f32x4 a0 = *reinterpret_cast<const f32x4*>(s_add + c);
+        const f32x4 a1 = *reinterpret_cast<const f32x4*>(s_add + c + 4);
+        const f32x4 m0 = *reinterpret_cast<const f32x4*>(s_mul + c);
+        const f32x4 m1 = *reinterpret_cast<const f32x4*>(s_mul + c + 4);
+        float o[8];
+#pragma unroll
+        for (int i = 0; i < 8; ++i) {
+          const float xh = (v[ch][i] - mean) * rstd;
+          const float mul = (i < 4) ? m0[i] : m1[i - 4];
+          const float add = (i < 4) ? a0[i] : a1[i - 4];
+          o[i] = (MODE == 0) ? (xh * (mul + 1.0f) + add) : (xh * mul + add);
+        }
+        *reinterpret_cast<u16x8*>(yr + c) = pack8(o);
+      }
+    }
+  }
+}
+
+static int rownorm_run() {
+  const char* e = lcv_knob("LCV_ROWNORM_RUN");
+  const int v = e ? atoi(e) : 0;
+  return (v >= 1 && v <= 256) ? v : ROWNORM_RUN;
+}
+template <int MODE>
+static int rownorm_launch(const char* name, const void* x, const float* p_add, const float* p_mul, void* y, int64_t frames,
+                          int64_t S, int64_t C, int64_t mod_stride, float eps, void* stream) {
+  const int run = rownorm_run();
+  const int64_t runs_per_frame = (S + 4 * run - 1) / (4 * run);
+  LCV_CHECK_ARG(frames * runs_per_frame <= 0x7fffffffll, "%s: too many rows for one grid", name);
+  hipLaunchKernelGGL(rownorm_fwd_kernel<MODE>, dim3((unsigned)(frames * runs_per_frame)), dim3(256), 0, (hipStream_t)stream,
+                     (const bf16_t*)x, p_add, p_mul, (bf16_t*)y, (int)C, S, mod_stride, eps, run, runs_per_frame);
+  return LCV_OK;
 }
 
 extern "C" int lcv_adaln_modulate_fwd(const void* x, const float* mod, void* y, int64_t B, int64_t T,
@@ -76,11 +104,8 @@
   LCV_CHECK_ARG(C > 0 && C % 8 == 0 && C <= 4096, "adaln_modulate_fwd: C=%ld must be a multiple of 8 and <= 4096", (long)C);
   LCV_CHECK_ARG(B > 0 && T > 0 && S > 0, "adaln_modulate_fwd: bad sizes");
   LCV_CHECK_ARG(shift_off % 4 == 0 && scale_off % 4 == 0 && mod_stride % 4 == 0, "adaln_modulate_fwd: offsets must be 16-byte aligned");
-  const int64_t rows = B * T * S;
-  const unsigned grid = (unsigned)((rows + 3) / 4);
-  hipLaunchKernelGGL(rownorm_fwd_kernel<0>, dim3(grid), dim3(256), 0, (hipStream_t)stream,
-                     (const bf16_t*)x, mod + shift_off, mod + scale_off, (bf16_t*)y, rows, (int)C, S,
-                     mod_stride, eps);
+  const int rc = rownorm_launch<0>("adaln_modulate_fwd", x, mod + shift_off, mod + scale_off, y, B * T, S, C, mod_stride, eps, stream);
+  if (rc != LCV_OK) return rc;
   LCV_LAUNCH_CHECK("adaln_modulate_fwd");
   return LCV_OK;
 }
@@ -90,9 +115,8 @@
   LCV_CHECK_ARG(x && w && b && y, "layernorm_affine_fwd: null pointer");
   LCV_CHECK_ARG(C > 0 && C % 8 == 0 && C <= 4096, "layernorm_affine_fwd: C=%ld must be a multiple of 8 and <= 4096", (long)C);
   if (rows == 0) return LCV_OK;
-  const unsigned grid = (unsigned)((rows + 3) / 4);
-  hipLaunchKernelGGL(rownorm_fwd_kernel<1>, dim3(grid), dim3(256), 0, (hipStream_t)stream,
-                     (const bf16_t*)x, b, w, (bf16_t*)y, rows, (int)C, (int64_t)1, (int64_t)0, eps);
+  const int rc = rownorm_launch<1>("layernorm_affine_fwd", x, b, w, y, 1, rows, C, 0, eps, stream);
+  if (rc != LCV_OK) return rc;
   LCV_LAUNCH_CHECK("layernorm_affine_fwd");
   return LCV_OK;
 }
@@ -142,32 +166,13 @@
                                               const float (&cs)[8], bool do_rope, float eps, float out_scale) {
   float f[8];
   unpack8(*reinterpret_cast<const u16x8*>(src), f);
-  float ss = 0.f;
-#pragma unroll
-  for (int i = 0; i < 8; ++i) ss += f[i] * f[i];
+  float ss = qknorm_ss8(f);
   ss += __shfl_xor(ss, 8, 64);
   ss += __shfl_xor(ss, 4, 64);
   ss += __shfl_xor(ss, 2, 64);
   ss += __shfl_xor(ss, 1, 64);
-  const float r = rsqrtf(ss * (1.0f / 128.0f) + eps);
-  float o[8];
-#pragma unroll
-  for (int i = 0; i < 8; ++i) f[i] = bfround(bfround(f[i] * r) * w[i]);
-  if (do_rope) {
-#pragma unroll
-    for (int i = 0; i < 4; ++i) {
-      const float c = cs[2 * i], s = cs[2 * i + 1];
-      const float x0 = f[2 * i], x1 = f[2 * i + 1];
-      o[2 * i] = __fadd_rn(__fmul_rn(x0, c), __fmul_rn(-x1, s));
-      o[2 * i + 1] = __fadd_rn(__fmul_rn(x1, c), __fmul_rn(x0, s));
-    }
-  } else {
-#pragma unroll
-    for (int i = 0; i < 8; ++i) o[i] = f[i];
-  }
-#pragma unroll
-  for (int i = 0; i < 8; ++i) o[i] *= out_scale;
-  *reinterpret_cast<u16x8*>(dst) = pack8(o);
+  const float r = qknorm_rstd(ss, eps);
+  *reinterpret_cast<u16x8*>(dst) = qknorm_rope_out8(f, r, w, cs, do_rope, out_scale);
 }
 
 __global__ __launch_bounds__(256) void qknorm_rope_fwd_kernel(
diff --git a/longcat-video-tta_amd/csrc/lcv_common.h b/longcat-video-tta_amd/csrc/lcv_common.h
--- a/longcat-video-tta_amd/csrc/lcv_common.h
+++ b/longcat-video-tta_amd/csrc/lcv_common.h
@@ -71,6 +71,35 @@
 
 __device__ __forceinline__ float silu_f(float x) { return x / (1.0f + __expf(-x)); }
 
+__device__ __forceinline__ float qknorm_ss8(const float (&f)[8]) {
+  float ss = 0.f;
+#pragma unroll
+  for (int i = 0; i < 8; ++i) ss += f[i] * f[i];
+  return ss;
+}
+__device__ __forceinline__ float qknorm_rstd(float ss, float eps) { return rsqrtf(ss * (1.0f / 128.0f) + eps); }
+__device__ __forceinline__ u16x8 qknorm_rope_out8(float (&f)[8], float r, const float (&w)[8], const float (&cs)[8],
+                                                  bool do_rope, float out_scale) {
+  float o[8];
+#pragma unroll
+  for (int i = 0; i < 8; ++i) f[i] = bfround(bfround(f[i] * r) * w[i]);
+  if (do_rope) {
+#pragma unroll
+    for (int i = 0; i < 4; ++i) {
+      const float c = cs[2 * i], s = cs[2 * i + 1];
+      const float x0 = f[2 * i], x1 = f[2 * i + 1];
+      o[2 * i] = __fadd_rn(__fmul_rn(x0, c), __fmul_rn(-x1, s));
+      o[2 * i + 1] = __fadd_rn(__fmul_rn(x1, c), __fmul_rn(x0, s));
+    }
+  } else {
+#pragma unroll
+    for (int i = 0; i < 8; ++i) o[i] = f[i];
+  }
+#pragma unroll
+  for (int i = 0; i < 8; ++i) o[i] *= out_scale;
+  return pack8(o);
+}
+
 __device__ __forceinline__ void lcv_lds_dma16(const void* gsrc, unsigned lds_dst) {
   unsigned keep;
   asm volatile("s_mov_b32 %0, m0\n\ts_mov_b32 m0, %2\n\ts_nop 0\n\tglobal_load_lds_dwordx4 %1, off\n\ts_mov_b32 m0, %0"
diff --git a/longcat-video-tta_amd/csrc/lib.hip b/longcat-video-tta_amd/csrc/lib.hip
--- a/longcat-video-tta_amd/csrc/lib.hip
+++ b/longcat-video-tta_amd/csrc/lib.hip
@@ -42,6 +42,7 @@
     {"LCV_ATTN_FWD_W64"}, {"LCV_ATTN_XCD"},
     {"LCV_ATTN_BWD_VAR"}, {"LCV_ATTN_BWD_DKV_WAVES"}, {"LCV_ATTN_BWD_DQ_WAVES"}, {"LCV_ATTN_BWD_PIPE"}, {"LCV_ATTN_BWD_STAGGER"},
     {"LCV_ATTN_BWD_XCD"},
+    {"LCV_ROWNORM_RUN"},
 };
 std::mutex g_knob_mutex;
 bool g_knobs_read = false;
diff --git a/longcat-video-tta_amd/lcv_hip/autograd_ops.py b/longcat-video-tta_amd/lcv_hip/autograd_ops.py
--- a/longcat-video-tta_amd/lcv_hip/autograd_ops.py
+++ b/longcat-video-tta_amd/lcv_hip/autograd_ops.py
@@ -1,3 +1,4 @@
+import os
 import weakref
 from typing import List, Optional
 
@@ -273,18 +274,20 @@
     return out
 
 
-def _attend_regions(q, k, v, scale, n_cond, need_lse):
+def _attend_regions(q, k, v, scale, n_cond, need_lse, q_norm=None):
     B, N, H, D = q.shape
     o = torch.empty((B, N, H, D), dtype=BF16, device=q.device)
     lses = []
+    kw = (lambda first: {}) if q_norm is None else (
+        lambda first: {"q_norm": ops.QNorm(q_norm.w, q_norm.cs, q_norm.pos_off + first, q_norm.eps, q_norm.q_scale)})
     if n_cond > 0:
-        _, l1 = ops.attention(q[:, :n_cond], k[:, :n_cond], v[:, :n_cond], scale, out=o[:, :n_cond], need_lse=need_lse)
+        _, l1 = ops.attention(q[:, :n_cond], k[:, :n_cond], v[:, :n_cond], scale, out=o[:, :n_cond], need_lse=need_lse, **kw(0))
         lses.append(l1)
         if N > n_cond:
-            _, l2 = ops.attention(q[:, n_cond:], k, v, scale, out=o[:, n_cond:], need_lse=need_lse)
+            _, l2 = ops.attention(q[:, n_cond:], k, v, scale, out=o[:, n_cond:], need_lse=need_lse, **kw(n_cond))
             lses.append(l2)
     else:
-        _, l1 = ops.attention(q, k, v, scale, out=o, need_lse=need_lse)
+        _, l1 = ops.attention(q, k, v, scale, out=o, need_lse=need_lse, **kw(0))
         lses.append(l1)
     return o, lses
 
@@ -327,12 +330,16 @@
                 dwk.to(wk.dtype) if (want_dw and wk.requires_grad) else None, None, None, None, None)
 
 
-def self_attention(qkv, wq, wk, cs, scale, n_cond, eps, return_kv=False):
+def self_attention(qkv, wq, wk, cs, scale, n_cond, eps, return_kv=False, fuse_q_norm=False):
     if _needs_grad(qkv, wq, wk):
         if return_kv:
             raise LcvError("self_attention: return_kv is an inference-only path")
         return _SelfAttentionFn.apply(qkv, wq, wk, cs, scale, n_cond, eps), None
     q, k, v = qkv[:, :, 0], qkv[:, :, 1], qkv[:, :, 2]
+    if fuse_q_norm and not return_kv and os.environ.get("LCV_ATTN_FWD_W64", "")[:1] != "0":
+        ops.qknorm_rope(None, k, None, None, k, None, wq, wk, cs, 0, eps)
+        o, _ = _attend_regions(q, k, v, ops.LN2, n_cond, False, ops.QNorm(wq, cs, 0, eps, ops.log2_qscale(scale)))
+        return o, None
     ops.qknorm_rope(q, k, None, q, k, None, wq, wk, cs, 0, eps, q_scale=ops.log2_qscale(scale))
     o, _ = _attend_regions(q, k, v, ops.LN2, n_cond, False)
     kv = (k.contiguous(), v.contiguous()) if return_kv else None
@@ -508,11 +515,17 @@
                 dwk.to(wk.dtype) if (want_dw and wk.requires_grad) else None, None, None, None)
 
 
-def cross_attention(q, kv, wq, wk, seqlens: List[int], scale, eps):
+def cross_attention(q, kv, wq, wk, seqlens: List[int], scale, eps, fuse_q_norm=False):
     if _needs_grad(q, kv, wq, wk):
         return _CrossAttentionFn.apply(q, kv, wq, wk, seqlens, scale, eps)
     B, N, H, D = q.shape
     k, v = kv[:, :, 0], kv[:, :, 1]
+    lens = [int(n) for n in list(seqlens)[:B]]
+    if fuse_q_norm and len(lens) == B and max(lens) <= 512:
+        ops.qknorm_rope(None, k, None, None, k, None, wq, wk, None, 0, eps)
+        o, _ = ops.attention(q, k, v, scale, q_norm=ops.QNorm(wq, None, 0, eps, 1.0),
+                             kv_ranges=ops.kv_ranges(lens, kv.shape[1], q.device), max_keys=max(lens))
+        return o
     ops.qknorm_rope(q, None, None, q, None, None, wq, wk, None, 0, eps)
     ops.qknorm_rope(None, k, None, None, k, None, wq, wk, None, 0, eps)
     o = torch.empty_like(q)
diff --git a/longcat-video-tta_amd/lcv_hip/lib.py b/longcat-video-tta_amd/lcv_hip/lib.py
--- a/longcat-video-tta_amd/lcv_hip/lib.py
+++ b/longcat-video-tta_amd/lcv_hip/lib.py
@@ -17,7 +17,7 @@
     "lcv_gate_residual_bwd": [P, P, P, P, P, I64, I64, I64, I64, I64, I64, P],
     "lcv_qknorm_rope_fwd": [P, P, P, P, P, P, P, P, P, I64, I64, I64, I64, I64, I64, I64, I64, I64, I64, F32, F32, P],
     "lcv_qknorm_rope_bwd": [P, P, P, P, P, P, P, P, P, I64, I64, I64, I64, I64, I64, I64, I64, I64, I64, I64, I64, F32, F32, P, P, I64, P],
-    "lcv_attn_fwd": [P, P, P, P, P, I64, I64, I64, I64] + [I64] * 12 + [F32, P],
+    "lcv_attn_fwd": [P, P, P, P, P, I64, I64, I64, I64] + [I64] * 12 + [F32, P, P, I64, F32, F32, P, I64, P],
     "lcv_attn_bwd": [P, P, P, P, P, P, P, P, P, P, I, I64, I64, I64, I64] + [I64] * 21 + [F32, P],
     "lcv_gemm_nt": [P, P, P, P, P, P, I64, I64, I64, I64, I64, I64, I64, I64, I64, I, I, P, P, I64, I64, I64, P],
     "lcv_gemm_set_workspace": [P, I64],
diff --git a/longcat-video-tta_amd/lcv_hip/ops.py b/longcat-video-tta_amd/lcv_hip/ops.py
--- a/longcat-video-tta_amd/lcv_hip/ops.py
+++ b/longcat-video-tta_amd/lcv_hip/ops.py
@@ -134,14 +134,57 @@
     return scale * LOG2E
 
 
+class QNorm:
+    __slots__ = ("w", "cs", "pos_off", "eps", "q_scale")
+
+    def __init__(self, w: torch.Tensor, cs: Optional[torch.Tensor] = None, pos_off: int = 0, eps: float = 1e-6,
+                 q_scale: float = 1.0):
+        self.w, self.cs, self.pos_off, self.eps, self.q_scale = w, cs, int(pos_off), float(eps), float(q_scale)
+
+
+_KV_RANGES = {}
+
+
+def kv_ranges(seqlens, total: int, device) -> torch.Tensor:
+    lens = tuple(int(n) for n in seqlens)
+    if not lens or min(lens) < 1 or sum(lens) > total:
+        raise _lib.LcvError(f"kv_ranges: lengths {lens} must be positive and fit the {total} packed rows")
+    key = (str(device), lens)
+    tab = _KV_RANGES.get(key)
+    if tab is None:
+        if len(_KV_RANGES) >= 64:
+            _KV_RANGES.clear()
+        offs = [sum(lens[:i]) for i in range(len(lens))]
+        tab = torch.tensor([[o, n] for o, n in zip(offs, lens)], dtype=torch.int32).to(device)
+        _KV_RANGES[key] = tab
+    return tab
+
+
 def attention(q: torch.Tensor, k: torch.Tensor, v: torch.Tensor, scale: float,
-              out: Optional[torch.Tensor] = None, need_lse: bool = False) -> Tuple[torch.Tensor, Optional[torch.Tensor]]:
+              out: Optional[torch.Tensor] = None, need_lse: bool = False, q_norm: Optional[QNorm] = None,
+              kv_ranges: Optional[torch.Tensor] = None, max_keys: int = 0) -> Tuple[torch.Tensor, Optional[torch.Tensor]]:
     for t, nme in ((q, "q"), (k, "k"), (v, "v")):
         _req(t, BF16, "attention." + nme)
         if t.shape[-1] != 128 or t.stride(-1) != 1:
             raise _lib.LcvError("attention: head_dim must be 128 and contiguous")
     B, Nq, H, D = q.shape
     Nk = k.shape[1]
+    k_sb, v_sb, kv_rows = k.stride(0), v.stride(0), 0
+    if kv_ranges is not None:
+        if k.shape[0] != 1 or v.shape[0] != 1 or kv_ranges.dtype != torch.int32 or tuple(kv_ranges.shape) != (B, 2) \
+                or not kv_ranges.is_cuda or not kv_ranges.is_contiguous() or not 1 <= max_keys <= min(512, Nk):
+            raise _lib.LcvError("attention: kv_ranges wants one packed k/v sequence, an int32 [B, 2] device table and 1 <= max_keys <= 512")
+        k_sb, v_sb, kv_rows, Nk = 0, 0, Nk, int(max_keys)
+    qn = (None, None, 0, 0.0, 1.0)
+    if q_norm is not None:
+        _req(q_norm.w, BF16, "attention.q_norm.w")
+        if q_norm.w.numel() != D or not q_norm.w.is_contiguous():
+            raise _lib.LcvError("attention: q_norm.w must be a contiguous [128] tensor")
+        if q_norm.cs is not None:
+            _req(q_norm.cs, F32, "attention.q_norm.cs")
+            if not q_norm.cs.is_contiguous() or q_norm.cs.shape[0] < q_norm.pos_off + Nq or q_norm.cs[0].numel() != D:
+                raise _lib.LcvError("attention: cos/sin table must be contiguous [rows, 64, 2] and reach pos_off + Nq rows")
+        qn = (_ptr(q_norm.w), _ptr(q_norm.cs), q_norm.pos_off, q_norm.eps, q_norm.q_scale)
     if out is None:
         out = torch.empty((B, Nq, H, D), dtype=BF16, device=q.device)
     lse = torch.empty((B, H, Nq), dtype=F32, device=q.device) if need_lse else None
@@ -149,9 +192,9 @@
         ev0 = torch.cuda.Event(enable_timing=True); ev1 = torch.cuda.Event(enable_timing=True)
         ev0.record()
     call("lcv_attn_fwd", _ptr(q), _ptr(k), _ptr(v), _ptr(out), _ptr(lse), B, H, Nq, Nk,
-         q.stride(0), q.stride(1), q.stride(2), k.stride(0), k.stride(1), k.stride(2),
-         v.stride(0), v.stride(1), v.stride(2), out.stride(0), out.stride(1), out.stride(2),
-         float(scale), _stream())
+         q.stride(0), q.stride(1), q.stride(2), k_sb, k.stride(1), k.stride(2),
+         v_sb, v.stride(1), v.stride(2), out.stride(0), out.stride(1), out.stride(2),
+         float(scale), *qn, _ptr(kv_ranges), kv_rows, _stream())
     if PROFILE is not None:
         ev1.record()
         PROFILE.append((ev0, ev1, 4.0 * B * H * Nq * Nk * D, Nq, Nk, _lib.load().lcv_attn_fwd_last_kernel().decode()))
diff --git a/longcat-video-tta_amd/longcat_video/modules/layers.py b/longcat-video-tta_amd/longcat_video/modules/layers.py
--- a/longcat-video-tta_amd/longcat_video/modules/layers.py
+++ b/longcat-video-tta_amd/longcat_video/modules/layers.py
@@ -122,8 +122,9 @@
         n_cond = 0
         if num_cond_latents is not None and num_cond_latents > 0:
             n_cond = num_cond_latents * (N // shape[0])
+        fq = not torch.is_grad_enabled() and not return_kv and is_pristine(self.q_norm, RMSNorm_FP32)
         o, kv = A.self_attention(qkv, self.q_norm.weight, self.k_norm.weight, cs, self.scale, n_cond,
-                                 self.q_norm.eps, return_kv)
+                                 self.q_norm.eps, return_kv, **({"fuse_q_norm": True} if fq else {}))
         out = _proj_out(self.proj, o.view(B, N, C), fuse_residual)
         if return_kv:
             return out, kv
@@ -180,8 +181,9 @@
         H, D = self.num_heads, self.head_dim
         q = self.q_linear(x).view(B, N, H, D)
         kv = self.kv_linear(cond).view(1, -1, 2, H, D)
+        fq = not torch.is_grad_enabled() and is_pristine(self.q_norm, RMSNorm_FP32)
         o = A.cross_attention(q, kv, self.q_norm.weight, self.k_norm.weight, list(kv_seqlen), self.scale,
-                              self.q_norm.eps)
+                              self.q_norm.eps, **({"fuse_q_norm": True} if fq else {}))
         return _proj_out(self.proj, o.view(B, N, C), fuse_residual)
 
     def forward(self, x, cond, kv_seqlen, num_cond_latents=None, shape=None, fuse_residual=None):
```

Result: no change. 0.06216 latent frames/s (median of 6 runs) (+0.9%).
